# JokerYan/MS-GS

Hardware: AMD Instinct MI355X
Metric: Mpixels/s fwd+bwd @1080p, 1M Gaussians; fraction of HBM roofline (higher is better)
Workload: dtype f32

## Files before the change

### __graft_entry__.py

```python
import os
import subprocess
import sys

ROOT = os.path.dirname(os.path.abspath(__file__))
PKG = os.path.join(ROOT, "ms-gs_amd")


def _paths():
    for p in (ROOT, PKG, os.path.join(PKG, "host"), os.path.join(ROOT, "tests")):
        if p not in sys.path:
            sys.path.insert(0, p)


def build():
    subprocess.check_call(["make", "-C", PKG, "-j4"])
    subprocess.call(["make", "-C", PKG, "isa"], stdout=subprocess.DEVNULL, stderr=subprocess.DEVNULL)
    subprocess.check_call(["make", "-C", os.path.join(ROOT, "oracle")])
    _paths()
    import diff_gaussian_rasterization
    import gaussian_renderer
    import view_parallel
    lib = os.path.join(PKG, "lib", "libmsgs_hip.so")
    assert os.path.exists(lib), lib
    harness = os.path.join(PKG, "build", "libmsgs_sort_harness.so")
    assert os.path.exists(harness), harness
    print("built", lib)


def smoke():
    _paths()
    import torch
    assert torch.cuda.is_available(), "smoke() needs a GPU"
    import scenes
    from oracle import oracle_ctypes as oc
    from parity_utils import check_backward, check_forward, hip_render, small_scene
    torch.cuda.set_device(0)
    W, H = 160, 96
    sc, cam = small_scene(4000, W, H, seed=123, multiscale=True, scale_k=0.004 * 1920.0 / W * 0.25)
    st = dict(filter_small=True, filter_large=True, fade_size=0.0)
    bg = torch.tensor([0.1, 0.2, 0.3])
    dL = scenes.grad_seed(W, H, 123)
    out, pc, m2 = hip_render(sc, cam, st, bg, dL, device="cuda:0")
    orc = oc.rasterize(pc.seen, cam, st, bg)
    og = oc.backward(orc, dL)
    fwd = check_forward(out, orc, "smoke")
    bwd = check_backward(pc, m2, og, "smoke", flagged=orc.borderline_gaussians)
    print(f"smoke ok: visible={(out['radii'] > 0).sum().item()} fwd_maxdiff={fwd:.2e} bwd_rel={max(bwd.values()):.2e}")


if __name__ == "__main__":
    build()
    if len(sys.argv) > 1 and sys.argv[1] == "smoke":
        smoke()
```

### include/msgs.h

```cpp
#ifndef MSGS_H_
#define MSGS_H_

#include <stddef.h>
#include <stdint.h>

#ifdef __cplusplus
extern "C" {
#endif

#define MSGS_ABI_VERSION 11

#define MSGS_OK 0
#define MSGS_ERR_INVALID_ARG (-1)
#define MSGS_ERR_CAPACITY (-2)
#define MSGS_ERR_TOO_MANY (-3)
#define MSGS_ERR_SH_DEGREE (-4)
#define MSGS_ERR_INTERNAL (-5)

#define MSGS_TILE 16

typedef struct msgs_view {
    int32_t image_height;
    int32_t image_width;
    float tanfovx;
    float tanfovy;
    float scale_modifier;
    float fade_size;
    int32_t sh_degree;
    int32_t sh_coeffs;
    int32_t filter_small;
    int32_t filter_large;
    int32_t prefiltered;
    int32_t debug;
    int32_t no_heavy_queue;
    int32_t feedback_tag;
    float slab_fraction;
    int32_t reserved1;
    const float* bg;
    const float* viewmatrix;
    const float* projmatrix;
    const float* campos;
} msgs_view_t;

typedef struct msgs_gaussians {
    int32_t P;
    int32_t raw_params;
    const float* means3D;
    const float* shs;
    const float* colors_precomp;
    const float* opacities;
    const float* scales;
    const float* rotations;
    const float* cov3D_precomp;
    const float* max_pixel_sizes;
    const float* min_pixel_sizes;
    const float* occ_multiplier;
    const float* dc_delta;
    const uint8_t* base_mask;
    const float* features_dc;
    const float* features_rest;
    const float* rotations_raw;
} msgs_gaussians_t;

typedef struct msgs_adam_moments {
    float* exp_avg;
    float* exp_avg_sq;
    double lr;
} msgs_adam_moments_t;
typedef struct msgs_adam_in_backward {
    int64_t step;
    double beta1, beta2, eps;
    msgs_adam_moments_t t[6];
} msgs_adam_in_backward_t;

typedef struct msgs_grads {
    float* dL_dmeans3D;
    float* dL_dmeans2D;
    float* dL_dshs;
    float* dL_dcolors;
    float* dL_dopacities;
    float* dL_dscales;
    float* dL_drotations;
    float* dL_dcov3D;
    float* dL_dfeatures_dc;
    float* dL_dfeatures_rest;
    void* factors_ready;
    int32_t scratch_is_clear;
    int32_t accumulate;
    void* wait_before_accumulate;
    void* accumulated;
    const msgs_adam_in_backward_t* adam_in_backward;
} msgs_grads_t;

enum {
    MSGS_K_PREPROCESS = 0, MSGS_K_DEPTH_SORT = 1, MSGS_K_SCAN = 2, MSGS_K_EMIT = 3,
    MSGS_K_TILE_SORT = 4, MSGS_K_RANGES = 5, MSGS_K_BLEND_FWD = 6, MSGS_K_BLEND_BWD = 7,
    MSGS_K_PREPROCESS_BWD = 8,
    MSGS_K_SLAB_B = 9,
    MSGS_K_COUNT = 10
};
typedef struct msgs_timing {
    void* ev[2 * MSGS_K_COUNT];
} msgs_timing_t;

int msgs_abi_version(void);
const char* msgs_error_string(int code);

size_t msgs_geom_bytes(int32_t P);
size_t msgs_stage1_scratch_bytes(int32_t P);
size_t msgs_binning_bytes(int64_t num_instances, int32_t width, int32_t height);
size_t msgs_binning_bytes_slab(int64_t num_instances, int32_t width, int32_t height, float slab_fraction);
size_t msgs_stage2_scratch_bytes_slab(int64_t num_instances, int32_t width, int32_t height);
size_t msgs_stage2_scratch_bytes(int64_t num_instances, int32_t width, int32_t height);
size_t msgs_image_bytes(int32_t width, int32_t height);
size_t msgs_backward_scratch_bytes(int32_t P);

int msgs_forward_stage1(const msgs_view_t* view, const msgs_gaussians_t* g,
                        int32_t* radii, float* pixel_sizes,
                        void* geom, size_t geom_bytes,
                        void* scratch, size_t scratch_bytes,
                        int64_t* num_instances_host,
                        const msgs_timing_t* timing, void* stream);

int msgs_forward_stage2(const msgs_view_t* view, const msgs_gaussians_t* g,
                        const void* geom, size_t geom_bytes,
                        int64_t num_instances,
                        void* binning, size_t binning_bytes,
                        void* scratch, size_t scratch_bytes,
                        void* image_state, size_t image_bytes,
                        float* out_color, float* out_acc_pixel_size, float* out_depth,
                        void* grad_records, size_t grad_records_bytes, int32_t backward_follows,
                        const msgs_timing_t* timing, void* stream);

int msgs_backward(const msgs_view_t* view, const msgs_gaussians_t* g,
                  const int32_t* radii,
                  const void* geom, size_t geom_bytes,
                  int64_t num_instances,
                  const void* binning, size_t binning_bytes,
                  const void* image_state, size_t image_bytes,
                  const float* dL_dcolor,
                  void* scratch, size_t scratch_bytes,
                  const msgs_grads_t* grads,
                  const msgs_timing_t* timing, void* stream);

int msgs_backward_with_depth(const msgs_view_t* view, const msgs_gaussians_t* g,
                             const int32_t* radii,
                             const void* geom, size_t geom_bytes,
                             int64_t num_instances,
                             const void* binning, size_t binning_bytes,
                             const void* image_state, size_t image_bytes,
                             const float* dL_dcolor, const float* dL_ddepth,
                             void* scratch, size_t scratch_bytes,
                             const msgs_grads_t* grads,
                             const msgs_timing_t* timing, void* stream);

int msgs_backward_with_camera(const msgs_view_t* view, const msgs_gaussians_t* g,
                              const int32_t* radii,
                              const void* geom, size_t geom_bytes,
                              int64_t num_instances,
                              const void* binning, size_t binning_bytes,
                              const void* image_state, size_t image_bytes,
                              const float* dL_dcolor, const float* dL_ddepth,
                              void* scratch, size_t scratch_bytes,
                              const msgs_grads_t* grads,
                              float* dL_dviewmatrix, float* dL_dprojmatrix, float* dL_dcampos,
                              void* camera_scratch, size_t camera_scratch_bytes,
                              const msgs_timing_t* timing, void* stream);
size_t msgs_camera_grad_scratch_bytes(int32_t P);

int msgs_alpha_map(const msgs_view_t* view, const void* image_state, size_t image_bytes, float* out_alpha, void* stream);

int msgs_backward_with_alpha(const msgs_view_t* view, const msgs_gaussians_t* g,
                             const int32_t* radii,
                             const void* geom, size_t geom_bytes,
                             int64_t num_instances,
                             const void* binning, size_t binning_bytes,
                             const void* image_state, size_t image_bytes,
                             const float* dL_dcolor, const float* dL_ddepth, const float* dL_dalpha,
                             void* scratch, size_t scratch_bytes,
                             const msgs_grads_t* grads,
                             float* dL_dviewmatrix, float* dL_dprojmatrix, float* dL_dcampos,
                             void* camera_scratch, size_t camera_scratch_bytes,
                             const msgs_timing_t* timing, void* stream);

size_t msgs_bg_grad_scratch_bytes(int32_t width, int32_t height);
int msgs_bg_grad(const msgs_view_t* view, const void* image_state, size_t image_bytes, const float* dL_dcolor,
                 float* dL_dbg, void* scratch, size_t scratch_bytes, void* stream);

size_t msgs_absgrad_scratch_bytes(int32_t P);
int msgs_absgrad(const msgs_view_t* view, int32_t P,
                 const void* geom, size_t geom_bytes,
                 int64_t num_instances,
                 const void* binning, size_t binning_bytes,
                 const void* image_state, size_t image_bytes,
                 const float* dL_dcolor, const float* dL_ddepth, const float* dL_dalpha,
                 void* scratch, size_t scratch_bytes,
                 float* out_absgrad, void* stream);

size_t msgs_contrib_scratch_bytes(int32_t P);
int msgs_contrib_accumulate(const msgs_view_t* view, int32_t P,
                            const void* geom, size_t geom_bytes,
                            int64_t num_instances,
                            const void* binning, size_t binning_bytes,
                            const void* image_state, size_t image_bytes,
                            const float* pixel_weights,
                            void* acc, size_t acc_bytes, int32_t clear_first, void* stream);
int msgs_contrib_finish(int32_t P, const void* acc, size_t acc_bytes,
                        float* weight_sum, float* weight_max, int64_t* pixel_count, void* stream);

size_t msgs_features_scratch_bytes(int32_t P, int32_t C);
int msgs_features_forward(const msgs_view_t* view, int32_t P,
                          const void* geom, size_t geom_bytes,
                          int64_t num_instances,
                          const void* binning, size_t binning_bytes,
                          const void* image_state, size_t image_bytes,
                          const float* features, int32_t C,
                          float* out, void* stream);
int msgs_features_backward(const msgs_view_t* view, int32_t P,
                           const void* geom, size_t geom_bytes,
                           int64_t num_instances,
                           const void* binning, size_t binning_bytes,
                           const void* image_state, size_t image_bytes,
                           const float* features, int32_t C,
                           const float* dL_dfeature_map,
                           void* grad_records, size_t grad_records_bytes,
                           void* scratch, size_t scratch_bytes,
                           float* dL_dfeatures, void* stream);

int msgs_distortion_forward(const msgs_view_t* view, int32_t P,
                            const void* geom, size_t geom_bytes,
                            int64_t num_instances,
                            const void* binning, size_t binning_bytes,
                            const void* image_state, size_t image_bytes,
                            float* out_distortion, float* out_moment, void* stream);
int msgs_distortion_backward(const msgs_view_t* view, int32_t P,
                             const void* geom, size_t geom_bytes,
                             int64_t num_instances,
                             const void* binning, size_t binning_bytes,
                             const void* image_state, size_t image_bytes,
                             const float* moment, const float* dL_ddistortion,
                             void* grad_records, size_t grad_records_bytes, void* stream);

int msgs_median_depth_forward(const msgs_view_t* view, int32_t P,
                              const void* geom, size_t geom_bytes,
                              int64_t num_instances,
                              const void* binning, size_t binning_bytes,
                              const void* image_state, size_t image_bytes,
                              float* out_median_depth, int32_t* out_median_id, void* stream);
int msgs_median_depth_backward(const msgs_view_t* view, int32_t P,
                               const int32_t* median_id, const float* dL_dmedian_depth,
                               void* grad_records, size_t grad_records_bytes, void* stream);

size_t msgs_screen_compensation_scratch_bytes(int32_t P);
int msgs_screen_compensation_forward(const msgs_view_t* view, const msgs_gaussians_t* g, float* o_eff, void* stream);
int msgs_screen_compensation_backward(const msgs_view_t* view, const msgs_gaussians_t* g, const float* dL_do_eff,
                                      float* dL_dopacity, float* dL_dmeans3D, float* dL_dscales, float* dL_drotations,
                                      float* dL_dcov3D, float* dL_dV, void* scratch, size_t scratch_bytes, void* stream);

int msgs_backward_per_gaussian(const msgs_view_t* view, const msgs_gaussians_t* g, const int32_t* radii,
                               const void* geom, size_t geom_bytes, const double* sums2d, const msgs_grads_t* grads,
                               void* stream);

int msgs_sh_grad_from_views(int32_t P, int32_t n_views, int32_t sh_degree, const float* means3D, const float* campos,
                            int64_t campos_stride, const float* drgb, int64_t drgb_stride, float scale,
                            float* dL_dfeatures_dc, float* dL_dfeatures_rest, void* stream);

int msgs_mark_visible(int32_t P, const float* means3D, const float* viewmatrix,
                      const float* projmatrix, uint8_t* present, void* stream);

int msgs_binning_stats(const msgs_view_t* view, int32_t P, const int32_t* radii,
                       const void* binning, size_t binning_bytes,
                       const void* image_state, size_t image_bytes,
                       void* scratch, size_t scratch_bytes,
                       int64_t* out_host, void* stream);

int msgs_blend_lane_stats(const msgs_view_t* view, const void* geom, size_t geom_bytes, int32_t P, int64_t D,
                          const void* binning, size_t binning_bytes, const void* image_state, size_t image_bytes,
                          void* scratch, size_t scratch_bytes, int64_t* out_host, void* stream);

int msgs_set_deterministic(int32_t on);
int msgs_get_deterministic(void);
size_t msgs_backward_scratch_bytes_deterministic(int32_t P, int64_t D);
size_t msgs_backward_scratch_bytes_deterministic_depth(int32_t P, int64_t D);

int msgs_set_backward_generation(int32_t gen);

int msgs_set_blend_granularity(int32_t mode);

int msgs_set_occlusion(int32_t on);
int msgs_forward_info(int64_t* out_host);
int msgs_occlusion_stats(const void* geom, size_t geom_bytes, int32_t P, int64_t* out_host, void* stream);
int msgs_slab_stats(const void* geom, size_t geom_bytes, int32_t P, int64_t* out_host, void* stream);

int msgs_forward(const msgs_view_t* view, const msgs_gaussians_t* gaussians, int32_t* radii, float* pixel_sizes,
                 void* geom, size_t geom_bytes, void* scratch1, size_t scratch1_bytes, void* binning,
                 size_t binning_bytes, void* scratch2, size_t scratch2_bytes, void* image, size_t image_bytes,
                 float* out_color, float* out_acc_pixel_size, float* out_depth, void* grad_records,
                 size_t grad_records_bytes, int32_t backward_follows, int64_t* num_instances_host, int32_t* stage2_done,
                 const msgs_timing_t* timing, void* stream);

typedef struct msgs_status msgs_status_t;
int msgs_status_create(msgs_status_t** out);
int msgs_status_destroy(msgs_status_t* status);
int msgs_forward_launch(const msgs_view_t* view, const msgs_gaussians_t* gaussians, int32_t* radii, float* pixel_sizes,
                        void* geom, size_t geom_bytes, void* scratch1, size_t scratch1_bytes, void* binning,
                        size_t binning_bytes, void* scratch2, size_t scratch2_bytes, void* image, size_t image_bytes,
                        float* out_color, float* out_acc_pixel_size, float* out_depth, void* grad_records,
                        size_t grad_records_bytes, int32_t backward_follows, msgs_status_t* status,
                        const msgs_timing_t* timing, void* stream);
int msgs_forward_finish(msgs_status_t* status, int64_t* num_instances_host, int32_t* stage2_done);

int msgs_preprocess_only(const msgs_view_t* view, const msgs_gaussians_t* gaussians, int32_t* radii,
                         float* pixel_sizes, void* geom, size_t geom_bytes, void* stream);

size_t msgs_voxel_pool_scratch_bytes(int64_t M);
int msgs_voxel_pool_build(const float* positions, int64_t M, float voxel_size, uint32_t* order, uint32_t* seg_start,
                          int32_t* voxel_index, void* scratch, size_t scratch_bytes, int64_t* num_voxels_host,
                          void* stream);
int msgs_voxel_pool_average(const float* features, int32_t F, const uint32_t* order, const uint32_t* seg_start,
                            int64_t num_voxels, float* out, void* stream);

#define MSGS_ADAM_MAX_TENSORS 8
typedef struct msgs_adam_tensor {
    float* param;
    const float* grad;
    float* exp_avg;
    float* exp_avg_sq;
    int64_t n;
    double lr;
} msgs_adam_tensor_t;
int msgs_adam_step(const msgs_adam_tensor_t* tensors, int32_t n_tensors, int64_t step, double beta1, double beta2,
                   double eps, void* stream);

#define MSGS_STATS_BASE_MASK 1
#define MSGS_STATS_PIXEL_SIZES 2
#define MSGS_STATS_DENSIFY 4
typedef struct msgs_densify_stats {
    int32_t P;
    int32_t flags;
    int32_t reso_lvl;
    int32_t reso_lvls;
    const int32_t* radii;
    const float* pixel_sizes;
    const float* means2D_grad;
    const int64_t* target_reso_lvl;
    float* xyz_gradient_accum;
    float* denom;
    float* max_radii2D;
    float* max_pixel_sizes;
    float* min_pixel_sizes;
    uint8_t* base_mask;
} msgs_densify_stats_t;
int msgs_densify_stats(const msgs_densify_stats_t* stats, void* stream);

#define MSGS_DENSIFY_PRUNE 0
#define MSGS_DENSIFY_GROW 1
#define MSGS_DENSIFY_PRUNE_MASK 2
#define MSGS_DENSIFY_APPEND 3
typedef struct msgs_densify_select {
    int32_t mode;
    int32_t reso_lvl;
    int32_t reso_lvls;
    int32_t has_max_screen_size;
    int64_t P;
    int64_t n_append;
    float grad_threshold;
    float min_opacity;
    float scale_limit;
    float big_world_limit;
    float max_screen_size;
    int32_t reserved;
    const float* opacity;
    const float* scaling;
    float* xyz_gradient_accum;
    float* denom;
    const int64_t* target_reso_lvl;
    const uint8_t* prune_mask;
} msgs_densify_select_t;
size_t msgs_densify_scratch_bytes(int64_t P, int64_t n_append);
int msgs_densify_select(const msgs_densify_select_t* sel, void* scratch, size_t scratch_bytes, int64_t* counts_host,
                        void* stream);

#define MSGS_DR_COPY 0
#define MSGS_DR_ZERO 1
#define MSGS_DR_COPY_CLEAR_COL 2
#define MSGS_DR_SPLIT_XYZ 3
#define MSGS_DR_SPLIT_SCALE 4
#define MSGS_DR_SPLIT_DIV 5
#define MSGS_DR_GROW_OPACITY 6
#define MSGS_DR_GROW_SCALE 7
#define MSGS_DR_GROW_MUL 8
#define MSGS_DR_CONST 9
#define MSGS_DR_APPEND 10
#define MSGS_DENSIFY_MAX_TENSORS 32
typedef struct msgs_densify_tensor {
    void* dst;
    const void* src;
    const void* append_src;
    int64_t constant;
    int32_t width;
    int32_t elem_bytes;
    uint8_t rule[8];
} msgs_densify_tensor_t;
typedef struct msgs_densify_apply {
    int64_t P;
    int64_t n_append;
    int64_t P_out;
    int64_t n_split;
    int32_t n_tensors;
    int32_t reso_lvl;
    const float* xyz;
    const float* scaling;
    const float* rotation;
    const float* draws;
    const msgs_densify_tensor_t* tensors;
} msgs_densify_apply_t;
int msgs_densify_apply(const msgs_densify_apply_t* apply, const void* scratch, size_t scratch_bytes, void* stream);

size_t msgs_loss_scratch_bytes(int32_t C, int32_t H, int32_t W);
int msgs_loss_forward(const float* img, const float* gt, int32_t C, int32_t H, int32_t W, float lambda_dssim,
                      float* out3, void* scratch, size_t scratch_bytes, int32_t keep_for_backward, void* stream);
int msgs_loss_backward(const float* img, const float* gt, int32_t C, int32_t H, int32_t W, float lambda_dssim,
                       const float* upstream, const void* scratch, size_t scratch_bytes, float* dL_dimg, void* stream);
int msgs_ssim_window(float* taps11_host);

size_t msgs_knn_scratch_bytes(int64_t P);
int msgs_dist2_knn3(const float* points, int64_t P, float* mean_dist2, void* scratch, size_t scratch_bytes,
                    void* stream);

int msgs_timing_create(msgs_timing_t* t);
int msgs_timing_destroy(msgs_timing_t* t);
int msgs_timing_read(const msgs_timing_t* t, float* ms_host);

#ifdef __cplusplus
}
#endif
#endif
```

### ms-gs_amd/csrc/api.hip

```cpp
#include "msgs_internal.h"

#include <atomic>
#include <new>

#include <cstring>

using namespace msgs;

namespace {

struct Timer {
    const msgs_timing_t* t;
    hipStream_t s;
    void begin(int k) const { if (t && t->ev[2 * k]) (void)hipEventRecord((hipEvent_t)t->ev[2 * k], s); }
    void end(int k) const { if (t && t->ev[2 * k + 1]) (void)hipEventRecord((hipEvent_t)t->ev[2 * k + 1], s); }
};

inline int check_inputs(const msgs_view_t* v, const msgs_gaussians_t* g) {
    if (!v || !g) return MSGS_ERR_INVALID_ARG;
    if (g->P < 0 || v->image_width <= 0 || v->image_height <= 0) return MSGS_ERR_INVALID_ARG;
    if (!v->bg || !v->viewmatrix || !v->projmatrix || !v->campos) return MSGS_ERR_INVALID_ARG;
    if (g->P > 0 && (!g->means3D || !g->opacities)) return MSGS_ERR_INVALID_ARG;
    if (g->raw_params) {
        if (g->raw_params != 1 && g->raw_params != 2) return MSGS_ERR_INVALID_ARG;
        if (!g->features_dc || !g->features_rest || !g->scales || !g->rotations) return MSGS_ERR_INVALID_ARG;
        if (g->raw_params == 2 && !g->rotations_raw) return MSGS_ERR_INVALID_ARG;
        if ((g->shs && g->raw_params != 2) || g->colors_precomp || g->cov3D_precomp) return MSGS_ERR_INVALID_ARG;
        if (v->sh_degree < 0 || v->sh_degree > 3 || v->sh_coeffs != 16) return MSGS_ERR_SH_DEGREE;
        if ((v->image_width + TILE - 1) / TILE > 65535 || (v->image_height + TILE - 1) / TILE > 65535)
            return MSGS_ERR_INVALID_ARG;
        return MSGS_OK;
    }
    if ((g->shs != nullptr) == (g->colors_precomp != nullptr)) return MSGS_ERR_INVALID_ARG;
    const bool sr = g->scales != nullptr && g->rotations != nullptr;
    if ((g->scales != nullptr) != (g->rotations != nullptr)) return MSGS_ERR_INVALID_ARG;
    if (sr == (g->cov3D_precomp != nullptr)) return MSGS_ERR_INVALID_ARG;
    if (g->shs) {
        if (v->sh_degree < 0 || v->sh_degree > 3) return MSGS_ERR_SH_DEGREE;
        if ((v->sh_degree + 1) * (v->sh_degree + 1) > v->sh_coeffs) return MSGS_ERR_SH_DEGREE;
    }
    if ((v->image_width + TILE - 1) / TILE > 65535 || (v->image_height + TILE - 1) / TILE > 65535)
        return MSGS_ERR_INVALID_ARG;
    return MSGS_OK;
}

inline int debug_sync(const msgs_view_t* v, hipStream_t s) {
    if (!v->debug) return MSGS_OK;
    hipError_t e = hipStreamSynchronize(s);
    if (e != hipSuccess) return (int)e;
    e = hipGetLastError();
    return e == hipSuccess ? MSGS_OK : (int)e;
}

inline int tile_bits(int num_tiles) {
    int b = 1;
    while ((1ll << b) <= (long long)num_tiles) ++b;
    return b;
}

#define HIP_TRY(expr)                                   \
    do {                                                \
        hipError_t _e = (expr);                         \
        if (_e != hipSuccess) return (int)_e;           \
    } while (0)

}

extern "C" {

int msgs_abi_version(void) { return MSGS_ABI_VERSION; }

const char* msgs_error_string(int code) {
    switch (code) {
        case MSGS_OK: return "ok";
        case MSGS_ERR_INVALID_ARG: return "invalid argument (NULL or inconsistent pointers: provide exactly one of shs/colors_precomp and exactly one of scales+rotations/cov3D_precomp)";
        case MSGS_ERR_CAPACITY: return "a caller-supplied buffer is smaller than its size query";
        case MSGS_ERR_TOO_MANY: return "more than 2^32-1 tile instances";
        case MSGS_ERR_SH_DEGREE: return "sh_degree must be 0..3 and (sh_degree+1)^2 <= sh_coeffs";
        case MSGS_ERR_INTERNAL: return "internal error: a look-back wait in the sort/scan kernels timed out";
        default: return code > 0 ? hipGetErrorString((hipError_t)code) : "unknown error";
    }
}

size_t msgs_geom_bytes(int32_t P) { return GeomLayout(P > 0 ? P : 1).total; }
size_t msgs_stage1_scratch_bytes(int32_t P) { return Stage1Scratch(P > 0 ? P : 1).total; }
size_t msgs_binning_bytes(int64_t D, int32_t W, int32_t H) {
    return BinningLayout(D, (int64_t)((W + TILE - 1) / TILE) * ((H + TILE - 1) / TILE)).total;
}
size_t msgs_stage2_scratch_bytes(int64_t D, int32_t W, int32_t H) {
    (void)W; (void)H;
    const Stage2Scratch L(D);
    return L.total + align256(4 * (size_t)(D > 0 ? D : 1));
}
static int64_t tiles_of(int32_t W, int32_t H) { return (int64_t)((W + TILE - 1) / TILE) * ((H + TILE - 1) / TILE); }
size_t msgs_binning_bytes_slab(int64_t D, int32_t W, int32_t H, float fraction) {
    if (!(fraction > 0.f)) return msgs_binning_bytes(D, W, H);
    return msgs_binning_bytes(SlabGeom::ids_needed(D > 0 ? D : 1, (double)fraction, tiles_of(W, H)), W, H);
}
size_t msgs_stage2_scratch_bytes_slab(int64_t D, int32_t W, int32_t H) {
    return msgs_stage2_scratch_bytes((D > 0 ? D : 1) + SLAB_SLACK + 256, W, H);
}
size_t msgs_image_bytes(int32_t W, int32_t H) { return ImageLayout(W, H).total; }
size_t msgs_backward_scratch_bytes(int32_t P) {
    return align256(GRAD_REC_BYTES * (size_t)(P > 0 ? P : 1));
}
size_t msgs_backward_scratch_bytes_deterministic(int32_t P, int64_t D) { return DetScratch(P, D).total; }
size_t msgs_backward_scratch_bytes_deterministic_depth(int32_t P, int64_t D) { return DetScratch(P, D, DET_INST_FLOATS_DEPTH).total; }

static std::atomic<int> g_deterministic{[] { const char* e = getenv("MSGS_DETERMINISTIC"); return (e && e[0] == '1') ? 1 : 0; }()};
int msgs_set_deterministic(int32_t on) { return g_deterministic.exchange(on ? 1 : 0); }
int msgs_get_deterministic(void) { return g_deterministic.load(); }
int msgs_set_backward_generation(int32_t gen) { return set_backward_generation(gen); }
int msgs_set_blend_granularity(int32_t mode) { return set_blend_granularity(mode); }
int msgs_set_occlusion(int32_t on) { return set_occlusion(on); }

}

namespace {
struct Stage2Buffers {
    void* binning; size_t binning_bytes;
    void* scratch2; size_t scratch2_bytes;
    void* image; size_t image_bytes;
    float* out_color; float* out_acc_ps; float* out_depth;
    void* grad_records; size_t grad_records_bytes;
    int backward_follows;
};

struct SpecStage2 {
    int64_t capacity;
    Stage2Buffers buf;
    int launched_rc;
};
int forward_stage2_impl(const msgs_view_t* view, const msgs_gaussians_t* g, const void* geom_v, size_t geom_bytes, int64_t D,
                        const Stage2Buffers& b, const msgs_timing_t* timing, void* stream, const uint32_t* D_dev,
                        uint64_t* fb_dev, uint64_t fb_ticket);

struct StatusBlock {
    uint64_t* host = nullptr;
    uint64_t* dev = nullptr;
    uint64_t ticket = 0;
    bool tried = false;
    void ensure() {
        if (tried) return;
        tried = true;
        void* h = nullptr;
        if (hipHostMalloc(&h, 64, hipHostMallocPortable | hipHostMallocMapped) == hipSuccess) {
            void* d = nullptr;
            if (hipHostGetDevicePointer(&d, h, 0) == hipSuccess) {
                host = (uint64_t*)h;
                dev = (uint64_t*)d;
                for (int k = 0; k < 8; ++k) host[k] = 0;
            } else {
                (void)hipHostFree(h);
            }
        }
        (void)hipGetLastError();
    }
    void release() {
        if (host) (void)hipHostFree(host);
        host = dev = nullptr;
        tried = false;
    }
};

struct PendingCount {
    bool active = false;
    bool polled = false;
    hipStream_t stream = nullptr;
    uint64_t ticket = 0;
    volatile uint64_t* host = nullptr;
    const uint64_t* status_dev = nullptr;
};

thread_local uint64_t t_last_info = 0;
thread_local uint64_t t_last_feedback[4] = {0, 0, 0, 0};

static bool blocking_sync() {
    static const bool blocking = [] { const char* e = getenv("MSGS_BLOCKING_SYNC"); return e && e[0] == '1'; }();
    return blocking;
}

static bool slab_wanted(const msgs_view_t* view, const msgs_gaussians_t* g) {
    const float f = view->slab_fraction;
    if (!(f > 0.f) || !(f <= 0.5f) || g->P <= 0 || g_deterministic.load() != 0) return false;
    const int64_t tiles = (int64_t)((view->image_width + TILE - 1) / TILE) * ((view->image_height + TILE - 1) / TILE);
    return tiles >= SLAB_MIN_TILES && tiles < 65535 * 16 && forward_uses_quadrant_kernel((int)tiles);
}

int forward_stage1_launch(const msgs_view_t* view, const msgs_gaussians_t* g, int32_t* radii, float* pixel_sizes,
                          void* geom_v, size_t geom_bytes, void* scratch_v, size_t scratch_bytes,
                          const msgs_timing_t* timing, void* stream, SpecStage2* spec, StatusBlock& sb,
                          PendingCount& pend) {
    pend.active = false;
    int rc = check_inputs(view, g);
    if (rc) return rc;
    const int P = g->P;
    if (P == 0) return MSGS_OK;
    if (!radii || !pixel_sizes || !geom_v || !scratch_v) return MSGS_ERR_INVALID_ARG;
    if (geom_bytes < msgs_geom_bytes(P) || scratch_bytes < msgs_stage1_scratch_bytes(P)) return MSGS_ERR_CAPACITY;
    hipStream_t s = (hipStream_t)stream;
    char* geom = (char*)geom_v;
    char* scratch = (char*)scratch_v;
    const GeomLayout GL(P);
    const Stage1Scratch SL(P);
    const ViewParams vp = make_view_params(view);
    const Timer tm{timing, s};

    ZeroJob zj1{nullptr, 0, (uint32_t*)(geom + GL.slab_hdr), (GL.occ_hdr - GL.slab_hdr) / 4 + sizeof(OccHeader) / 4 + 2 * (size_t)OCC_BUCKETS};
    const bool sort1_prezeroed = radix_sort_zero_region(P, 0, 32, scratch + SL.sort, &zj1.p0, &zj1.n0);
    const bool occlusion = get_occlusion() != 0;
    uint32_t* heavy_list = occlusion ? (uint32_t*)(scratch + SL.heavy_list) : nullptr;
    uint32_t* heavy_count = occlusion ? (uint32_t*)(scratch + SL.heavy_count) : nullptr;
    uint32_t* heavy_blk = occlusion ? (uint32_t*)(scratch + SL.heavy_blk) : nullptr;
    tm.begin(MSGS_K_PREPROCESS);
    HIP_TRY(launch_preprocess(vp, *g, radii, pixel_sizes, geom, s, zj1, heavy_list, heavy_count, heavy_blk, g_deterministic.load() != 0));
    if (occlusion)
        HIP_TRY(launch_occlusion(vp, P, geom, heavy_list, heavy_count, heavy_blk, (OccCand*)(scratch + SL.occ_cand), s));
    tm.end(MSGS_K_PREPROCESS);
    if ((rc = debug_sync(view, s))) return rc;

    if (!blocking_sync()) sb.ensure();
    const bool polled = !blocking_sync() && sb.host != nullptr;
    const uint64_t ticket = ++sb.ticket;
    uint64_t* total_dev = (uint64_t*)(scratch + SL.total_out);
    uint64_t* status_dev = total_dev + 2;
    uint32_t* clamped_dev = (uint32_t*)(total_dev + 5);
    uint32_t* heavy_q_word = spec ? (uint32_t*)((char*)spec->buf.scratch2 + Stage2Scratch(spec->capacity).heavy_q) : nullptr;

    tm.begin(MSGS_K_DEPTH_SORT);
    HIP_TRY(radix_sort_pairs((uint32_t*)(geom + GL.key), nullptr, (uint32_t*)(geom + GL.skey),
                             (uint32_t*)(geom + GL.order), P, 0, 32, scratch + SL.sort, s, sort1_prezeroed,
                             (uint32_t*)(geom + GL.nvalid)));
    tm.end(MSGS_K_DEPTH_SORT);
    if ((rc = debug_sync(view, s))) return rc;
    tm.begin(MSGS_K_SCAN);
    HIP_TRY(exclusive_scan_u32((const uint32_t*)(geom + GL.tiles), (const uint32_t*)(geom + GL.order),
                               (uint32_t*)(geom + GL.offs), P, (uint64_t*)(scratch + SL.scan_partials), total_dev, s,
                               status_dev, polled ? sb.dev : nullptr, ticket,
                               (const uint32_t*)(geom + GL.nvalid), spec ? clamped_dev : nullptr,
                               spec ? (uint64_t)spec->capacity : 0, (const uint32_t*)(geom + GL.occ_hdr), heavy_q_word, nullptr,
                               vp.cell_sx >= 0 ? TILE_COUNT_MASK : 0xFFFFFFFFu,
                               vp.cell_sx >= 0 && slab_wanted(view, g) ? (uint32_t*)(geom + GL.offs_b) : nullptr,
                               &reinterpret_cast<SlabHeader*>(geom + GL.slab_hdr)->pad[0]));
    tm.end(MSGS_K_SCAN);
    pend.active = true;
    pend.polled = polled;
    pend.stream = s;
    pend.ticket = ticket;
    pend.host = sb.host;
    pend.status_dev = status_dev;
    if (spec)
        spec->launched_rc = forward_stage2_impl(view, g, geom_v, geom_bytes, spec->capacity, spec->buf, timing, stream,
                                                clamped_dev, polled ? sb.dev : nullptr, ticket);
    return MSGS_OK;
}

int forward_stage1_wait(PendingCount& pend, int64_t* num_instances_host) {
    *num_instances_host = 0;
    if (!pend.active) { t_last_info = 0; for (int k = 0; k < 4; ++k) t_last_feedback[k] = 0; return MSGS_OK; }
    pend.active = false;
    hipStream_t s = pend.stream;
    uint64_t host_status[3] = {0, 0, 0};
    if (pend.polled) {
        volatile uint64_t* hv = pend.host;
        const uint64_t ticket = pend.ticket;
        uint64_t spins = 0;
        while (hv[2] != ticket) {
            if ((++spins & 0xFFFF) == 0) {
                const hipError_t q = hipStreamQuery(s);
                if (q != hipErrorNotReady && q != hipSuccess) return (int)q;
                if (q == hipSuccess && hv[2] != ticket) {
                    HIP_TRY(hipMemcpyAsync(host_status, pend.status_dev, sizeof(host_status), hipMemcpyDeviceToHost, s));
                    HIP_TRY(hipStreamSynchronize(s));
                    break;
                }
            }
        }
        if (hv[2] == ticket) { host_status[0] = hv[0]; host_status[1] = hv[1]; host_status[2] = hv[3]; }
        for (int k = 0; k < 4; ++k) t_last_feedback[k] = 0;
        for (int attempt = 0; attempt < 4; ++attempt) {
            const uint64_t w7 = hv[7], w4 = hv[4], w5 = hv[5], w6 = hv[6];
            if (hv[7] == w7) { t_last_feedback[0] = w4; t_last_feedback[1] = w5; t_last_feedback[2] = w6; t_last_feedback[3] = w7; break; }
        }
    } else {
        for (int k = 0; k < 4; ++k) t_last_feedback[k] = 0;
        HIP_TRY(hipMemcpyAsync(host_status, pend.status_dev, sizeof(host_status), hipMemcpyDeviceToHost, s));
        HIP_TRY(hipStreamSynchronize(s));
    }
    const uint64_t total = host_status[0];
    t_last_info = host_status[2];
    if (host_status[1] != 0) return MSGS_ERR_INTERNAL;
    if (total > 0xFFFFFFFFull) return MSGS_ERR_TOO_MANY;
    *num_instances_host = (int64_t)total;
    return MSGS_OK;
}

StatusBlock& thread_status_block() {
    static thread_local StatusBlock sb;
    return sb;
}

template <class F>
static int64_t max_instances_for(size_t bytes, F bytes_of) {
    if (bytes_of(1) > bytes) return 0;
    int64_t lo = 1, hi = 0xFFFFFFFFll;
    while (lo < hi) {
        const int64_t mid = lo + (hi - lo + 1) / 2;
        if (bytes_of(mid) <= bytes) lo = mid; else hi = mid - 1;
    }
    return lo;
}

void stage2_capacities(const msgs_view_t* view, size_t binning_bytes, size_t scratch2_bytes, int64_t& cb, int64_t& cs) {
    const int W0 = view->image_width, H0 = view->image_height;
    cb = max_instances_for(binning_bytes, [&](int64_t d) { return msgs_binning_bytes(d, W0, H0); });
    cs = max_instances_for(scratch2_bytes, [&](int64_t d) { return msgs_stage2_scratch_bytes(d, W0, H0); });
}

bool prepare_spec(const msgs_view_t* view, const msgs_gaussians_t* g, const Stage2Buffers& b, SpecStage2& spec) {
    if (view->debug || g->P <= 0 || !b.binning || !b.scratch2 || !b.image || !b.out_color || !b.out_acc_ps || !b.out_depth ||
        view->image_width <= 0 || view->image_height <= 0)
        return false;
    const int W0 = view->image_width, H0 = view->image_height;
    int64_t cb, cs;
    stage2_capacities(view, b.binning_bytes, b.scratch2_bytes, cb, cs);
    int64_t cap = cb < cs ? cb : cs;
    const int tiles0 = ((W0 + TILE - 1) / TILE) * ((H0 + TILE - 1) / TILE);
    if (slab_wanted(view, g)) {
        const SlabGeom SG(cb, cs, (double)view->slab_fraction, tiles0, (int64_t)1 << 40);
        if (SG.ok && SG.cap_d >= 4096) cap = SG.cap_d;
    }
    if (cap < 4096 || !radix_sort_supports_device_count(cap, 0, tile_bits(tiles0))) return false;
    spec.capacity = cap;
    spec.buf = b;
    spec.launched_rc = MSGS_OK;
    return true;
}

struct ForwardLaunch {
    PendingCount pend;
    bool spec = false;
    int64_t capacity = 0;
    int launched_rc = MSGS_OK;
};

int forward_launch(const msgs_view_t* view, const msgs_gaussians_t* g, int32_t* radii, float* pixel_sizes, void* geom,
                   size_t geom_bytes, void* scratch1, size_t scratch1_bytes, const Stage2Buffers* b,
                   const msgs_timing_t* timing, void* stream, StatusBlock& sb, ForwardLaunch& fl) {
    SpecStage2 spec{};
    fl.spec = b && prepare_spec(view, g, *b, spec);
    const int rc = forward_stage1_launch(view, g, radii, pixel_sizes, geom, geom_bytes, scratch1, scratch1_bytes, timing,
                                         stream, fl.spec ? &spec : nullptr, sb, fl.pend);
    if (rc) return rc;
    fl.capacity = spec.capacity;
    fl.launched_rc = spec.launched_rc;
    return MSGS_OK;
}

int forward_finish(ForwardLaunch& fl, int64_t* num_instances_host, int32_t* stage2_done) {
    *stage2_done = 0;
    const int rc = forward_stage1_wait(fl.pend, num_instances_host);
    if (rc) return rc;
    if (fl.spec && fl.launched_rc != MSGS_OK) return fl.launched_rc;
    *stage2_done = fl.spec && *num_instances_host <= fl.capacity;
    return MSGS_OK;
}

int forward_stage2_exact(const msgs_view_t* view, const msgs_gaussians_t* g, const void* geom, size_t geom_bytes, int64_t D,
                         const Stage2Buffers& b, const msgs_timing_t* timing, void* stream) {
    uint64_t* fb_dev = nullptr;
    uint64_t fb_ticket = 0;
    if (view && view->feedback_tag != 0 && !blocking_sync()) {
        StatusBlock& sb = thread_status_block();
        sb.ensure();
        fb_dev = sb.dev;
        fb_ticket = sb.ticket;
    }
    return forward_stage2_impl(view, g, geom, geom_bytes, D, b, timing, stream, nullptr, fb_dev, fb_ticket);
}

}

struct msgs_status {
    StatusBlock sb;
    ForwardLaunch fl;
    bool launched = false;
};

extern "C" {

int msgs_forward_stage1(const msgs_view_t* view, const msgs_gaussians_t* g, int32_t* radii, float* pixel_sizes,
                        void* geom_v, size_t geom_bytes, void* scratch_v, size_t scratch_bytes,
                        int64_t* num_instances_host, const msgs_timing_t* timing, void* stream) {
    if (!num_instances_host) return MSGS_ERR_INVALID_ARG;
    *num_instances_host = 0;
    ForwardLaunch fl;
    int32_t stage2_done;
    const int rc = forward_launch(view, g, radii, pixel_sizes, geom_v, geom_bytes, scratch_v, scratch_bytes, nullptr, timing,
                                  stream, thread_status_block(), fl);
    return rc ? rc : forward_finish(fl, num_instances_host, &stage2_done);
}

int msgs_status_create(msgs_status_t** out) {
    if (!out) return MSGS_ERR_INVALID_ARG;
    *out = new (std::nothrow) msgs_status();
    if (!*out) return (int)hipErrorOutOfMemory;
    if (!blocking_sync()) (*out)->sb.ensure();
    return MSGS_OK;
}

int msgs_status_destroy(msgs_status_t* st) {
    if (!st) return MSGS_OK;
    if (st->launched && st->fl.pend.active) (void)hipStreamSynchronize(st->fl.pend.stream);
    st->sb.release();
    delete st;
    return MSGS_OK;
}

int msgs_forward_launch(const msgs_view_t* view, const msgs_gaussians_t* g, int32_t* radii, float* pixel_sizes, void* geom,
                        size_t geom_bytes, void* scratch1, size_t scratch1_bytes, void* binning, size_t binning_bytes,
                        void* scratch2, size_t scratch2_bytes, void* image, size_t image_bytes, float* out_color,
                        float* out_acc_ps, float* out_depth, void* grad_records, size_t grad_records_bytes,
                        int32_t backward_follows, msgs_status_t* status, const msgs_timing_t* timing, void* stream) {
    if (!view || !g || !status) return MSGS_ERR_INVALID_ARG;
    if (status->launched) return MSGS_ERR_INVALID_ARG;
    const Stage2Buffers b{binning, binning_bytes, scratch2, scratch2_bytes, image, image_bytes, out_color, out_acc_ps, out_depth,
                          grad_records, grad_records_bytes, backward_follows};
    const int rc = forward_launch(view, g, radii, pixel_sizes, geom, geom_bytes, scratch1, scratch1_bytes, &b, timing, stream,
                                  status->sb, status->fl);
    if (rc) return rc;
    status->launched = true;
    return MSGS_OK;
}

int msgs_forward_finish(msgs_status_t* status, int64_t* num_instances_host, int32_t* stage2_done) {
    if (!status || !num_instances_host || !stage2_done) return MSGS_ERR_INVALID_ARG;
    *stage2_done = 0;
    *num_instances_host = 0;
    if (!status->launched) return MSGS_ERR_INVALID_ARG;
    status->launched = false;
    return forward_finish(status->fl, num_instances_host, stage2_done);
}

int msgs_forward(const msgs_view_t* view, const msgs_gaussians_t* g, int32_t* radii, float* pixel_sizes, void* geom,
                 size_t geom_bytes, void* scratch1, size_t scratch1_bytes, void* binning, size_t binning_bytes,
                 void* scratch2, size_t scratch2_bytes, void* image, size_t image_bytes, float* out_color,
                 float* out_acc_ps, float* out_depth, void* grad_records, size_t grad_records_bytes,
                 int32_t backward_follows, int64_t* num_instances_host, int32_t* stage2_done, const msgs_timing_t* timing,
                 void* stream) {
    if (!stage2_done) return MSGS_ERR_INVALID_ARG;
    *stage2_done = 0;
    if (!view || !g || !num_instances_host) return MSGS_ERR_INVALID_ARG;
    *num_instances_host = 0;
    const Stage2Buffers b{binning, binning_bytes, scratch2, scratch2_bytes, image, image_bytes, out_color, out_acc_ps, out_depth,
                          grad_records, grad_records_bytes, backward_follows};
    ForwardLaunch fl;
    int rc = forward_launch(view, g, radii, pixel_sizes, geom, geom_bytes, scratch1, scratch1_bytes, &b, timing, stream,
                            thread_status_block(), fl);
    if (!rc) rc = forward_finish(fl, num_instances_host, stage2_done);
    if (rc || fl.spec) return rc;
    const int64_t D = *num_instances_host;
    const int W = view->image_width, H = view->image_height;
    if (!binning || binning_bytes < msgs_binning_bytes(D, W, H)) return MSGS_OK;
    if (D > 0 && (!scratch2 || scratch2_bytes < msgs_stage2_scratch_bytes(D, W, H))) return MSGS_OK;
    if ((rc = forward_stage2_exact(view, g, geom, geom_bytes, D, b, timing, stream))) return rc;
    *stage2_done = 1;
    return MSGS_OK;
}

int msgs_preprocess_only(const msgs_view_t* view, const msgs_gaussians_t* g, int32_t* radii, float* pixel_sizes,
                         void* geom_v, size_t geom_bytes, void* stream) {
    int rc = check_inputs(view, g);
    if (rc) return rc;
    const int P = g->P;
    if (P == 0) return MSGS_OK;
    if (!radii || !pixel_sizes || !geom_v) return MSGS_ERR_INVALID_ARG;
    if (geom_bytes < msgs_geom_bytes(P)) return MSGS_ERR_CAPACITY;
    hipStream_t s = (hipStream_t)stream;
    HIP_TRY(launch_preprocess(make_view_params(view), *g, radii, pixel_sizes, (char*)geom_v, s));
    return debug_sync(view, s);
}

int msgs_forward_stage2(const msgs_view_t* view, const msgs_gaussians_t* g, const void* geom_v, size_t geom_bytes,
                        int64_t D, void* binning_v, size_t binning_bytes, void* scratch_v, size_t scratch_bytes,
                        void* image_v, size_t image_bytes, float* out_color, float* out_acc_ps, float* out_depth,
                        void* grad_records, size_t grad_records_bytes, int32_t backward_follows, const msgs_timing_t* timing,
                        void* stream) {
    const Stage2Buffers b{binning_v, binning_bytes, scratch_v, scratch_bytes, image_v, image_bytes, out_color, out_acc_ps,
                          out_depth, grad_records, grad_records_bytes, backward_follows};
    return forward_stage2_exact(view, g, geom_v, geom_bytes, D, b, timing, stream);
}

}

namespace {
int forward_stage2_impl(const msgs_view_t* view, const msgs_gaussians_t* g, const void* geom_v, size_t geom_bytes, int64_t D,
                        const Stage2Buffers& b, const msgs_timing_t* timing, void* stream, const uint32_t* D_dev,
                        uint64_t* fb_dev, uint64_t fb_ticket) {
    int rc = check_inputs(view, g);
    if (rc) return rc;
    if (D < 0 || D > 0xFFFFFFFFll) return MSGS_ERR_TOO_MANY;
    const int P = g->P, W = view->image_width, H = view->image_height;
    if (!b.binning || !b.image || !b.out_color || !b.out_acc_ps || !b.out_depth) return MSGS_ERR_INVALID_ARG;
    if (P > 0 && (!geom_v || geom_bytes < msgs_geom_bytes(P))) return MSGS_ERR_CAPACITY;
    if (b.binning_bytes < msgs_binning_bytes(D, W, H) || b.image_bytes < msgs_image_bytes(W, H)) return MSGS_ERR_CAPACITY;
    if (D > 0 && (!b.scratch2 || b.scratch2_bytes < msgs_stage2_scratch_bytes(D, W, H))) return MSGS_ERR_CAPACITY;
    if (b.grad_records && b.grad_records_bytes < msgs_backward_scratch_bytes(P)) return MSGS_ERR_CAPACITY;
    hipStream_t s = (hipStream_t)stream;
    char* geom = const_cast<char*>((const char*)geom_v);
    char* binning = (char*)b.binning;
    char* scratch = (char*)b.scratch2;
    char* image = (char*)b.image;
    const ViewParams vp = make_view_params(view);
    const int num_tiles = vp.gx * vp.gy;
    const ImageLayout IL(W, H);
    const Timer tm{timing, s};
    const int tbits = tile_bits(num_tiles);
    const BinningLayout BL(D, num_tiles);
    uint32_t* ids = (uint32_t*)(binning + BL.ids);
    uint2* ranges = (uint2*)(binning + BL.ranges);
    float* final_T = (float*)(image + IL.final_T);
    uint32_t* n_contrib = (uint32_t*)(image + IL.n_contrib);
    uint32_t* tile_last = (uint32_t*)(image + IL.tile_last);
    const bool literal = g_deterministic.load() != 0;
    const bool feedback = view->feedback_tag != 0 && fb_dev != nullptr && P > 0 && forward_uses_quadrant_kernel(num_tiles) && !literal;
    unsigned long long* dtrav = feedback ? (unsigned long long*)(binning + BL.dtrav) : nullptr;
    const size_t clear_bytes = b.grad_records ? GRAD_REC_BYTES * (size_t)P : 0;

    bool slab = D > 0 && slab_wanted(view, g) && radix_sort_supports_device_count(D, 0, tbits);
    int64_t n_a_max = 0, cap_b = 0;
    if (slab) {
        int64_t cb, cs;
        stage2_capacities(view, b.binning_bytes, b.scratch2_bytes, cb, cs);
        const SlabGeom SG(cb, cs, (double)view->slab_fraction, num_tiles, D);
        slab = SG.ok && SG.cap_d == D && SortScratch(SG.n_a_max).total <= SortScratch(SG.cap_b).total;
// ... 326 lines not shown
    if (P == 0 || D == 0) {
        HIP_TRY(launch_zero(out_distortion, sizeof(float) * (size_t)W * H, s));
        HIP_TRY(launch_zero(out_moment, sizeof(float) * (size_t)W * H, s));
        return debug_sync(view, s);
    }
    if (!geom_v || !binning_v || !image_v) return MSGS_ERR_INVALID_ARG;
    if (geom_bytes < msgs_geom_bytes(P) || binning_bytes < msgs_binning_bytes(D, W, H) || image_bytes < msgs_image_bytes(W, H))
        return MSGS_ERR_CAPACITY;
    const ViewParams vp = make_view_params(view);
    const BinningLayout BL(D, vp.gx * vp.gy);
    const ImageLayout IL(W, H);
    const char* binning = (const char*)binning_v;
    const char* image = (const char*)image_v;
    HIP_TRY(launch_blend_distortion_forward(vp, (const char*)geom_v, (const uint32_t*)(binning + BL.ids),
                                            (const uint2*)(binning + BL.ranges), (const float*)(image + IL.final_T),
                                            (const uint32_t*)(image + IL.n_contrib), out_distortion, out_moment, s));
    return debug_sync(view, s);
}

int msgs_distortion_backward(const msgs_view_t* view, int32_t P, const void* geom_v, size_t geom_bytes, int64_t D,
                             const void* binning_v, size_t binning_bytes, const void* image_v, size_t image_bytes,
                             const float* moment, const float* dL_ddistortion, void* grad_records, size_t grad_records_bytes,
                             void* stream) {
    if (!view || P < 0 || D < 0 || view->image_width < 1 || view->image_height < 1) return MSGS_ERR_INVALID_ARG;
    if (g_deterministic.load() != 0) return MSGS_ERR_INVALID_ARG;
    if (P == 0 || D == 0) return MSGS_OK;
    if (!geom_v || !binning_v || !image_v || !moment || !dL_ddistortion || !grad_records || ((uintptr_t)grad_records & 7))
        return MSGS_ERR_INVALID_ARG;
    const int W = view->image_width, H = view->image_height;
    if (geom_bytes < msgs_geom_bytes(P) || binning_bytes < msgs_binning_bytes(D, W, H) || image_bytes < msgs_image_bytes(W, H) ||
        grad_records_bytes < msgs_backward_scratch_bytes(P))
        return MSGS_ERR_CAPACITY;
    hipStream_t s = (hipStream_t)stream;
    const ViewParams vp = make_view_params(view);
    const BinningLayout BL(D, vp.gx * vp.gy);
    const ImageLayout IL(W, H);
    const char* binning = (const char*)binning_v;
    const char* image = (const char*)image_v;
    HIP_TRY(launch_blend_distortion_backward(vp, (const char*)geom_v, (const uint32_t*)(binning + BL.ids),
                                             (const uint2*)(binning + BL.ranges), (const float*)(image + IL.final_T),
                                             (const uint32_t*)(image + IL.n_contrib), moment, dL_ddistortion,
                                             (grad_acc_t*)grad_records, s));
    return debug_sync(view, s);
}

int msgs_median_depth_forward(const msgs_view_t* view, int32_t P, const void* geom_v, size_t geom_bytes, int64_t D,
                              const void* binning_v, size_t binning_bytes, const void* image_v, size_t image_bytes,
                              float* out_median_depth, int32_t* out_median_id, void* stream) {
    if (!view || P < 0 || D < 0 || view->image_width < 1 || view->image_height < 1 || !out_median_depth || !out_median_id)
        return MSGS_ERR_INVALID_ARG;
    if (g_deterministic.load() != 0) return MSGS_ERR_INVALID_ARG;
    const int W = view->image_width, H = view->image_height;
    hipStream_t s = (hipStream_t)stream;
    if (P == 0 || D == 0) {
        HIP_TRY(launch_zero(out_median_depth, sizeof(float) * (size_t)W * H, s));
        HIP_TRY(hipMemsetAsync(out_median_id, 0xFF, sizeof(int32_t) * (size_t)W * H, s));
        return debug_sync(view, s);
    }
    if (!geom_v || !binning_v || !image_v) return MSGS_ERR_INVALID_ARG;
    if (geom_bytes < msgs_geom_bytes(P) || binning_bytes < msgs_binning_bytes(D, W, H) || image_bytes < msgs_image_bytes(W, H))
        return MSGS_ERR_CAPACITY;
    const ViewParams vp = make_view_params(view);
    const BinningLayout BL(D, vp.gx * vp.gy);
    const ImageLayout IL(W, H);
    const char* binning = (const char*)binning_v;
    const char* image = (const char*)image_v;
    HIP_TRY(launch_blend_median_depth_forward(vp, (const char*)geom_v, (const uint32_t*)(binning + BL.ids),
                                              (const uint2*)(binning + BL.ranges), (const uint32_t*)(image + IL.n_contrib),
                                              out_median_depth, out_median_id, s));
    return debug_sync(view, s);
}

int msgs_median_depth_backward(const msgs_view_t* view, int32_t P, const int32_t* median_id, const float* dL_dmedian_depth,
                               void* grad_records, size_t grad_records_bytes, void* stream) {
    if (!view || P < 0 || view->image_width < 1 || view->image_height < 1) return MSGS_ERR_INVALID_ARG;
    if (g_deterministic.load() != 0) return MSGS_ERR_INVALID_ARG;
    if (P == 0) return MSGS_OK;
    if (!median_id || !dL_dmedian_depth || !grad_records || ((uintptr_t)grad_records & 7)) return MSGS_ERR_INVALID_ARG;
    if (grad_records_bytes < msgs_backward_scratch_bytes(P)) return MSGS_ERR_CAPACITY;
    hipStream_t s = (hipStream_t)stream;
    const ViewParams vp = make_view_params(view);
    HIP_TRY(launch_median_depth_backward(vp, P, median_id, dL_dmedian_depth, (grad_acc_t*)grad_records, s));
    return debug_sync(view, s);
}

}
namespace {
inline int check_compensation_inputs(const msgs_view_t* v, const msgs_gaussians_t* g) {
    if (!v || !g || g->P < 0 || v->image_width <= 0 || v->image_height <= 0 || !v->viewmatrix) return MSGS_ERR_INVALID_ARG;
    if (g->raw_params != 0) return MSGS_ERR_INVALID_ARG;
    if (g->P == 0) return MSGS_OK;
    if (!g->means3D || !g->opacities) return MSGS_ERR_INVALID_ARG;
    const bool sr = g->scales != nullptr && g->rotations != nullptr;
    if ((g->scales != nullptr) != (g->rotations != nullptr) || sr == (g->cov3D_precomp != nullptr)) return MSGS_ERR_INVALID_ARG;
    return MSGS_OK;
}
}
extern "C" {

size_t msgs_screen_compensation_scratch_bytes(int32_t P) { return screen_compensation_rows_bytes(P); }

int msgs_screen_compensation_forward(const msgs_view_t* view, const msgs_gaussians_t* g, float* o_eff, void* stream) {
    const int rc = check_compensation_inputs(view, g);
    if (rc != MSGS_OK) return rc;
    if (g->P == 0) return MSGS_OK;
    if (!o_eff) return MSGS_ERR_INVALID_ARG;
    hipStream_t s = (hipStream_t)stream;
    HIP_TRY(launch_screen_compensation_forward(make_view_params(view), *g, o_eff, s));
    return debug_sync(view, s);
}

int msgs_screen_compensation_backward(const msgs_view_t* view, const msgs_gaussians_t* g, const float* dL_do_eff,
                                      float* dL_dopacity, float* dL_dmeans3D, float* dL_dscales, float* dL_drotations,
                                      float* dL_dcov3D, float* dL_dV, void* scratch, size_t scratch_bytes, void* stream) {
    const int rc = check_compensation_inputs(view, g);
    if (rc != MSGS_OK) return rc;
    hipStream_t s = (hipStream_t)stream;
    if (g->P == 0) {
        if (dL_dV) HIP_TRY(launch_zero(dL_dV, sizeof(float) * 16, s));
        return debug_sync(view, s);
    }
    if (!dL_do_eff) return MSGS_ERR_INVALID_ARG;
    if ((g->cov3D_precomp && (dL_dscales || dL_drotations)) || (!g->cov3D_precomp && dL_dcov3D)) return MSGS_ERR_INVALID_ARG;
    if (dL_dV) {
        if (!scratch || ((uintptr_t)scratch & 7)) return MSGS_ERR_INVALID_ARG;
        if (scratch_bytes < msgs_screen_compensation_scratch_bytes(g->P)) return MSGS_ERR_CAPACITY;
    }
    HIP_TRY(launch_screen_compensation_backward(make_view_params(view), *g, dL_do_eff, dL_dopacity, dL_dmeans3D, dL_dscales,
                                                dL_drotations, dL_dcov3D, dL_dV, (double*)scratch, s));
    return debug_sync(view, s);
}
}

namespace {
int backward_impl(const msgs_view_t* view, const msgs_gaussians_t* g, const int32_t* radii, const void* geom_v,
                  size_t geom_bytes, int64_t D, const void* binning_v, size_t binning_bytes, const void* image_v,
                  size_t image_bytes, const float* dL_dcolor, const float* dL_ddepth, const float* dL_dalpha, void* scratch_v,
                  size_t scratch_bytes, const msgs_grads_t* grads, const CameraGrads* cam, const msgs_timing_t* timing,
                  void* stream) {
    int rc = check_inputs(view, g);
    if (rc) return rc;
    if (!grads || !dL_dcolor) return MSGS_ERR_INVALID_ARG;
    const int P = g->P, W = view->image_width, H = view->image_height;
    if (P == 0) {
        if (cam) {
            hipStream_t s0 = (hipStream_t)stream;
            if (cam->dL_dviewmatrix) HIP_TRY(hipMemsetAsync(cam->dL_dviewmatrix, 0, 16 * sizeof(float), s0));
            if (cam->dL_dprojmatrix) HIP_TRY(hipMemsetAsync(cam->dL_dprojmatrix, 0, 16 * sizeof(float), s0));
            if (cam->dL_dcampos) HIP_TRY(hipMemsetAsync(cam->dL_dcampos, 0, 3 * sizeof(float), s0));
        }
        return MSGS_OK;
    }
    if (!radii || !geom_v || !binning_v || !image_v || !scratch_v) return MSGS_ERR_INVALID_ARG;
    const bool det = g_deterministic.load() != 0;
    if (geom_bytes < msgs_geom_bytes(P) || binning_bytes < msgs_binning_bytes(D, W, H) ||
        image_bytes < msgs_image_bytes(W, H) ||
        scratch_bytes < (det ? (dL_ddepth ? msgs_backward_scratch_bytes_deterministic_depth(P, D)
                                          : msgs_backward_scratch_bytes_deterministic(P, D))
                             : msgs_backward_scratch_bytes(P)))
        return MSGS_ERR_CAPACITY;
    if (g->shs && !g->raw_params && !grads->dL_dshs) return MSGS_ERR_INVALID_ARG;
    if (g->raw_params && (!grads->dL_dfeatures_dc != !grads->dL_dfeatures_rest)) return MSGS_ERR_INVALID_ARG;
    if (g->raw_params && !grads->dL_dfeatures_dc && !grads->dL_dcolors && !grads->adam_in_backward) return MSGS_ERR_INVALID_ARG;
    if (const msgs_adam_in_backward_t* ad = grads->adam_in_backward) {
        if (g->raw_params != 1 || !g->features_dc || !g->features_rest || g->shs || g->colors_precomp || g->cov3D_precomp ||
            !g->scales || !g->rotations || view->sh_coeffs != 16 || grads->accumulate || grads->wait_before_accumulate ||
            ad->step < 1)
            return MSGS_ERR_INVALID_ARG;
        uintptr_t bits = (uintptr_t)g->means3D | (uintptr_t)g->features_dc | (uintptr_t)g->features_rest |
                         (uintptr_t)g->opacities | (uintptr_t)g->scales | (uintptr_t)g->rotations;
        for (int t = 0; t < 6; ++t) {
            if (!ad->t[t].exp_avg || !ad->t[t].exp_avg_sq) return MSGS_ERR_INVALID_ARG;
            bits |= (uintptr_t)ad->t[t].exp_avg | (uintptr_t)ad->t[t].exp_avg_sq;
        }
        if (bits & 15) return MSGS_ERR_INVALID_ARG;
    }
    if (grads->accumulate && ((g->shs && !g->raw_params && view->sh_coeffs != 16) ||
                              (g->raw_params && !grads->dL_dfeatures_dc)))
        return MSGS_ERR_INVALID_ARG;
    hipStream_t s = (hipStream_t)stream;
    const char* geom = (const char*)geom_v;
    const char* binning = (const char*)binning_v;
    const char* image = (const char*)image_v;
    const ViewParams vp = make_view_params(view);
    const BinningLayout BL(D, vp.gx * vp.gy);
    const ImageLayout IL(W, H);
    const Timer tm{timing, s};
    grad_acc_t* grad_rec = (grad_acc_t*)scratch_v;

    if (det && grads->scratch_is_clear) return MSGS_ERR_INVALID_ARG;
    if (!grads->scratch_is_clear)
        HIP_TRY(launch_zero(grad_rec, GRAD_REC_BYTES * (size_t)P, s));
    tm.begin(MSGS_K_BLEND_BWD);
    if (det)
        HIP_TRY(launch_blend_backward_det(vp, P, geom, (const uint32_t*)(binning + BL.ids), D,
                                          (const uint2*)(binning + BL.ranges), (const float*)(image + IL.final_T),
                                          (const uint32_t*)(image + IL.n_contrib), dL_dcolor, (char*)scratch_v, s, dL_ddepth,
                                          dL_dalpha));
    else
        HIP_TRY(launch_blend_backward(vp, geom, (const uint32_t*)(binning + BL.ids), (const uint2*)(binning + BL.ranges),
                                      (const float*)(image + IL.final_T), (const uint32_t*)(image + IL.n_contrib),
                                      dL_dcolor, grad_rec, s, (const uint32_t*)(image + IL.tile_order), dL_ddepth,
                                      dL_dalpha));
    tm.end(MSGS_K_BLEND_BWD);
    if ((rc = debug_sync(view, s))) return rc;

    tm.begin(MSGS_K_PREPROCESS_BWD);
    HIP_TRY(launch_preprocess_backward(vp, *g, radii, geom, grad_rec, *grads, s, det, dL_ddepth != nullptr, cam));
    tm.end(MSGS_K_PREPROCESS_BWD);
    return debug_sync(view, s);
}
}

extern "C" {

int msgs_backward_per_gaussian(const msgs_view_t* view, const msgs_gaussians_t* g, const int32_t* radii,
                               const void* geom_v, size_t geom_bytes, const double* sums2d, const msgs_grads_t* grads,
                               void* stream) {
    int rc = check_inputs(view, g);
    if (rc) return rc;
    if (!grads || g->raw_params || grads->adam_in_backward) return MSGS_ERR_INVALID_ARG;
    if (grads->accumulate || grads->wait_before_accumulate || grads->accumulated) return MSGS_ERR_INVALID_ARG;
    const int P = g->P;
    if (P == 0) return MSGS_OK;
    if (!radii || !geom_v || !sums2d) return MSGS_ERR_INVALID_ARG;
    if (geom_bytes < msgs_geom_bytes(P)) return MSGS_ERR_CAPACITY;
    if (g->shs && !grads->dL_dshs) return MSGS_ERR_INVALID_ARG;
    hipStream_t s = (hipStream_t)stream;
    HIP_TRY(launch_preprocess_backward(make_view_params(view), *g, radii, (const char*)geom_v,
                                       reinterpret_cast<const grad_acc_t*>(sums2d), *grads, s, true));
    return debug_sync(view, s);
}

int msgs_sh_grad_from_views(int32_t P, int32_t n_views, int32_t sh_degree, const float* means3D, const float* campos,
                            int64_t campos_stride, const float* drgb, int64_t drgb_stride, float scale,
                            float* dL_dfeatures_dc, float* dL_dfeatures_rest, void* stream) {
    if (P < 0 || n_views < 1 || sh_degree < 0 || sh_degree > 3 || campos_stride < 0 || drgb_stride < 0)
        return MSGS_ERR_INVALID_ARG;
    if (P > 0 && (!means3D || !campos || !drgb || !dL_dfeatures_dc || !dL_dfeatures_rest)) return MSGS_ERR_INVALID_ARG;
    HIP_TRY(launch_sh_grad_from_views(P, n_views, sh_degree, means3D, campos, campos_stride, drgb, drgb_stride, scale,
                                      dL_dfeatures_dc, dL_dfeatures_rest, (hipStream_t)stream));
    return MSGS_OK;
}

int msgs_mark_visible(int32_t P, const float* means3D, const float* viewmatrix, const float* projmatrix,
                      uint8_t* present, void* stream) {
    if (P < 0 || (P > 0 && (!means3D || !viewmatrix || !present))) return MSGS_ERR_INVALID_ARG;
    HIP_TRY(launch_mark_visible(P, means3D, viewmatrix, projmatrix, present, (hipStream_t)stream));
    return MSGS_OK;
}

int msgs_binning_stats(const msgs_view_t* view, int32_t P, const int32_t* radii, const void* binning,
                       size_t binning_bytes, const void* image_v, size_t image_bytes, void* scratch,
                       size_t scratch_bytes, int64_t* out_host, void* stream) {
    (void)binning; (void)binning_bytes;
    if (!view || !image_v || !scratch || !out_host || scratch_bytes < 16) return MSGS_ERR_INVALID_ARG;
    const int W = view->image_width, H = view->image_height;
    if (image_bytes < msgs_image_bytes(W, H)) return MSGS_ERR_CAPACITY;
    hipStream_t s = (hipStream_t)stream;
    const ViewParams vp = make_view_params(view);
    const ImageLayout IL(W, H);
    unsigned long long* dev = (unsigned long long*)scratch;
    HIP_TRY(launch_binning_stats(vp, P, radii, (const uint32_t*)((const char*)image_v + IL.n_contrib), dev, s));
    unsigned long long host[2] = {0, 0};
    HIP_TRY(hipMemcpyAsync(host, dev, 16, hipMemcpyDeviceToHost, s));
    HIP_TRY(hipStreamSynchronize(s));
    out_host[0] = (int64_t)host[0];
    out_host[1] = (int64_t)host[1];
    return MSGS_OK;
}

int msgs_forward_info(int64_t* out_host) {
    if (!out_host) return MSGS_ERR_INVALID_ARG;
    out_host[0] = (int64_t)(t_last_info & 0xFFFFFFFFull);
    out_host[1] = (int64_t)(t_last_info >> 32) != 0 ? 1 : 0;
    const uint64_t w4 = t_last_feedback[0], w5 = t_last_feedback[1], w6 = t_last_feedback[2], w7 = t_last_feedback[3];
    const uint32_t n_open = (uint32_t)(w5 >> 32);
    out_host[2] = (int64_t)(w5 & 0xFFFFFFFFull);
    out_host[3] = (int64_t)(w7 & 0xFFFFFFFFFFull);
    out_host[4] = (int64_t)(w4 & ~(1ull << 63));
    out_host[5] = n_open == 0xFFFFFFFFu ? -1 : (int64_t)n_open;
    out_host[6] = (int64_t)(w6 & 0xFFFFFFFFull);
    out_host[7] = (w4 >> 63) ? -1 : (int64_t)(w6 >> 32);
    return MSGS_OK;
}

int msgs_slab_stats(const void* geom_v, size_t geom_bytes, int32_t P, int64_t* out_host, void* stream) {
    if (!geom_v || !out_host || P <= 0) return MSGS_ERR_INVALID_ARG;
    if (geom_bytes < msgs_geom_bytes(P)) return MSGS_ERR_CAPACITY;
    const GeomLayout GL(P);
    SlabHeader h;
    hipStream_t s = (hipStream_t)stream;
    HIP_TRY(hipMemcpyAsync(&h, (const char*)geom_v + GL.slab_hdr, sizeof(h), hipMemcpyDeviceToHost, s));
    HIP_TRY(hipStreamSynchronize(s));
    out_host[0] = h.active;
    out_host[1] = h.rA;
    out_host[2] = h.DA;
    out_host[3] = h.n_open;
    out_host[4] = (int64_t)h.total_b;
    out_host[5] = h.pad0;
    return MSGS_OK;
}

int msgs_occlusion_stats(const void* geom_v, size_t geom_bytes, int32_t P, int64_t* out_host, void* stream) {
    if (!geom_v || !out_host || P <= 0) return MSGS_ERR_INVALID_ARG;
    if (geom_bytes < msgs_geom_bytes(P)) return MSGS_ERR_CAPACITY;
    const GeomLayout GL(P);
    OccHeader h;
    hipStream_t s = (hipStream_t)stream;
    static uint32_t table[OCC_MAX_BLOCKS];
    HIP_TRY(hipMemcpyAsync(&h, (const char*)geom_v + GL.occ_hdr, sizeof(h), hipMemcpyDeviceToHost, s));
    HIP_TRY(hipStreamSynchronize(s));
    for (int k = 0; k < 8; ++k) out_host[k] = 0;
    out_host[0] = h.enabled ? (h.watchdog ? 2 : 1) : 0;
    if (!h.enabled) return MSGS_OK;
    const int n_blocks = (int)(h.nbx * h.nby);
    if (n_blocks < 0 || n_blocks > OCC_MAX_BLOCKS) return MSGS_ERR_INTERNAL;
    if (h.any_closed) {
        HIP_TRY(hipMemcpyAsync(table, (const char*)geom_v + GL.occ_cut, 4 * (size_t)n_blocks, hipMemcpyDeviceToHost, s));
        HIP_TRY(hipStreamSynchronize(s));
    } else {
        for (int k = 0; k < n_blocks; ++k) table[k] = 0xFFFFu;
    }
    uint32_t lo = 0xFFFFFFFFu, hi = 0u;
    int closed = 0;
    for (int k = 0; k < n_blocks; ++k) {
        const uint32_t key = table[k] >= 0xFFFFu ? 0xFFFFFFFFu : (((table[k] + OCC_KEY_BASE + 1u) << OCC_KEY_SHIFT) - 1u);
        closed += key != 0xFFFFFFFFu;
        lo = key < lo ? key : lo;
        hi = key > hi ? key : hi;
    }
    out_host[1] = h.n_heavy;
    out_host[2] = h.n_cand;
    out_host[3] = closed;
    out_host[4] = n_blocks;
    out_host[5] = 1u << h.block_log2;
    out_host[6] = lo;
    out_host[7] = hi;
    return MSGS_OK;
}

int msgs_blend_lane_stats(const msgs_view_t* view, const void* geom, size_t geom_bytes, int32_t P, int64_t D,
                          const void* binning_v, size_t binning_bytes, const void* image_v, size_t image_bytes,
                          void* scratch, size_t scratch_bytes, int64_t* out_host, void* stream) {
    if (!view || !geom || !binning_v || !scratch || !out_host || scratch_bytes < 64 || P < 0) return MSGS_ERR_INVALID_ARG;
    const int W = view->image_width, H = view->image_height;
    if (geom_bytes < msgs_geom_bytes(P) || binning_bytes < msgs_binning_bytes(D, W, H)) return MSGS_ERR_CAPACITY;
    if (image_v && image_bytes < msgs_image_bytes(W, H)) return MSGS_ERR_CAPACITY;
    hipStream_t s = (hipStream_t)stream;
    const ViewParams vp = make_view_params(view);
    const BinningLayout BL(D, vp.gx * vp.gy);
    const ImageLayout IL(W, H);
    const char* binning = (const char*)binning_v;
    unsigned long long* dev = (unsigned long long*)scratch;
    HIP_TRY(launch_blend_lane_stats(vp, (const char*)geom, (const uint32_t*)(binning + BL.ids),
                                    (const uint2*)(binning + BL.ranges), dev, s));
    if (image_v)
        HIP_TRY(launch_blend_backward_lane_stats(vp, (const char*)geom, (const uint32_t*)(binning + BL.ids),
                                                 (const uint2*)(binning + BL.ranges),
                                                 (const float*)((const char*)image_v + IL.final_T),
                                                 (const uint32_t*)((const char*)image_v + IL.n_contrib), dev + 4, s));
    unsigned long long host[8] = {0, 0, 0, 0, 0, 0, 0, 0};
    HIP_TRY(hipMemcpyAsync(host, dev, 64, hipMemcpyDeviceToHost, s));
    HIP_TRY(hipStreamSynchronize(s));
    for (int k = 0; k < 3; ++k) out_host[k] = (int64_t)host[k];
    for (int k = 0; k < 4; ++k) out_host[3 + k] = image_v ? (int64_t)host[4 + k] : -1;
    return MSGS_OK;
}

int msgs_adam_step(const msgs_adam_tensor_t* tensors, int32_t n_tensors, int64_t step, double beta1, double beta2,
                   double eps, void* stream) {
    if (n_tensors < 0 || n_tensors > MSGS_ADAM_MAX_TENSORS || step < 1 || (n_tensors && !tensors))
        return MSGS_ERR_INVALID_ARG;
    for (int k = 0; k < n_tensors; ++k) {
        const msgs_adam_tensor_t& t = tensors[k];
        if (t.n < 0 || (t.n > 0 && (!t.param || !t.grad || !t.exp_avg || !t.exp_avg_sq))) return MSGS_ERR_INVALID_ARG;
        if (t.n > (int64_t)1 << 40) return MSGS_ERR_TOO_MANY;
    }
    HIP_TRY(launch_adam(tensors, n_tensors, step, beta1, beta2, eps, (hipStream_t)stream));
    return MSGS_OK;
}

int msgs_densify_stats(const msgs_densify_stats_t* d, void* stream) {
    if (!d || d->P < 0 || d->reso_lvls < 1 || d->reso_lvl < 0 || d->reso_lvl >= d->reso_lvls) return MSGS_ERR_INVALID_ARG;
    if (d->P == 0 || d->flags == 0) return MSGS_OK;
    if (!d->radii) return MSGS_ERR_INVALID_ARG;
    if ((d->flags & MSGS_STATS_BASE_MASK) && !d->base_mask) return MSGS_ERR_INVALID_ARG;
    if ((d->flags & MSGS_STATS_PIXEL_SIZES) &&
        (!d->pixel_sizes || !d->target_reso_lvl || !d->max_pixel_sizes || !d->min_pixel_sizes)) return MSGS_ERR_INVALID_ARG;
    if ((d->flags & MSGS_STATS_DENSIFY) && (!d->means2D_grad || !d->xyz_gradient_accum || !d->denom || !d->max_radii2D))
        return MSGS_ERR_INVALID_ARG;
    HIP_TRY(launch_densify_stats(*d, (hipStream_t)stream));
    return MSGS_OK;
}

size_t msgs_densify_scratch_bytes(int64_t P, int64_t n_append) {
    return densify_scratch_bytes(P > 0 ? P : 0, n_append > 0 ? n_append : 0);
}

int msgs_densify_select(const msgs_densify_select_t* sel, void* scratch, size_t scratch_bytes, int64_t* counts_host,
                        void* stream) {
    if (!sel || !counts_host || !scratch) return MSGS_ERR_INVALID_ARG;
    if (int rc = densify_check_select(*sel)) return rc;
    if (scratch_bytes < densify_scratch_bytes(sel->P, sel->n_append)) return MSGS_ERR_CAPACITY;
    return densify_select(*sel, (char*)scratch, counts_host, (hipStream_t)stream);
}

int msgs_densify_apply(const msgs_densify_apply_t* apply, const void* scratch, size_t scratch_bytes, void* stream) {
    if (!apply || !scratch) return MSGS_ERR_INVALID_ARG;
    if (int rc = densify_check_apply(*apply)) return rc;
    if (scratch_bytes < densify_scratch_bytes(apply->P, apply->n_append)) return MSGS_ERR_CAPACITY;
    return densify_apply(*apply, (const char*)scratch, (hipStream_t)stream);
}

static int loss_args_ok(const float* img, const float* gt, int32_t C, int32_t H, int32_t W, float lambda) {
    if (!img || !gt || C < 1 || H < 1 || W < 1 || !(lambda >= 0.f && lambda <= 1.f)) return MSGS_ERR_INVALID_ARG;
    if ((int64_t)C * H * W > (int64_t)1 << 31 || C > 65535) return MSGS_ERR_TOO_MANY;
    return MSGS_OK;
}

size_t msgs_loss_scratch_bytes(int32_t C, int32_t H, int32_t W) {
    if (C < 1 || H < 1 || W < 1) return 0;
    return loss_scratch_bytes(C, H, W);
}

int msgs_loss_forward(const float* img, const float* gt, int32_t C, int32_t H, int32_t W, float lambda_dssim,
                      float* out3, void* scratch, size_t scratch_bytes, int32_t keep_for_backward, void* stream) {
    if (int rc = loss_args_ok(img, gt, C, H, W, lambda_dssim)) return rc;
    if (!out3 || !scratch) return MSGS_ERR_INVALID_ARG;
    if (scratch_bytes < loss_scratch_bytes(C, H, W)) return MSGS_ERR_CAPACITY;
    HIP_TRY(launch_loss_forward(img, gt, C, H, W, lambda_dssim, out3, (char*)scratch, keep_for_backward != 0,
                                (hipStream_t)stream));
    return MSGS_OK;
}

int msgs_loss_backward(const float* img, const float* gt, int32_t C, int32_t H, int32_t W, float lambda_dssim,
                       const float* upstream, const void* scratch, size_t scratch_bytes, float* dL_dimg, void* stream) {
    if (int rc = loss_args_ok(img, gt, C, H, W, lambda_dssim)) return rc;
    if (!dL_dimg || !scratch) return MSGS_ERR_INVALID_ARG;
    if (scratch_bytes < loss_scratch_bytes(C, H, W)) return MSGS_ERR_CAPACITY;
    HIP_TRY(launch_loss_backward(img, gt, C, H, W, lambda_dssim, upstream, (const char*)scratch, dL_dimg,
                                 (hipStream_t)stream));
    return MSGS_OK;
}

int msgs_ssim_window(float* taps11_host) {
    if (!taps11_host) return MSGS_ERR_INVALID_ARG;
    ssim_window_host(taps11_host);
    return MSGS_OK;
}

size_t msgs_knn_scratch_bytes(int64_t P) { return knn_scratch_bytes(P); }

int msgs_dist2_knn3(const float* points, int64_t P, float* mean_dist2, void* scratch, size_t scratch_bytes,
                    void* stream) {
    if (P < 4 || !points || !mean_dist2 || !scratch) return MSGS_ERR_INVALID_ARG;
    if (P > 0x7FFFFFFFll) return MSGS_ERR_TOO_MANY;
    if (scratch_bytes < knn_scratch_bytes(P)) return MSGS_ERR_CAPACITY;
    HIP_TRY(knn_mean_dist2(points, P, mean_dist2, (char*)scratch, (hipStream_t)stream));
    return MSGS_OK;
}

size_t msgs_voxel_pool_scratch_bytes(int64_t M) { return voxel_pool_scratch_bytes(M); }

int msgs_voxel_pool_build(const float* positions, int64_t M, float voxel_size, uint32_t* order, uint32_t* seg_start,
                          int32_t* voxel_index, void* scratch, size_t scratch_bytes, int64_t* num_voxels_host,
                          void* stream) {
    if (!num_voxels_host || M < 0 || !(voxel_size > 0.f)) return MSGS_ERR_INVALID_ARG;
    *num_voxels_host = 0;
    if (M == 0) return MSGS_OK;
    if (M > 0x7FFFFFFFll) return MSGS_ERR_TOO_MANY;
    if (!positions || !order || !seg_start || !scratch) return MSGS_ERR_INVALID_ARG;
    if (scratch_bytes < voxel_pool_scratch_bytes(M)) return MSGS_ERR_CAPACITY;
    HIP_TRY(voxel_pool_build(positions, M, voxel_size, order, seg_start, voxel_index, (char*)scratch, num_voxels_host,
                             (hipStream_t)stream));
    return MSGS_OK;
}

int msgs_voxel_pool_average(const float* features, int32_t F, const uint32_t* order, const uint32_t* seg_start,
                            int64_t num_voxels, float* out, void* stream) {
    if (F < 0 || num_voxels < 0) return MSGS_ERR_INVALID_ARG;
    if (F == 0 || num_voxels == 0) return MSGS_OK;
    if (!features || !order || !seg_start || !out) return MSGS_ERR_INVALID_ARG;
    HIP_TRY(voxel_pool_average(features, F, order, seg_start, num_voxels, out, (hipStream_t)stream));
    return MSGS_OK;
}

int msgs_timing_create(msgs_timing_t* t) {
    if (!t) return MSGS_ERR_INVALID_ARG;
    std::memset(t, 0, sizeof(*t));
    for (int i = 0; i < 2 * MSGS_K_COUNT; ++i) {
        hipEvent_t e;
        HIP_TRY(hipEventCreate(&e));
        t->ev[i] = (void*)e;
    }
    return MSGS_OK;
}

int msgs_timing_destroy(msgs_timing_t* t) {
    if (!t) return MSGS_ERR_INVALID_ARG;
    for (int i = 0; i < 2 * MSGS_K_COUNT; ++i)
        if (t->ev[i]) { (void)hipEventDestroy((hipEvent_t)t->ev[i]); t->ev[i] = nullptr; }
    return MSGS_OK;
}

int msgs_timing_read(const msgs_timing_t* t, float* ms_host) {
    if (!t || !ms_host) return MSGS_ERR_INVALID_ARG;
    for (int k = 0; k < MSGS_K_COUNT; ++k) {
        float ms = -1.0f;
        if (t->ev[2 * k] && t->ev[2 * k + 1]) {
            if (hipEventElapsedTime(&ms, (hipEvent_t)t->ev[2 * k], (hipEvent_t)t->ev[2 * k + 1]) != hipSuccess) {
                ms = -1.0f;
                (void)hipGetLastError();
            }
        }
        ms_host[k] = ms;
    }
    return MSGS_OK;
}

}
```

### ms-gs_amd/csrc/msgs_internal.h

```cpp
#pragma once
#include <hip/hip_runtime.h>
#include <stdint.h>
#include <cmath>
#include <type_traits>
#include "../../include/msgs.h"

namespace msgs {

constexpr int TILE = MSGS_TILE;
constexpr int WAVE = 64;

struct __attribute__((aligned(16))) GaussRec { float4 r0, r1, r2; };

struct __attribute__((aligned(32))) BinRec { float4 q0, q1; };

#if defined(MSGS_GRAD_REC_F32)
typedef float grad_acc_t;
constexpr int GRAD_REC_FLOATS = 12;
#else
typedef double grad_acc_t;
constexpr int GRAD_REC_FLOATS = 10;
#endif
constexpr uint32_t TILE_ORDER_MAGIC = 0x4C505431u;
constexpr size_t GRAD_REC_BYTES = sizeof(grad_acc_t) * GRAD_REC_FLOATS;
constexpr int DET_INST_FLOATS = 9;
constexpr int DET_INST_FLOATS_DEPTH = 10;

__host__ __device__ inline size_t align256(size_t x) { return (x + 255) & ~size_t(255); }

constexpr int OCC_MAX_BLOCKS = 2048;
constexpr int OCC_MAX_CAND = 32768;
constexpr uint32_t OCC_HEAVY_MIN = 96;
constexpr int OCC_BUCKETS = 2048;
constexpr int OCC_KEY_SHIFT = 19;
constexpr uint32_t OCC_KEY_BASE = 0x3E4CCCCDu >> OCC_KEY_SHIFT;
struct OccHeader {
    uint32_t n_cand;
    uint32_t any_closed;
    uint32_t n_heavy;
    uint32_t enabled;
    uint32_t block_log2;
    uint32_t nbx;
    uint32_t nby;
    uint32_t n_written;
    uint32_t depth_limit;
    uint32_t bar[3];
    uint32_t watchdog;
    uint32_t pad[3];
};
static_assert(sizeof(OccHeader) == 64, "OccHeader layout");
constexpr int SLAB_SCAN_CHUNK = 4096;
struct __attribute__((aligned(16))) OccCand { float4 c0, c1; uint32_t rect_lo, rect_hi, pad0, pad1; };
static_assert(sizeof(OccCand) == 48, "OccCand layout");

struct SlabHeader {
    uint32_t rA;
    uint32_t DA;
    uint32_t DB;
    uint32_t active;
    uint32_t n_open;
    uint32_t pad0;
    uint64_t total_b;
    uint32_t pad[8];
};
static_assert(sizeof(SlabHeader) == 64, "SlabHeader layout");

struct GeomLayout {
    size_t rec, binrec, tiles, key, flags, weight, order, offs, nvalid, skey, slab_hdr, occ_hdr, occ_cut, offs_b, scan_b, litrec, shjac, total;
    __host__ __device__ explicit GeomLayout(int64_t P) {
        size_t o = 0;
        rec = o;    o = align256(o + sizeof(GaussRec) * P);
        binrec = o; o = align256(o + sizeof(BinRec) * P);
        tiles = o;  o = align256(o + 4 * P);
        key = o;    o = align256(o + 4 * P);
        flags = o;  o = align256(o + 4 * P);
        weight = o; o = align256(o + 4 * P);
        order = o;  o = align256(o + 4 * P);
        offs = o;   o = align256(o + 4 * P);
        nvalid = o; o += 256;
        skey = o;   o = align256(o + 4 * P);
        slab_hdr = o; o += 256;
        occ_hdr = o; o = align256(o + sizeof(OccHeader) + 8 * (size_t)OCC_BUCKETS);
        occ_cut = o; o = align256(o + 4 * (size_t)OCC_MAX_BLOCKS);
        offs_b = o; o = align256(o + 4 * P);
        scan_b = o; o = align256(o + 8 * (size_t)((P + SLAB_SCAN_CHUNK - 1) / SLAB_SCAN_CHUNK + 2));
        litrec = o; o = align256(o + 16 * P);
        shjac = o;  o = align256(o + 36 * P);
        total = o;
    }
};

constexpr int SORT_THREADS = 256;
constexpr int SORT_ITEMS = 4;
constexpr int64_t SORT_BIG_N = 2'000'000;
constexpr int64_t SORT_MID_N = 400'000;
constexpr int SORT_MAX_GROUPS = 128;
constexpr int64_t SORT_SCANNED_MIN_BLOCKS = 4096;
constexpr int SORT_SCANNED_GSIZE = 32;
constexpr int SCAN_THREADS = 256;
constexpr int SCAN_ITEMS = 16;
constexpr int SCAN_CHUNK = SCAN_THREADS * SCAN_ITEMS;
static_assert(SCAN_CHUNK == SLAB_SCAN_CHUNK, "GeomLayout::scan_b is sized with SLAB_SCAN_CHUNK");

__host__ __device__ inline int64_t scan_blocks(int64_t n) { return (n + SCAN_CHUNK - 1) / SCAN_CHUNK; }

struct SortGeom {
    bool big, mid, scanned;
    int items, gsize, ngroups;
    int64_t nb;
    __host__ __device__ explicit SortGeom(int64_t n) {
        if (n < 1) n = 1;
        big = n >= SORT_BIG_N;
        mid = !big && n >= SORT_MID_N;
        items = big ? 16 : (mid ? 8 : SORT_ITEMS);
        nb = (n + (int64_t)SORT_THREADS * items - 1) / ((int64_t)SORT_THREADS * items);
        scanned = big && nb >= SORT_SCANNED_MIN_BLOCKS;
        if (scanned) {
            gsize = SORT_SCANNED_GSIZE;
        } else {
            gsize = 8;
            while ((int64_t)gsize * gsize < nb) gsize += 8;
            const int64_t floor_g = (nb + SORT_MAX_GROUPS - 1) / SORT_MAX_GROUPS;
            if (floor_g > gsize) gsize = (int)floor_g;
        }
        ngroups = (int)((nb + gsize - 1) / gsize);
    }
    __host__ __device__ size_t zero_words(int passes) const { return (size_t)passes * 256 * ngroups; }
};

struct SortScratch {
    size_t keys_alt, vals_alt, hist, total;
    __host__ __device__ explicit SortScratch(int64_t n) {
        size_t o = 0;
        const size_t nn = (size_t)(n > 0 ? n : 1);
        const SortGeom G(n);
        keys_alt = o; o = align256(o + 4 * nn);
        vals_alt = o; o = align256(o + 4 * nn);
        hist = o;     o = align256(o + 4 * ((size_t)256 * G.nb + G.zero_words(4)));
        total = o;
    }
};

struct Stage1Scratch {
    size_t sort, scan_partials, total_out, heavy_list, heavy_count, heavy_blk, occ_cand, total;
    __host__ __device__ explicit Stage1Scratch(int64_t P) {
        size_t o = 0;
        const size_t Pn = (size_t)(P > 0 ? P : 1);
        const size_t waves = 4 * ((Pn + 255) / 256);
        sort = o;          o = align256(o + SortScratch(P).total);
        scan_partials = o; o = align256(o + 8 * (size_t)(scan_blocks(P > 0 ? P : 1) + 2));
        total_out = o;     o = align256(o + 64);
        heavy_list = o;    o = align256(o + 8 * 64 * waves);
        heavy_count = o;   o = align256(o + 4 * waves);
        heavy_blk = o;     o = align256(o + 2 * waves);
        occ_cand = o;      o = align256(o + sizeof(OccCand) * OCC_MAX_CAND);
        total = o;
    }
};

constexpr int DTRAV_SLOTS = 64;
struct BinningLayout {
    size_t ids, ranges, dtrav, total;
    __host__ __device__ BinningLayout(int64_t D, int64_t tiles) {
        size_t o = 0;
        ranges = o; o = align256(o + 8 * (size_t)tiles);
        dtrav = o;  o = align256(o + 8 * (size_t)DTRAV_SLOTS);
        ids = o;    o = align256(o + 4 * (size_t)(D > 0 ? D : 1));
        total = o;
    }
    __host__ __device__ size_t ranges_and_dtrav_words() const { return (dtrav + 8 * (size_t)DTRAV_SLOTS - ranges) / 4; }
};

constexpr int64_t SLAB_SLACK = 65536;
constexpr int SLAB_MIN_TILES = 2048;
struct SlabGeom {
    int64_t cap_d, n_a_max, cap_b;
    bool ok;
    __host__ SlabGeom(int64_t cb, int64_t cs, double fraction, int64_t tiles, int64_t cap_d_limit) {
        const int64_t by_ids = (int64_t)((double)(cb - tiles - SLAB_SLACK - 256) / (1.0 + fraction));
        const int64_t by_scratch = cs - SLAB_SLACK;
        cap_d = by_ids < by_scratch ? by_ids : by_scratch;
        if (cap_d > cap_d_limit) cap_d = cap_d_limit;
        if (cap_d < 0) cap_d = 0;
        n_a_max = (((int64_t)(fraction * (double)cap_d) + tiles + 64) + 63) & ~(int64_t)63;
        cap_b = cap_d + SLAB_SLACK;
        ok = cap_d > 0 && n_a_max + cap_b <= cb && cap_b <= cs && n_a_max + cap_b <= 0xFFFFFFFFll;
    }
    __host__ static int64_t ids_needed(int64_t D, double fraction, int64_t tiles) {
        return (int64_t)((double)(D + 1) * (1.0 + fraction)) + tiles + SLAB_SLACK + 512;
    }
};

constexpr uint32_t EMIT_HEAVY_MIN = 96;
struct Stage2Scratch {
    size_t keys_a, ids_a, sort, heavy_q, total;
    __host__ __device__ explicit Stage2Scratch(int64_t D) {
        size_t o = 0;
        int64_t n = D > 0 ? D : 1;
        keys_a = o; o = align256(o + 4 * (size_t)n);
        ids_a = o;  o = align256(o + 4 * (size_t)n);
        sort = o;   o = align256(o + SortScratch(n).total);
        heavy_q = o; o = align256(o + 4 * ((size_t)n / EMIT_HEAVY_MIN + 66));
        total = o;
    }
};

struct ImageLayout {
    size_t final_T, n_contrib, tile_last, tile_order, open_bits, open_list, total;
    __host__ __device__ ImageLayout(int64_t W, int64_t H) {
        size_t o = 0;
        const size_t tiles = (size_t)((W + TILE - 1) / TILE) * (size_t)((H + TILE - 1) / TILE);
        final_T = o;    o = align256(o + 4 * (size_t)(W * H));
        n_contrib = o;  o = align256(o + 4 * (size_t)(W * H));
        tile_last = o;  o = align256(o + 4 * tiles);
        tile_order = o; o = align256(o + 4 * (tiles + 1));
        open_bits = o;  o = align256(o + 4 * ((tiles + 31) / 32 + 1));
        open_list = o;  o = align256(o + 4 * tiles);
        total = o;
    }
};

__device__ __forceinline__ double wave_sum_f64(double v) {
    for (int off = 32; off > 0; off >>= 1) {
        const unsigned long long u = (unsigned long long)__double_as_longlong(v);
        const unsigned lo = (unsigned)__shfl_xor((int)(unsigned)u, off), hi = (unsigned)__shfl_xor((int)(unsigned)(u >> 32), off);
        v += __longlong_as_double((long long)(((unsigned long long)hi << 32) | lo));
    }
    return v;
}
struct AdamScalars {
    float w1;
    float beta2, w2;
    float bc2_sqrt, eps;
};
inline AdamScalars adam_scalars(int64_t step, double beta1, double beta2, double eps) {
    AdamScalars a;
    a.w1 = (float)(1.0 - beta1);
    a.beta2 = (float)beta2;
    a.w2 = (float)(1.0 - beta2);
    a.bc2_sqrt = (float)sqrt(1.0 - pow(beta2, (double)step));
    a.eps = (float)eps;
    return a;
}
inline float adam_neg_step_size(double lr, int64_t step, double beta1) { return (float)(-(lr / (1.0 - pow(beta1, (double)step)))); }

struct AdamInBackward {
    float* m[6];
    float* v[6];
    float nss[6];
    AdamScalars a;
};

constexpr int CAM_PARTIALS = 27;
constexpr int CAM_ROW = 32;
struct CamPartials {
    double* rows;
};
struct CameraGrads {
    float* dL_dviewmatrix;
    float* dL_dprojmatrix;
    float* dL_dcampos;
    double* rows;
};
size_t camera_grad_rows_bytes(int P);

#if defined(__HIPCC__)

__device__ __forceinline__ void adam_update(float& p, float g, float& m, float& v, float nss, const AdamScalars& a) {
#pragma clang fp contract(off)
    m = __fmaf_rn(a.w1, g - m, m);
    v = __fmaf_rn(a.w2 * g, g, v * a.beta2);
    const float denom = __fsqrt_rn(v) / a.bc2_sqrt + a.eps;
    p = p + (nss * m) / denom;
}

__device__ __forceinline__ bool levelset_hits_rect(float gx, float gy, float A, float Bh, float C,
                                                   float tau2, float x0, float x1, float y0, float y1) {
#pragma clang fp contract(off)
    const float dxlo = __fsub_rn(gx, x1), dxhi = __fsub_rn(gx, x0);
    const float dylo = __fsub_rn(gy, y1), dyhi = __fsub_rn(gy, y0);
    const float cx = fminf(fmaxf(0.0f, dxlo), dxhi);
    const float cy = fminf(fmaxf(0.0f, dylo), dyhi);
    if (cx == 0.0f && cy == 0.0f) return true;
    float fbest = -3.0e38f;
    if (cx != 0.0f) {
        float dy = __fdiv_rn(-__fmul_rn(Bh, cx), C);
        dy = fminf(fmaxf(dy, dylo), dyhi);
        const float u = __fmaf_rn(A, cx, __fmul_rn(Bh, dy)), w = __fmaf_rn(C, dy, __fmul_rn(Bh, cx));
        fbest = fmaxf(fbest, __fmaf_rn(cx, u, __fmul_rn(dy, w)));
    }
    if (cy != 0.0f) {
        float dx = __fdiv_rn(-__fmul_rn(Bh, cy), A);
        dx = fminf(fmaxf(dx, dxlo), dxhi);
        const float u = __fmaf_rn(A, dx, __fmul_rn(Bh, cy)), w = __fmaf_rn(C, cy, __fmul_rn(Bh, dx));
        fbest = fmaxf(fbest, __fmaf_rn(dx, u, __fmul_rn(cy, w)));
    }
    return fbest >= tau2;
}

constexpr float LEVELSET_MARGIN_EMIT = 0.02f;
constexpr float LEVELSET_MARGIN_COUNT = 0.03f;
struct LevelSetRows {
    float A, Bh, C, Atau, det, invA, dymax, dyR;
};
__device__ __forceinline__ LevelSetRows levelset_rows_setup(float A, float Bh, float C, float tau2) {
#pragma clang fp contract(off)
    LevelSetRows r;
    r.A = A; r.Bh = Bh; r.C = C;
    r.det = __fsub_rn(__fmul_rn(A, C), __fmul_rn(Bh, Bh));
    r.Atau = __fmul_rn(A, tau2);
    r.invA = __frcp_rn(A);
    r.dymax = __fsqrt_rn(__fdiv_rn(r.Atau, r.det));
    const float dx_ext = __fsqrt_rn(__fdiv_rn(__fmul_rn(C, tau2), r.det));
    r.dyR = __fdiv_rn(-__fmul_rn(Bh, dx_ext), C);
    return r;
}
__device__ __forceinline__ bool levelset_row_interval(const LevelSetRows& r, float gx, float gy, int ty, int minx,
                                                      int maxx, float margin, int& tlo, int& thi) {
#pragma clang fp contract(off)
    const float y0 = (float)(ty * TILE);
    const float dym = r.dymax + margin;
    const float lo = fmaxf(__fsub_rn(gy, y0 + (float)(TILE - 1)), -dym);
    const float hi = fminf(__fsub_rn(gy, y0), dym);
    if (lo > hi) return false;
    const float dyr = fminf(fmaxf(r.dyR, lo), hi);
    const float dyl = fminf(fmaxf(-r.dyR, lo), hi);
    const float sr = __fsqrt_rn(fmaxf(0.0f, __fmaf_rn(-r.det, __fmul_rn(dyr, dyr), r.Atau)));
    const float sl = __fsqrt_rn(fmaxf(0.0f, __fmaf_rn(-r.det, __fmul_rn(dyl, dyl), r.Atau)));
    const float dx_max = __fmul_rn(__fsub_rn(-__fmul_rn(r.Bh, dyr), sr), r.invA);
    const float dx_min = __fmul_rn(__fadd_rn(-__fmul_rn(r.Bh, dyl), sl), r.invA);
    const float xl = __fsub_rn(__fsub_rn(gx, dx_max), margin);
    const float xr = __fadd_rn(__fsub_rn(gx, dx_min), margin);
    tlo = max(minx, (int)ceilf(__fmul_rn(__fsub_rn(xl, (float)(TILE - 1)), 1.0f / TILE)));
    thi = min(maxx - 1, (int)floorf(__fmul_rn(xr, 1.0f / TILE)));
    return tlo <= thi;
}

template <int CTRL, int ROW_MASK = 0xF, int BANK_MASK = 0xF, bool BOUND = false>
__device__ __forceinline__ float dpp_mov(float v, float old = 0.0f) {
    return __int_as_float(__builtin_amdgcn_update_dpp(__float_as_int(old), __float_as_int(v), CTRL, ROW_MASK,
                                                      BANK_MASK, BOUND));
}
template <int CTRL, int ROW_MASK = 0xF, int BANK_MASK = 0xF, bool BOUND = false>
__device__ __forceinline__ unsigned dpp_mov_u(unsigned v, unsigned old = 0u) {
    return (unsigned)__builtin_amdgcn_update_dpp((int)old, (int)v, CTRL, ROW_MASK, BANK_MASK, BOUND);
}

__device__ __forceinline__ float cross_row_allreduce(float x) {
    typedef unsigned u2 __attribute__((ext_vector_type(2)));
    const u2 a = __builtin_amdgcn_permlane16_swap(__float_as_uint(x), __float_as_uint(x), false, false);
    const float s = __uint_as_float(a.x) + __uint_as_float(a.y);
    const u2 b = __builtin_amdgcn_permlane32_swap(__float_as_uint(s), __float_as_uint(s), false, false);
    return __uint_as_float(b.x) + __uint_as_float(b.y);
}

__device__ __forceinline__ float cross_row_allreduce_bperm(float x, int addr16, int addr32) {
    x += __int_as_float(__builtin_amdgcn_ds_bpermute(addr16, __float_as_int(x)));
    x += __int_as_float(__builtin_amdgcn_ds_bpermute(addr32, __float_as_int(x)));
    return x;
}

__device__ __forceinline__ int lane_bcast(int v, int src) { return __builtin_amdgcn_readlane(v, src); }
__device__ __forceinline__ uint32_t lane_bcast(uint32_t v, int src) { return (uint32_t)__builtin_amdgcn_readlane((int)v, src); }
__device__ __forceinline__ float lane_bcast(float v, int src) {
    return __int_as_float(__builtin_amdgcn_readlane(__float_as_int(v), src));
}

__device__ __forceinline__ float wave_allreduce_sum(float v) {
    v += dpp_mov<0xB1>(v);
    v += dpp_mov<0x4E>(v);
    v += dpp_mov<0x124>(v);
    v += dpp_mov<0x128>(v);
    return cross_row_allreduce(v);
}

__device__ __forceinline__ unsigned wave_max_u32(unsigned v) {
    for (int off = 32; off > 0; off >>= 1) v = max(v, (unsigned)__shfl_xor((int)v, off));
    return v;
}

constexpr int OCC_MAX_BLOCK_ROWS = 256;
constexpr int OCC_LIGHT_RECT = 1024;
__device__ __forceinline__ uint32_t occ_bucket(uint32_t depth_key) {
    const uint32_t kb = depth_key >> OCC_KEY_SHIFT;
    return kb > OCC_KEY_BASE ? min(kb - OCC_KEY_BASE, (uint32_t)(OCC_BUCKETS - 1)) : 0u;
}
struct OccTable {
    uint16_t cut[OCC_MAX_BLOCKS];
    uint16_t rowmax[OCC_MAX_BLOCK_ROWS];
    uint32_t red[2][16];
    uint32_t cut_min, cut_max;
};
__device__ __forceinline__ void occ_table_load(OccTable& t, const uint32_t* __restrict__ occ_cut, int nbx, int nby) {
    const int n = nbx * nby;
    uint32_t lo = 0xFFFFu, hi = 0u;
    for (int q = threadIdx.x; q < n; q += blockDim.x) {
        const uint32_t c = min(occ_cut[q], 0xFFFFu);
        t.cut[q] = (uint16_t)c;
        lo = min(lo, c);
        hi = max(hi, c);
    }
    for (int off = 32; off > 0; off >>= 1) {
        lo = min(lo, (uint32_t)__shfl_xor((int)lo, off));
        hi = max(hi, (uint32_t)__shfl_xor((int)hi, off));
    }
    if ((threadIdx.x & 63) == 0) { t.red[0][threadIdx.x >> 6] = lo; t.red[1][threadIdx.x >> 6] = hi; }
    __syncthreads();
    for (int by = threadIdx.x; by < nby; by += blockDim.x) {
        uint32_t m = 0u;
        for (int bx = 0; bx < nbx; ++bx) m = max(m, (uint32_t)t.cut[by * nbx + bx]);
        t.rowmax[by] = (uint16_t)m;
    }
    if (threadIdx.x == 0) {
        uint32_t a = 0xFFFFu, b = 0u;
        for (int w = 0; w < (int)(blockDim.x + 63) / 64; ++w) { a = min(a, t.red[0][w]); b = max(b, t.red[1][w]); }
        t.cut_min = a;
        t.cut_max = b;
    }
    __syncthreads();
}

#endif

struct ViewParams {
    int W, H, gx, gy;
    float tanfovx, tanfovy, fx, fy;
    float scale_modifier, fade_size;
    int sh_degree, sh_coeffs;
    int filter_small, filter_large;
    const float* bg;
    const float* viewmatrix;
    const float* projmatrix;
    const float* campos;
    int cell_sx, cell_sy;
};

constexpr uint32_t TILE_COUNT_BITS = 20, TILE_COUNT_MASK = (1u << TILE_COUNT_BITS) - 1u;
__host__ __device__ inline uint32_t cell_range_pack(int minx, int miny, int maxx, int maxy, int sx, int sy) {
    return (uint32_t)(minx >> sx) | ((uint32_t)((maxx - 1) >> sx) << 3) | ((uint32_t)(miny >> sy) << 6) | ((uint32_t)((maxy - 1) >> sy) << 9);
}
__host__ __device__ inline uint64_t cell_range_mask(uint32_t packed) {
    const uint32_t c0 = packed & 7u, c1 = (packed >> 3) & 7u, r0 = (packed >> 6) & 7u, r1 = (packed >> 9) & 7u;
    const uint64_t cols = ((2ull << c1) - (1ull << c0)) & 0xFFull;
    uint64_t m = 0;
    for (uint32_t r = r0; r <= r1; ++r) m |= cols << (8u * r);
    return m;
}

inline ViewParams make_view_params(const msgs_view_t* v) {
    ViewParams p;
    p.W = v->image_width; p.H = v->image_height;
    p.gx = (p.W + TILE - 1) / TILE; p.gy = (p.H + TILE - 1) / TILE;
    p.tanfovx = v->tanfovx; p.tanfovy = v->tanfovy;
    p.fx = p.W / (2.0f * v->tanfovx); p.fy = p.H / (2.0f * v->tanfovy);
    p.scale_modifier = v->scale_modifier; p.fade_size = v->fade_size;
    p.sh_degree = v->sh_degree; p.sh_coeffs = v->sh_coeffs;
    p.filter_small = v->filter_small; p.filter_large = v->filter_large;
    p.bg = v->bg; p.viewmatrix = v->viewmatrix; p.projmatrix = v->projmatrix; p.campos = v->campos;
    p.cell_sx = p.cell_sy = -1;
    if ((int64_t)p.gx * p.gy < (int64_t)(1u << TILE_COUNT_BITS)) {
        p.cell_sx = p.cell_sy = 0;
        while ((p.gx + (1 << p.cell_sx) - 1) >> p.cell_sx > 8) ++p.cell_sx;
        while ((p.gy + (1 << p.cell_sy) - 1) >> p.cell_sy > 8) ++p.cell_sy;
    }
    return p;
}

struct ZeroJob { uint32_t* p0; size_t n0; uint32_t* p1; size_t n1; };

hipError_t launch_preprocess(const ViewParams& vp, const msgs_gaussians_t& g, int32_t* radii, float* pixel_sizes,
                             char* geom, hipStream_t s, ZeroJob zj = ZeroJob{nullptr, 0, nullptr, 0},
                             uint32_t* heavy_list = nullptr, uint32_t* heavy_count = nullptr, uint32_t* heavy_blk = nullptr,
                             bool write_litrec = false);
hipError_t launch_occlusion(const ViewParams& vp, int P, char* geom, const uint32_t* heavy_list, const uint32_t* heavy_count,
                            const uint32_t* heavy_blk, OccCand* cand, hipStream_t s);
int set_occlusion(int on);
int get_occlusion();
int occlusion_block_log2(int gx, int gy);
hipError_t launch_preprocess_backward(const ViewParams& vp, const msgs_gaussians_t& g, const int32_t* radii,
                                      const char* geom, const grad_acc_t* grad_rec, const msgs_grads_t& grads,
                                      hipStream_t s, bool textbook = false, bool depth = false,
                                      const CameraGrads* camera = nullptr);
hipError_t launch_blend_forward_literal(const ViewParams& vp, const char* geom, int P, const uint32_t* ids, const uint2* ranges,
                                        float* out_color, float* out_ps, float* out_depth, float* final_T, uint32_t* n_contrib,
                                        uint32_t* order_flag, hipStream_t s);
hipError_t launch_blend_backward_literal(const ViewParams& vp, const char* geom, int P, const uint32_t* ids, const uint2* ranges,
                                         const float* final_T, const uint32_t* n_contrib, const float* dL_dcolor, double* inst_grad,
                                         hipStream_t s, const float* dL_ddepth = nullptr,
                                         const float* dL_dalpha = nullptr);
hipError_t launch_sh_grad_from_views(int P, int n_views, int deg, const float* means3D, const float* campos,
                                     int64_t campos_stride, const float* drgb, int64_t drgb_stride, float scale,
                                     float* d_dc, float* d_rest, hipStream_t s);
hipError_t launch_mark_visible(int P, const float* means3D, const float* viewmatrix, const float* projmatrix,
                               uint8_t* present, hipStream_t s);
hipError_t radix_sort_pairs(uint32_t* keys_in, uint32_t* vals_in, uint32_t* keys_out, uint32_t* vals_out,
                            int64_t n, int begin_bit, int end_bit, char* scratch ,
                            hipStream_t s, bool pre_zeroed = false, uint32_t* n_valid_dev = nullptr,
                            const uint32_t* n_dev = nullptr, bool keys16 = false);
bool radix_sort_keys16_ok(int64_t n, int begin_bit, int end_bit);
bool radix_sort_zero_region(int64_t n, int begin_bit, int end_bit, char* scratch, uint32_t** ptr, size_t* words);
bool radix_sort_supports_device_count(int64_t n, int begin_bit, int end_bit);

hipError_t exclusive_scan_u32(const uint32_t* in, const uint32_t* gather, uint32_t* out, int64_t n,
                              uint64_t* partials , uint64_t* total, hipStream_t s,
                              uint64_t* status = nullptr, uint64_t* host_mapped = nullptr, uint64_t ticket = 0,
                              const uint32_t* n_ptr = nullptr, uint32_t* clamped_total = nullptr, uint64_t clamp = 0,
                              const uint32_t* extra = nullptr,
                              uint32_t* zero_word = nullptr,
                              uint32_t* overflow_flag = nullptr, uint32_t in_mask = 0xFFFFFFFFu, uint32_t* side_out = nullptr,
                              uint32_t* side_flag = nullptr);
template <class F>
inline void with_bool(bool b, F&& f) {
    if (b) f(std::true_type{}); else f(std::false_type{});
}
hipError_t launch_zero(void* ptr, size_t bytes, hipStream_t s);
hipError_t launch_emit(const ViewParams& vp, int P, const char* geom, uint32_t* keys, uint32_t* ids,
                       int64_t D, hipStream_t s, ZeroJob zj = ZeroJob{nullptr, 0, nullptr, 0}, const uint32_t* D_dev = nullptr,
                       bool keys16 = false, uint32_t* heavy_q = nullptr, int slab = 0, const uint32_t* open_bits = nullptr,
                       int64_t density_D = 0);
hipError_t launch_slab_split(int P, char* geom, int64_t D, const uint32_t* D_dev, float fraction, uint32_t* open_bits,
                             int num_tiles, hipStream_t s);
hipError_t launch_slab_recount(const ViewParams& vp, int P, char* geom, const uint32_t* open_bits, const uint32_t* open_list, int64_t D,
                               const uint32_t* D_dev, hipStream_t s);
hipError_t launch_ranges(const uint32_t* keys, int64_t D, uint2* ranges, int num_tiles, hipStream_t s,
                         bool pre_zeroed = false, const uint32_t* D_dev = nullptr, bool keys16 = false, uint32_t base = 0);
int set_backward_generation(int gen);
int set_blend_granularity(int mode);
struct DetScratch {
    size_t grad_rec, inst_grad, keys, keys_s, entry, sort, total;
    DetScratch(int64_t P, int64_t D, int nf = DET_INST_FLOATS);
};
hipError_t launch_blend_backward_det(const ViewParams& vp, int P, const char* geom, const uint32_t* ids, int64_t D,
                                     const uint2* ranges, const float* final_T, const uint32_t* n_contrib,
                                     const float* dL_dcolor, char* scratch, hipStream_t s, const float* dL_ddepth = nullptr,
                                     const float* dL_dalpha = nullptr);

hipError_t launch_alpha_map(const float* final_T, float* out_alpha, size_t N, hipStream_t s);
size_t bg_grad_rows_bytes(size_t N);
hipError_t launch_bg_grad(const float* final_T , const float* dL_dcolor, size_t N, float* dL_dbg,
                          double* rows, hipStream_t s);

hipError_t launch_adam(const msgs_adam_tensor_t* tensors, int n, int64_t step, double beta1, double beta2, double eps,
                       hipStream_t s);
hipError_t launch_densify_stats(const msgs_densify_stats_t& d, hipStream_t s);

size_t densify_scratch_bytes(int64_t P, int64_t n_append);
int densify_check_select(const msgs_densify_select_t& s);
int densify_check_apply(const msgs_densify_apply_t& a);
int densify_select(const msgs_densify_select_t& s, char* scratch, int64_t* counts_host, hipStream_t st);
int densify_apply(const msgs_densify_apply_t& a, const char* scratch, hipStream_t st);

size_t loss_scratch_bytes(int C, int H, int W);
void ssim_window_host(float w[11]);
hipError_t launch_loss_forward(const float* img, const float* gt, int C, int H, int W, float lambda, float* out3,
                               char* scratch, int write_maps, hipStream_t s);
hipError_t launch_loss_backward(const float* img, const float* gt, int C, int H, int W, float lambda,
                                const float* upstream, const char* scratch, float* dL_dimg, hipStream_t s);

size_t knn_scratch_bytes(int64_t P);
hipError_t knn_mean_dist2(const float* points, int64_t P, float* mean_dist2, char* scratch, hipStream_t s);

size_t voxel_pool_scratch_bytes(int64_t M);
hipError_t voxel_pool_build(const float* positions, int64_t M, float voxel_size, uint32_t* order, uint32_t* seg_start,
                            int32_t* voxel_index, char* scratch, int64_t* num_voxels_host, hipStream_t s);
hipError_t voxel_pool_average(const float* features, int F, const uint32_t* order, const uint32_t* seg_start,
                              int64_t Mv, float* out, hipStream_t s);
struct FwdSlabArgs {
    int pass;
    uint32_t* open_bits;
    uint32_t* open_list;
    uint32_t* n_open;
    unsigned long long* dtrav;
};
hipError_t launch_blend_forward(const ViewParams& vp, const char* geom, const uint32_t* ids, const uint2* ranges,
                                float* out_color, float* out_ps, float* out_depth, float* final_T,
                                uint32_t* n_contrib, uint32_t* tile_last, void* clear_ptr, size_t clear_bytes, hipStream_t s,
                                const FwdSlabArgs* slab = nullptr);
bool forward_uses_quadrant_kernel(int tiles);
hipError_t launch_forward_feedback(const unsigned long long* dtrav, const SlabHeader* hdr, int slab_mode, int64_t D,
                                   const uint32_t* D_dev, uint32_t tag, uint64_t ticket, uint64_t* host_mapped, hipStream_t s);
hipError_t launch_blend_backward(const ViewParams& vp, const char* geom, const uint32_t* ids, const uint2* ranges,
                                 const float* final_T, const uint32_t* n_contrib, const float* dL_dcolor,
                                 grad_acc_t* grad_rec, hipStream_t s, const uint32_t* tile_order = nullptr,
                                 const float* dL_ddepth = nullptr,
                                 const float* dL_dalpha = nullptr);
hipError_t launch_blend_absgrad(const ViewParams& vp, int P, const char* geom, const uint32_t* ids, const uint2* ranges,
                                const float* final_T, const uint32_t* n_contrib, const float* dL_dcolor, const float* dL_ddepth,
                                const float* dL_dalpha, double* acc, float* out, hipStream_t s);
constexpr size_t CONTRIB_ACC_BYTES = 24;
hipError_t launch_blend_contrib(const ViewParams& vp, const char* geom, const uint32_t* ids, const uint2* ranges,
                                const float* final_T, const uint32_t* n_contrib, const float* pixel_weights, void* acc,
                                hipStream_t s);
hipError_t launch_contrib_finish(int P, const void* acc, float* weight_sum, float* weight_max, int64_t* pixel_count, hipStream_t s);
size_t features_scratch_bytes(int P);
hipError_t launch_blend_features_forward(const ViewParams& vp, const char* geom, const uint32_t* ids, const uint2* ranges,
                                         const float* final_T, const uint32_t* n_contrib, const float* features, int C,
                                         float* out, hipStream_t s);
hipError_t launch_blend_features_backward(const ViewParams& vp, int P, const char* geom, const uint32_t* ids, const uint2* ranges,
                                          const float* final_T, const uint32_t* n_contrib, const float* features, int C,
                                          const float* dL_dF, grad_acc_t* grad_rec, double* acc, float* dL_dfeatures,
                                          hipStream_t s);
hipError_t launch_blend_distortion_forward(const ViewParams& vp, const char* geom, const uint32_t* ids, const uint2* ranges,
                                           const float* final_T, const uint32_t* n_contrib, float* out_distortion,
                                           float* out_moment, hipStream_t s);
hipError_t launch_blend_distortion_backward(const ViewParams& vp, const char* geom, const uint32_t* ids, const uint2* ranges,
                                            const float* final_T, const uint32_t* n_contrib, const float* moment,
                                            const float* dL_ddist, grad_acc_t* grad_rec, hipStream_t s);
size_t screen_compensation_rows_bytes(int P);
hipError_t launch_screen_compensation_forward(const ViewParams& vp, const msgs_gaussians_t& g, float* o_eff, hipStream_t s);
hipError_t launch_screen_compensation_backward(const ViewParams& vp, const msgs_gaussians_t& g, const float* dL_do_eff,
                                               float* dL_dopacity, float* dL_dmeans3D, float* dL_dscales, float* dL_drotations,
                                               float* dL_dcov3D, float* dL_dV, double* rows, hipStream_t s);
hipError_t launch_blend_median_depth_forward(const ViewParams& vp, const char* geom, const uint32_t* ids, const uint2* ranges,
                                             const uint32_t* n_contrib, float* out_depth, int32_t* out_id, hipStream_t s);
hipError_t launch_median_depth_backward(const ViewParams& vp, int P, const int32_t* median_id, const float* dL_dmedian,
                                        grad_acc_t* grad_rec, hipStream_t s);
hipError_t launch_tile_order(const ViewParams& vp, const uint32_t* tile_last, uint32_t* tile_order, hipStream_t s);
hipError_t launch_blend_lane_stats(const ViewParams& vp, const char* geom, const uint32_t* ids, const uint2* ranges,
                                   unsigned long long* out3 , hipStream_t s);
hipError_t launch_blend_backward_lane_stats(const ViewParams& vp, const char* geom, const uint32_t* ids, const uint2* ranges,
                                            const float* final_T, const uint32_t* n_contrib,
                                            unsigned long long* out4 , hipStream_t s);
hipError_t launch_binning_stats(const ViewParams& vp, int P, const int32_t* radii, const uint32_t* n_contrib,
                                unsigned long long* out2 , hipStream_t s);

}
```

### ms-gs_amd/csrc/sort.hip

```cpp
#include "msgs_internal.h"

#include <algorithm>

namespace msgs {

namespace {

__device__ __forceinline__ uint32_t wave_inclusive_scan(uint32_t v, int lane) {
#pragma unroll
    for (int off = 1; off < 64; off <<= 1) {
        const uint32_t n = (uint32_t)__shfl_up((int)v, off);
        if (lane >= off) v += n;
    }
    return v;
}

__device__ __forceinline__ uint32_t block_exclusive_scan(uint32_t v, uint32_t* s_wave , uint32_t* total) {
    const int lane = threadIdx.x & 63, w = threadIdx.x >> 6;
    const uint32_t inc = wave_inclusive_scan(v, lane);
    if (lane == 63) s_wave[w] = inc;
    __syncthreads();
    uint32_t base = 0;
#pragma unroll
    for (int k = 0; k < 4; ++k) {
        const uint32_t t = s_wave[k];
        if (k < w) base += t;
    }
    *total = s_wave[0] + s_wave[1] + s_wave[2] + s_wave[3];
    __syncthreads();
    return base + inc - v;
}

__device__ __forceinline__ uint64_t block_sum_u64(uint64_t v, uint64_t* s_sum ) {
    for (int off = 32; off > 0; off >>= 1)
        v += ((uint64_t)(uint32_t)__shfl_xor((int)(uint32_t)(v >> 32), off) << 32) | (uint32_t)__shfl_xor((int)(uint32_t)v, off);
    if ((threadIdx.x & 63) == 0) s_sum[threadIdx.x >> 6] = v;
    __syncthreads();
    return s_sum[0] + s_sum[1] + s_sum[2] + s_sum[3];
}

__device__ __forceinline__ void scan_load_items(const uint32_t* in, int64_t base, int64_t n, uint32_t v[SCAN_ITEMS]) {
    static_assert(SCAN_ITEMS % 4 == 0, "uint4 runs");
    if (base + SCAN_ITEMS <= n && (reinterpret_cast<uintptr_t>(in + base) & 15) == 0) {
#pragma unroll
        for (int q = 0; q < SCAN_ITEMS / 4; ++q) {
            const uint4 a = *reinterpret_cast<const uint4*>(in + base + 4 * q);
            v[4 * q] = a.x; v[4 * q + 1] = a.y; v[4 * q + 2] = a.z; v[4 * q + 3] = a.w;
        }
    } else {
#pragma unroll
        for (int k = 0; k < SCAN_ITEMS; ++k) v[k] = base + k < n ? in[base + k] : 0u;
    }
}
__device__ __forceinline__ void scan_store_items(uint32_t* out, int64_t base, int64_t n, const uint32_t v[SCAN_ITEMS]) {
    if (base + SCAN_ITEMS <= n && (reinterpret_cast<uintptr_t>(out + base) & 15) == 0) {
#pragma unroll
        for (int q = 0; q < SCAN_ITEMS / 4; ++q)
            *reinterpret_cast<uint4*>(out + base + 4 * q) = make_uint4(v[4 * q], v[4 * q + 1], v[4 * q + 2], v[4 * q + 3]);
    } else {
#pragma unroll
        for (int k = 0; k < SCAN_ITEMS; ++k) if (base + k < n) out[base + k] = v[k];
    }
}

__global__ __launch_bounds__(SCAN_THREADS) void scan_reduce_kernel(const uint32_t* __restrict__ in,
                                                                   const uint32_t* __restrict__ gather,
                                                                   int64_t n, uint64_t* __restrict__ partials,
                                                                   uint32_t* __restrict__ staged,
                                                                   const uint32_t* __restrict__ n_ptr, uint32_t in_mask,
                                                                   uint32_t* __restrict__ side_out, uint32_t* __restrict__ side_flag) {
    __shared__ uint64_t s_sum[4];
    if (n_ptr) n = (int64_t)*n_ptr;
    if (side_flag && blockIdx.x == 0 && threadIdx.x == 0) *side_flag = side_out ? 1u : 0u;
    const int64_t base = (int64_t)blockIdx.x * SCAN_CHUNK + (int64_t)threadIdx.x * SCAN_ITEMS;
    uint32_t v[SCAN_ITEMS];
    if (gather) {
        uint32_t g[SCAN_ITEMS];
        scan_load_items(gather, base, n, g);
#pragma unroll
        for (int k = 0; k < SCAN_ITEMS; ++k) v[k] = base + k < n ? in[g[k]] : 0u;
        if (side_out) {
#pragma unroll
            for (int k = 0; k < SCAN_ITEMS; ++k) g[k] = v[k] >> TILE_COUNT_BITS;
            scan_store_items(side_out, base, n, g);
        }
#pragma unroll
        for (int k = 0; k < SCAN_ITEMS; ++k) v[k] &= in_mask;
        if (staged) scan_store_items(staged, base, n, v);
    } else {
        scan_load_items(in, base, n, v);
    }
    uint64_t sum = 0;
#pragma unroll
    for (int k = 0; k < SCAN_ITEMS; ++k) sum += v[k];
    const uint64_t total = block_sum_u64(sum, s_sum);
    if (threadIdx.x == 0) partials[blockIdx.x] = total;
}

__global__ __launch_bounds__(SCAN_THREADS) void scan_apply_fused_kernel(const uint32_t* in, uint32_t* out, int64_t n,
                                                                        const uint64_t* __restrict__ partials, int64_t nb,
                                                                        const uint32_t* __restrict__ n_ptr,
                                                                        uint64_t* __restrict__ total_out,
                                                                        uint64_t* __restrict__ status,
                                                                        volatile uint64_t* host, uint64_t ticket,
                                                                        uint32_t* __restrict__ clamped_total, uint64_t clamp,
                                                                        const uint32_t* __restrict__ extra,
                                                                        uint32_t* __restrict__ zero_word,
                                                                        uint32_t* __restrict__ overflow_flag) {
    __shared__ uint32_t s_wave[4];
    __shared__ uint64_t s_sum[4];
    if (n_ptr) n = (int64_t)*n_ptr;
    const int64_t chunk0 = (int64_t)blockIdx.x * SCAN_CHUNK;
    if (blockIdx.x != 0 && chunk0 >= n) return;
    const int64_t upto = blockIdx.x == 0 ? nb : (int64_t)blockIdx.x;
    uint64_t acc = 0;
    for (int64_t q = threadIdx.x; q < upto; q += SCAN_THREADS) acc += partials[q];
    const uint64_t sum = block_sum_u64(acc, s_sum);
    uint64_t base = sum;
    if (blockIdx.x == 0) {
        base = 0;
        if (threadIdx.x == 0) {
            if (total_out) *total_out = sum;
            if (zero_word) *zero_word = 0u;
            if (clamped_total) *clamped_total = (uint32_t)(sum < clamp ? sum : clamp);
            if (overflow_flag && sum > clamp) *overflow_flag = 1u;
            const uint64_t info = extra ? ((uint64_t)extra[0] | ((uint64_t)extra[1] << 32)) : 0ull;
            if (status) { status[0] = sum; status[1] = 0; status[2] = info; }
            if (host) {
                host[0] = sum;
                host[1] = 0;
                host[3] = info;
                __threadfence_system();
                host[2] = ticket;
            }
        }
        if (chunk0 >= n) return;
    }
    const int64_t tb = chunk0 + (int64_t)threadIdx.x * SCAN_ITEMS;
    uint32_t v[SCAN_ITEMS];
    scan_load_items(in, tb, n, v);
    uint32_t tsum = 0;
#pragma unroll
    for (int k = 0; k < SCAN_ITEMS; ++k) tsum += v[k];
    uint32_t total;
    uint32_t run = block_exclusive_scan(tsum, s_wave, &total) + (uint32_t)base;
#pragma unroll
    for (int k = 0; k < SCAN_ITEMS; ++k) {
        const uint32_t x = v[k];
        v[k] = run;
        run += x;
    }
    scan_store_items(out, tb, n, v);
}

template <int ITEMS = SORT_ITEMS>
__device__ __forceinline__ int64_t elem_index(int64_t chunk_base, int w, int r, int lane) {
    return chunk_base + (int64_t)w * (64 * ITEMS) + r * 64 + lane;
}

template <int ITEMS, bool DROP = false, typename KeyT = uint32_t>
__global__ __launch_bounds__(SORT_THREADS) void radix_hist_kernel(const KeyT* __restrict__ keys, int64_t n,
                                                                  int shift, uint32_t mask, int64_t nblocks,
                                                                  uint32_t* __restrict__ hist,
                                                                  uint32_t* __restrict__ gsum, int gsize, int ngroups,
                                                                  const uint32_t* __restrict__ n_ptr = nullptr) {
    __shared__ uint32_t s_hist[256];
    const int64_t chunk_base = (int64_t)blockIdx.x * (SORT_THREADS * ITEMS);
    if (n_ptr) {
        n = (int64_t)*n_ptr;
        if (chunk_base >= n) return;
    }
    s_hist[threadIdx.x] = 0;
    __syncthreads();
    const int lane = threadIdx.x & 63, w = threadIdx.x >> 6;
    constexpr int KPV = 16 / (int)sizeof(KeyT);
    if (ITEMS % KPV == 0 && chunk_base + (int64_t)SORT_THREADS * ITEMS <= n) {
        const uint4* kv = reinterpret_cast<const uint4*>(keys + chunk_base);
#pragma unroll
        for (int r = 0; r < ITEMS / KPV; ++r) {
            const uint4 v = kv[r * SORT_THREADS + threadIdx.x];
            const uint32_t w4[4] = {v.x, v.y, v.z, v.w};
#pragma unroll
            for (int j = 0; j < KPV; ++j) {
                const uint32_t k = sizeof(KeyT) == 4 ? w4[j] : ((w4[j >> 1] >> ((j & 1) * 16)) & 0xFFFFu);
                if (!DROP || k != 0xFFFFFFFFu) atomicAdd(&s_hist[(k >> shift) & mask], 1u);
            }
        }
    } else {
#pragma unroll
        for (int r = 0; r < ITEMS; ++r) {
            const int64_t i = elem_index<ITEMS>(chunk_base, w, r, lane);
            if (i < n) {
                const uint32_t k = (uint32_t)keys[i];
                if (!DROP || k != 0xFFFFFFFFu) atomicAdd(&s_hist[(k >> shift) & mask], 1u);
            }
        }
    }
    __syncthreads();
    const uint32_t c = s_hist[threadIdx.x];
    hist[(int64_t)blockIdx.x * 256 + threadIdx.x] = c;
    if (c) atomicAdd(&gsum[(int64_t)(blockIdx.x / gsize) * 256 + threadIdx.x], c);
}

__global__ __launch_bounds__(256) void group_scan_kernel(uint32_t* __restrict__ gsum, int ngroups,
                                                         uint32_t* __restrict__ hist, int gsize, int64_t nblocks,
                                                         const uint32_t* __restrict__ n_ptr, int chunk) {
    if (n_ptr) {
        const int64_t n = (int64_t)*n_ptr;
        nblocks = (n + chunk - 1) / chunk;
        ngroups = (int)((nblocks + gsize - 1) / gsize);
        if ((int)blockIdx.x > ngroups) return;
        if (nblocks == 0) return;
    }
    const int d = threadIdx.x;
    if ((int)blockIdx.x < ngroups) {
        const int64_t first = (int64_t)blockIdx.x * gsize;
        const int rows = (int)min((int64_t)gsize, nblocks - first);
        uint32_t* q = hist + first * 256 + d;
        uint32_t run = 0;
#pragma unroll 8
        for (int k = 0; k < rows; ++k) {
            const uint32_t v = q[(int64_t)k * 256];
            q[(int64_t)k * 256] = run;
            run += v;
        }
        return;
    }
    __shared__ uint32_t s_wv[4];
    uint32_t tot = 0;
#pragma unroll 8
    for (int k = 0; k < ngroups; ++k) tot += gsum[(int64_t)k * 256 + d];
    uint32_t dummy;
    uint32_t run = block_exclusive_scan(tot, s_wv, &dummy);
#pragma unroll 8
    for (int k = 0; k < ngroups; ++k) {
        uint32_t* q = &gsum[(int64_t)k * 256 + d];
        const uint32_t v = *q;
        *q = run;
        run += v;
    }
}

template <int ITEMS, bool DROP = false, typename KeyT = uint32_t>
__global__ __launch_bounds__(SORT_THREADS) void radix_scatter_kernel(const KeyT* __restrict__ keys_in,
                                                                     const uint32_t* __restrict__ vals_in,
                                                                     KeyT* __restrict__ keys_out,
                                                                     uint32_t* __restrict__ vals_out, int64_t n,
                                                                     int shift, uint32_t mask, int64_t nblocks,
                                                                     const uint32_t* __restrict__ hist_scanned,
                                                                     const uint32_t* __restrict__ gsum, int gsize,
                                                                     int ngroups, bool gsum_is_base = false,
                                                                     const uint32_t* __restrict__ n_ptr = nullptr,
                                                                     uint32_t* __restrict__ n_out = nullptr) {
    __shared__ uint32_t s_cnt[4][256];
    __shared__ uint32_t s_wave[4];
    const int lane = threadIdx.x & 63, w = threadIdx.x >> 6;
    const int64_t chunk_base = (int64_t)blockIdx.x * (SORT_THREADS * ITEMS);
    if (n_ptr) {
        n = (int64_t)*n_ptr;
        if (chunk_base >= n) return;
    }
#pragma unroll
    for (int k = 0; k < 4; ++k) s_cnt[k][threadIdx.x] = 0;
    __syncthreads();

    uint32_t key[ITEMS], val[ITEMS], rank[ITEMS];
    const uint64_t lt_mask = (1ull << lane) - 1ull;
#pragma unroll
    for (int r = 0; r < ITEMS; ++r) {
        const int64_t i = elem_index<ITEMS>(chunk_base, w, r, lane);
        key[r] = i < n ? (uint32_t)keys_in[i] : 0xFFFFFFFFu;
        const bool valid = i < n && (!DROP || key[r] != 0xFFFFFFFFu);
        val[r] = valid ? (vals_in ? vals_in[i] : (uint32_t)i) : 0u;
        const uint32_t d = (key[r] >> shift) & mask;
        uint64_t peers = __ballot(valid);
#pragma unroll
        for (int b = 0; b < 8; ++b) {
            const uint64_t m = __ballot((d >> b) & 1u);
            peers &= ((d >> b) & 1u) ? m : ~m;
        }
        const uint32_t prev = s_cnt[w][d];
        const uint32_t before = (uint32_t)__popcll(peers & lt_mask);
        rank[r] = prev + before;
        if (valid && before == 0) s_cnt[w][d] = prev + (uint32_t)__popcll(peers);
    }
    __syncthreads();
    uint32_t gbase;
    {
        const uint32_t d = threadIdx.x;
        if (gsum_is_base) {
            const int g = blockIdx.x / gsize;
            gbase = gsum[(int64_t)g * 256 + d] + hist_scanned[(int64_t)blockIdx.x * 256 + d];
        } else {
            const int g = blockIdx.x / gsize;
            uint32_t tot = 0, before = 0;
#pragma unroll 8
            for (int k = 0; k < ngroups; ++k) {
                const uint32_t v = gsum[(int64_t)k * 256 + d];
                tot += v;
                before += k < g ? v : 0u;
            }
            const int nin = (int)(blockIdx.x - (int64_t)g * gsize);
            const uint32_t* hrow = hist_scanned + ((int64_t)g * gsize) * 256 + d;
#pragma unroll 8
            for (int k = 0; k < nin; ++k) before += hrow[(int64_t)k * 256];
            uint32_t total;
            gbase = block_exclusive_scan(tot, s_wave, &total) + before;
            if (n_out && blockIdx.x == 0 && threadIdx.x == 0) *n_out = total;
        }
    }
    __shared__ uint32_t s_key[SORT_THREADS * ITEMS], s_val[SORT_THREADS * ITEMS], s_delta[256];
    uint32_t nkept;
    {
        const uint32_t d = threadIdx.x;
        uint32_t c[4], ltot = 0;
#pragma unroll
        for (int k = 0; k < 4; ++k) { c[k] = s_cnt[k][d]; ltot += c[k]; }
        const uint32_t lbase = block_exclusive_scan(ltot, s_wave, &nkept);
        uint32_t run = lbase;
#pragma unroll
        for (int k = 0; k < 4; ++k) { s_cnt[k][d] = run; run += c[k]; }
        s_delta[d] = gbase - lbase;
    }
    __syncthreads();
#pragma unroll
    for (int r = 0; r < ITEMS; ++r) {
        const int64_t i = elem_index<ITEMS>(chunk_base, w, r, lane);
        if (i < n && (!DROP || key[r] != 0xFFFFFFFFu)) {
            const uint32_t lp = s_cnt[w][(key[r] >> shift) & mask] + rank[r];
            s_key[lp] = key[r];
            s_val[lp] = val[r];
        }
    }
    __syncthreads();
    const int nvalid = DROP ? (int)nkept : (int)min((int64_t)(SORT_THREADS * ITEMS), n - chunk_base);
#pragma unroll
    for (int r = 0; r < ITEMS; ++r) {
        const int j = r * SORT_THREADS + threadIdx.x;
        if (j < nvalid) {
            const uint32_t k = s_key[j];
            const uint32_t pos = (uint32_t)j + s_delta[(k >> shift) & mask];
            keys_out[pos] = (KeyT)k;
            vals_out[pos] = s_val[j];
        }
    }
}

}

hipError_t exclusive_scan_u32(const uint32_t* in, const uint32_t* gather, uint32_t* out, int64_t n,
                              uint64_t* partials, uint64_t* total, hipStream_t s, uint64_t* status,
                              uint64_t* host_mapped, uint64_t ticket, const uint32_t* n_ptr, uint32_t* clamped_total,
                              uint64_t clamp, const uint32_t* extra, uint32_t* zero_word, uint32_t* overflow_flag,
                              uint32_t in_mask, uint32_t* side_out, uint32_t* side_flag) {
    if ((in_mask != 0xFFFFFFFFu || side_out) && gather == nullptr) return hipErrorInvalidValue;
    if (n <= 0) {
        hipLaunchKernelGGL(scan_apply_fused_kernel, dim3(1), dim3(SCAN_THREADS), 0, s, in, out, (int64_t)0,
                           (const uint64_t*)partials, (int64_t)0, (const uint32_t*)nullptr, total, status,
                           (volatile uint64_t*)host_mapped, ticket, clamped_total, clamp, extra, zero_word, overflow_flag);
        return hipGetLastError();
    }
    if (gather != nullptr && out == in) return hipErrorInvalidValue;
    const int64_t nb = scan_blocks(n);
    const bool stage = gather != nullptr;
    hipLaunchKernelGGL(scan_reduce_kernel, dim3((unsigned)nb), dim3(SCAN_THREADS), 0, s, in, gather, n, partials,
                       stage ? out : (uint32_t*)nullptr, n_ptr, in_mask, side_out, side_flag);
    hipLaunchKernelGGL(scan_apply_fused_kernel, dim3((unsigned)nb), dim3(SCAN_THREADS), 0, s,
                       stage ? (const uint32_t*)out : in, out, n, (const uint64_t*)partials, nb, n_ptr, total, status,
                       (volatile uint64_t*)host_mapped, ticket, clamped_total, clamp, extra, zero_word, overflow_flag);
    return hipGetLastError();
}

namespace {
__global__ __launch_bounds__(256) void zero_kernel(uint32_t* __restrict__ p, size_t n_words) {
    const size_t n4 = n_words >> 2;
    uint4* p4 = reinterpret_cast<uint4*>(p);
    for (size_t i = (size_t)blockIdx.x * blockDim.x + threadIdx.x; i < n4; i += (size_t)gridDim.x * blockDim.x)
        p4[i] = make_uint4(0u, 0u, 0u, 0u);
    if (blockIdx.x == 0 && threadIdx.x < (n_words & 3)) p[(n4 << 2) + threadIdx.x] = 0u;
}
}

hipError_t launch_zero(void* ptr, size_t bytes, hipStream_t s) {
    if (bytes == 0) return hipSuccess;
    if ((reinterpret_cast<uintptr_t>(ptr) & 15) || (bytes & 3)) return hipMemsetAsync(ptr, 0, bytes, s);
    const size_t words = bytes >> 2;
    size_t blocks = (words / 4 + 255) / 256;
    if (blocks < 1) blocks = 1;
    if (blocks > 2048) blocks = 2048;
    hipLaunchKernelGGL(zero_kernel, dim3((unsigned)blocks), dim3(256), 0, s, (uint32_t*)ptr, words);
    return hipGetLastError();
}

static int passes_for(int begin_bit, int end_bit) {
    const int passes = (end_bit - begin_bit + 7) / 8;
    return passes < 1 ? 1 : passes;
}
typedef SortGeom GroupGeom;

bool radix_sort_supports_device_count(int64_t n, int begin_bit, int end_bit) {
    return n > 0 && passes_for(begin_bit, end_bit) <= 4;
}

bool radix_sort_keys16_ok(int64_t n, int begin_bit, int end_bit) {
    return end_bit <= 16 && radix_sort_supports_device_count(n, begin_bit, end_bit);
}

bool radix_sort_zero_region(int64_t n, int begin_bit, int end_bit, char* scratch, uint32_t** ptr, size_t* words) {
    if (n <= 0) return false;
    const int passes = passes_for(begin_bit, end_bit);
    if (passes > 4) return false;
    const GroupGeom G(n);
    const SortScratch L(n);
    *ptr = reinterpret_cast<uint32_t*>(scratch + L.hist) + (size_t)256 * G.nb;
    *words = G.zero_words(passes);
    return true;
}

namespace {
__global__ void store_u32_kernel(uint32_t* p, uint32_t v) { *p = v; }

template <int ITEMS, typename KeyT>
void launch_pass(const KeyT* src_k, const uint32_t* src_v, KeyT* dst_k, uint32_t* dst_v, int64_t n, int shift, uint32_t mask,
                 const GroupGeom& G, uint32_t* hist, uint32_t* gs, bool drop, const uint32_t* n_ptr, uint32_t* n_out,
                 hipStream_t s) {
    const dim3 grid((unsigned)G.nb), block(SORT_THREADS);
    if (drop) {
        hipLaunchKernelGGL((radix_hist_kernel<ITEMS, true, KeyT>), grid, block, 0, s, src_k, n, shift, mask, G.nb, hist, gs, G.gsize,
                           G.ngroups, (const uint32_t*)nullptr);
        hipLaunchKernelGGL((radix_scatter_kernel<ITEMS, true, KeyT>), grid, block, 0, s, src_k, src_v, dst_k, dst_v, n, shift,
                           mask, G.nb, hist, gs, G.gsize, G.ngroups, false, (const uint32_t*)nullptr, n_out);
        return;
    }
    hipLaunchKernelGGL((radix_hist_kernel<ITEMS, false, KeyT>), grid, block, 0, s, src_k, n, shift, mask, G.nb, hist, gs, G.gsize,
                       G.ngroups, n_ptr);
    if (G.scanned)
        hipLaunchKernelGGL(group_scan_kernel, dim3((unsigned)G.ngroups + 1), dim3(256), 0, s, gs, G.ngroups, hist, G.gsize, G.nb, n_ptr,
                           SORT_THREADS * ITEMS);
    hipLaunchKernelGGL((radix_scatter_kernel<ITEMS, false, KeyT>), grid, block, 0, s, src_k, src_v, dst_k, dst_v, n, shift, mask,
                       G.nb, hist, gs, G.gsize, G.ngroups, G.scanned, n_ptr, (uint32_t*)nullptr);
}

template <typename KeyT>
hipError_t sort_passes(KeyT* keys_in, uint32_t* vals_in, KeyT* keys_out, uint32_t* vals_out, int64_t n, int passes,
                       int begin_bit, int end_bit, const GroupGeom& G, KeyT* keys_alt, uint32_t* vals_alt, uint32_t* hist,
                       uint32_t* gsum_all, bool compact, uint32_t* n_valid_dev, const uint32_t* n_dev, hipStream_t s) {
    const KeyT* src_k = keys_in;
    const uint32_t* src_v = vals_in;
    int next_shift = begin_bit;
    for (int p = 0; p < passes; ++p) {
        const int shift = next_shift;
        const int left = end_bit - shift;
        const int bits = (left + (passes - p) - 1) / (passes - p);
        next_shift = shift + bits;
        const uint32_t mask = bits >= 8 ? 0xFFu : ((1u << (bits > 0 ? bits : 1)) - 1u);
        const bool to_out = ((passes - 1 - p) % 2) == 0;
        KeyT* dst_k = to_out ? keys_out : keys_alt;
        uint32_t* dst_v = to_out ? vals_out : vals_alt;
        uint32_t* gs = gsum_all + (size_t)p * 256 * G.ngroups;
        const bool drop = compact && p == 0;
        const uint32_t* np = n_dev ? n_dev : (compact && p > 0 ? n_valid_dev : nullptr);
        uint32_t* no = drop ? n_valid_dev : nullptr;
        if (G.big) launch_pass<16, KeyT>(src_k, src_v, dst_k, dst_v, n, shift, mask, G, hist, gs, drop, np, no, s);
        else if (G.mid) launch_pass<8, KeyT>(src_k, src_v, dst_k, dst_v, n, shift, mask, G, hist, gs, drop, np, no, s);
        else launch_pass<SORT_ITEMS, KeyT>(src_k, src_v, dst_k, dst_v, n, shift, mask, G, hist, gs, drop, np, no, s);
        src_k = dst_k;
        src_v = dst_v;
    }
    return hipGetLastError();
}
}

hipError_t radix_sort_pairs(uint32_t* keys_in, uint32_t* vals_in, uint32_t* keys_out, uint32_t* vals_out,
                            int64_t n, int begin_bit, int end_bit, char* scratch, hipStream_t s, bool pre_zeroed,
                            uint32_t* n_valid_dev, const uint32_t* n_dev, bool keys16) {
    if (n <= 0) {
        if (n_valid_dev) hipLaunchKernelGGL(store_u32_kernel, dim3(1), dim3(1), 0, s, n_valid_dev, 0u);
        return hipSuccess;
    }
    const int passes = passes_for(begin_bit, end_bit);
    if (passes > 4) return hipErrorInvalidValue;
    const SortScratch L(n);
    uint32_t* keys_alt = reinterpret_cast<uint32_t*>(scratch + L.keys_alt);
    uint32_t* vals_alt = reinterpret_cast<uint32_t*>(scratch + L.vals_alt);
    uint32_t* hist = reinterpret_cast<uint32_t*>(scratch + L.hist);
    const GroupGeom G(n);
    uint32_t* gsum_all = hist + (size_t)256 * G.nb;
    if (!pre_zeroed) {
        hipError_t e = launch_zero(gsum_all, sizeof(uint32_t) * G.zero_words(passes), s);
        if (e != hipSuccess) return e;
    }
    if (keys16) {
        if (n_valid_dev || end_bit > 16) return hipErrorInvalidValue;
        return sort_passes<uint16_t>(reinterpret_cast<uint16_t*>(keys_in), vals_in, reinterpret_cast<uint16_t*>(keys_out), vals_out,
                                     n, passes, begin_bit, end_bit, G, reinterpret_cast<uint16_t*>(keys_alt), vals_alt, hist,
                                     gsum_all, false, nullptr, n_dev, s);
    }
    const bool compact = n_valid_dev != nullptr && !G.scanned;
    if (n_valid_dev && !compact) hipLaunchKernelGGL(store_u32_kernel, dim3(1), dim3(1), 0, s, n_valid_dev, (uint32_t)n);
    return sort_passes<uint32_t>(keys_in, vals_in, keys_out, vals_out, n, passes, begin_bit, end_bit, G, keys_alt, vals_alt, hist,
                                 gsum_all, compact, n_valid_dev, n_dev, s);
}

}
```

### ms-gs_amd/diff_gaussian_rasterization/_backend.py

```python
import ctypes as C
import os
import threading

import torch

_PKG = os.path.dirname(os.path.abspath(__file__))
_LIB_PATH = os.environ.get("MSGS_HIP_LIB") or next(
    (p for p in (os.path.join(_PKG, "libmsgs_hip.so"),) if os.path.exists(p)),
    os.path.join(os.path.dirname(_PKG), "lib", "libmsgs_hip.so"))

ABI_VERSION = 11

K_NAMES = ("preprocess", "depth_sort", "scan", "emit", "tile_sort", "ranges", "blend_fwd", "blend_bwd",
           "preprocess_bwd", "slab_b")
K_COUNT = len(K_NAMES)


class View(C.Structure):
    _fields_ = [("image_height", C.c_int32), ("image_width", C.c_int32),
                ("tanfovx", C.c_float), ("tanfovy", C.c_float),
                ("scale_modifier", C.c_float), ("fade_size", C.c_float),
                ("sh_degree", C.c_int32), ("sh_coeffs", C.c_int32),
                ("filter_small", C.c_int32), ("filter_large", C.c_int32),
                ("prefiltered", C.c_int32), ("debug", C.c_int32),
                ("no_heavy_queue", C.c_int32), ("feedback_tag", C.c_int32),
                ("slab_fraction", C.c_float), ("reserved1", C.c_int32),
                ("bg", C.c_void_p), ("viewmatrix", C.c_void_p),
                ("projmatrix", C.c_void_p), ("campos", C.c_void_p)]


class Gaussians(C.Structure):
    _fields_ = [("P", C.c_int32), ("raw_params", C.c_int32),
                ("means3D", C.c_void_p), ("shs", C.c_void_p), ("colors_precomp", C.c_void_p),
                ("opacities", C.c_void_p), ("scales", C.c_void_p), ("rotations", C.c_void_p),
                ("cov3D_precomp", C.c_void_p), ("max_pixel_sizes", C.c_void_p),
                ("min_pixel_sizes", C.c_void_p), ("occ_multiplier", C.c_void_p),
                ("dc_delta", C.c_void_p), ("base_mask", C.c_void_p),
                ("features_dc", C.c_void_p), ("features_rest", C.c_void_p),
                ("rotations_raw", C.c_void_p)]


class Grads(C.Structure):
    _fields_ = [("dL_dmeans3D", C.c_void_p), ("dL_dmeans2D", C.c_void_p), ("dL_dshs", C.c_void_p),
                ("dL_dcolors", C.c_void_p), ("dL_dopacities", C.c_void_p), ("dL_dscales", C.c_void_p),
                ("dL_drotations", C.c_void_p), ("dL_dcov3D", C.c_void_p),
                ("dL_dfeatures_dc", C.c_void_p), ("dL_dfeatures_rest", C.c_void_p), ("factors_ready", C.c_void_p),
                ("scratch_is_clear", C.c_int32), ("accumulate", C.c_int32),
                ("wait_before_accumulate", C.c_void_p), ("accumulated", C.c_void_p), ("adam_in_backward", C.c_void_p)]


class AdamMoments(C.Structure):
    _fields_ = [("exp_avg", C.c_void_p), ("exp_avg_sq", C.c_void_p), ("lr", C.c_double)]


class AdamInBackward(C.Structure):
    _fields_ = [("step", C.c_int64), ("beta1", C.c_double), ("beta2", C.c_double), ("eps", C.c_double), ("t", AdamMoments * 6)]


class AdamTensor(C.Structure):
    _fields_ = [("param", C.c_void_p), ("grad", C.c_void_p), ("exp_avg", C.c_void_p), ("exp_avg_sq", C.c_void_p),
                ("n", C.c_int64), ("lr", C.c_double)]


ADAM_MAX_TENSORS = 8
STATS_BASE_MASK, STATS_PIXEL_SIZES, STATS_DENSIFY = 1, 2, 4


class DensifyStats(C.Structure):
    _fields_ = [("P", C.c_int32), ("flags", C.c_int32), ("reso_lvl", C.c_int32), ("reso_lvls", C.c_int32),
                ("radii", C.c_void_p), ("pixel_sizes", C.c_void_p), ("means2D_grad", C.c_void_p),
                ("target_reso_lvl", C.c_void_p), ("xyz_gradient_accum", C.c_void_p), ("denom", C.c_void_p),
                ("max_radii2D", C.c_void_p), ("max_pixel_sizes", C.c_void_p), ("min_pixel_sizes", C.c_void_p),
                ("base_mask", C.c_void_p)]


DENSIFY_PRUNE, DENSIFY_GROW, DENSIFY_PRUNE_MASK, DENSIFY_APPEND = 0, 1, 2, 3
(DR_COPY, DR_ZERO, DR_COPY_CLEAR_COL, DR_SPLIT_XYZ, DR_SPLIT_SCALE, DR_SPLIT_DIV, DR_GROW_OPACITY, DR_GROW_SCALE, DR_GROW_MUL,
 DR_CONST, DR_APPEND) = range(11)
DENSIFY_MAX_TENSORS = 32


class DensifySelect(C.Structure):
    _fields_ = [("mode", C.c_int32), ("reso_lvl", C.c_int32), ("reso_lvls", C.c_int32), ("has_max_screen_size", C.c_int32),
                ("P", C.c_int64), ("n_append", C.c_int64),
                ("grad_threshold", C.c_float), ("min_opacity", C.c_float), ("scale_limit", C.c_float),
                ("big_world_limit", C.c_float), ("max_screen_size", C.c_float), ("reserved", C.c_int32),
                ("opacity", C.c_void_p), ("scaling", C.c_void_p), ("xyz_gradient_accum", C.c_void_p), ("denom", C.c_void_p),
                ("target_reso_lvl", C.c_void_p), ("prune_mask", C.c_void_p)]


class DensifyTensor(C.Structure):
    _fields_ = [("dst", C.c_void_p), ("src", C.c_void_p), ("append_src", C.c_void_p), ("constant", C.c_int64),
                ("width", C.c_int32), ("elem_bytes", C.c_int32), ("rule", C.c_uint8 * 8)]


class DensifyApply(C.Structure):
    _fields_ = [("P", C.c_int64), ("n_append", C.c_int64), ("P_out", C.c_int64), ("n_split", C.c_int64),
                ("n_tensors", C.c_int32), ("reso_lvl", C.c_int32),
                ("xyz", C.c_void_p), ("scaling", C.c_void_p), ("rotation", C.c_void_p), ("draws", C.c_void_p),
                ("tensors", C.POINTER(DensifyTensor))]


class Timing(C.Structure):
    _fields_ = [("ev", C.c_void_p * (2 * K_COUNT))]


def _load():
    if not os.path.exists(_LIB_PATH):
        raise ImportError(
            f"diff_gaussian_rasterization: HIP library not found at {_LIB_PATH}. Build it with "
            f"`make -C {os.path.dirname(_PKG)}` (hipcc --offload-arch=gfx950). There is no fallback path.")
    lib = C.CDLL(_LIB_PATH)
    sz = C.c_size_t
    vp = C.c_void_p
    lib.msgs_abi_version.restype = C.c_int
    lib.msgs_error_string.restype = C.c_char_p
    lib.msgs_error_string.argtypes = [C.c_int]
    for name, args in (("msgs_geom_bytes", [C.c_int32]), ("msgs_stage1_scratch_bytes", [C.c_int32]),
                       ("msgs_binning_bytes", [C.c_int64, C.c_int32, C.c_int32]),
                       ("msgs_stage2_scratch_bytes", [C.c_int64, C.c_int32, C.c_int32]),
                       ("msgs_image_bytes", [C.c_int32, C.c_int32]),
                       ("msgs_binning_bytes_slab", [C.c_int64, C.c_int32, C.c_int32, C.c_float]),
                       ("msgs_stage2_scratch_bytes_slab", [C.c_int64, C.c_int32, C.c_int32]),
                       ("msgs_backward_scratch_bytes", [C.c_int32])):
        f = getattr(lib, name)
        f.restype = sz
        f.argtypes = args
    lib.msgs_forward_stage1.restype = C.c_int
    lib.msgs_forward_stage1.argtypes = [C.POINTER(View), C.POINTER(Gaussians), vp, vp, vp, sz, vp, sz,
                                        C.POINTER(C.c_int64), C.POINTER(Timing), vp]
    lib.msgs_set_deterministic.restype = C.c_int
    lib.msgs_set_deterministic.argtypes = [C.c_int32]
    lib.msgs_get_deterministic.restype = C.c_int
    lib.msgs_get_deterministic.argtypes = []
    lib.msgs_backward_scratch_bytes_deterministic.restype = sz
    lib.msgs_backward_scratch_bytes_deterministic.argtypes = [C.c_int32, C.c_int64]
    lib.msgs_backward_scratch_bytes_deterministic_depth.restype = sz
    lib.msgs_backward_scratch_bytes_deterministic_depth.argtypes = [C.c_int32, C.c_int64]
    lib.msgs_set_backward_generation.restype = C.c_int
    lib.msgs_set_backward_generation.argtypes = [C.c_int32]
    lib.msgs_set_blend_granularity.restype = C.c_int
    lib.msgs_set_blend_granularity.argtypes = [C.c_int32]
    lib.msgs_forward_info.restype = C.c_int
    lib.msgs_forward_info.argtypes = [C.POINTER(C.c_int64)]
    lib.msgs_set_occlusion.restype = C.c_int
    lib.msgs_set_occlusion.argtypes = [C.c_int32]
    lib.msgs_occlusion_stats.restype = C.c_int
    lib.msgs_occlusion_stats.argtypes = [vp, sz, C.c_int32, C.POINTER(C.c_int64), vp]
    lib.msgs_slab_stats.restype = C.c_int
    lib.msgs_slab_stats.argtypes = [vp, sz, C.c_int32, C.POINTER(C.c_int64), vp]
    lib.msgs_forward.restype = C.c_int
    lib.msgs_forward.argtypes = [C.POINTER(View), C.POINTER(Gaussians), vp, vp, vp, sz, vp, sz, vp, sz, vp, sz, vp, sz,
                                 vp, vp, vp, vp, sz, C.c_int32, C.POINTER(C.c_int64), C.POINTER(C.c_int32), C.POINTER(Timing), vp]
    lib.msgs_status_create.restype = C.c_int
    lib.msgs_status_create.argtypes = [C.POINTER(vp)]
    lib.msgs_status_destroy.restype = C.c_int
    lib.msgs_status_destroy.argtypes = [vp]
    lib.msgs_forward_launch.restype = C.c_int
    lib.msgs_forward_launch.argtypes = [C.POINTER(View), C.POINTER(Gaussians), vp, vp, vp, sz, vp, sz, vp, sz, vp, sz, vp, sz,
                                        vp, vp, vp, vp, sz, C.c_int32, vp, C.POINTER(Timing), vp]
    lib.msgs_forward_finish.restype = C.c_int
    lib.msgs_forward_finish.argtypes = [vp, C.POINTER(C.c_int64), C.POINTER(C.c_int32)]
    lib.msgs_preprocess_only.restype = C.c_int
    lib.msgs_preprocess_only.argtypes = [C.POINTER(View), C.POINTER(Gaussians), vp, vp, vp, sz, vp]
    lib.msgs_forward_stage2.restype = C.c_int
    lib.msgs_forward_stage2.argtypes = [C.POINTER(View), C.POINTER(Gaussians), vp, sz, C.c_int64, vp, sz, vp, sz,
                                        vp, sz, vp, vp, vp, vp, sz, C.c_int32, C.POINTER(Timing), vp]
    lib.msgs_backward.restype = C.c_int
    lib.msgs_backward.argtypes = [C.POINTER(View), C.POINTER(Gaussians), vp, vp, sz, C.c_int64, vp, sz, vp, sz,
                                  vp, vp, sz, C.POINTER(Grads), C.POINTER(Timing), vp]
    lib.msgs_backward_with_depth.restype = C.c_int
    lib.msgs_backward_with_depth.argtypes = [C.POINTER(View), C.POINTER(Gaussians), vp, vp, sz, C.c_int64, vp, sz, vp, sz,
                                             vp, vp, vp, sz, C.POINTER(Grads), C.POINTER(Timing), vp]
    lib.msgs_backward_with_camera.restype = C.c_int
    lib.msgs_backward_with_camera.argtypes = [C.POINTER(View), C.POINTER(Gaussians), vp, vp, sz, C.c_int64, vp, sz, vp, sz,
                                              vp, vp, vp, sz, C.POINTER(Grads), vp, vp, vp, vp, sz, C.POINTER(Timing), vp]
    lib.msgs_camera_grad_scratch_bytes.restype = sz
    lib.msgs_camera_grad_scratch_bytes.argtypes = [C.c_int32]
    lib.msgs_alpha_map.restype = C.c_int
    lib.msgs_alpha_map.argtypes = [C.POINTER(View), vp, sz, vp, vp]
    lib.msgs_backward_with_alpha.restype = C.c_int
    lib.msgs_backward_with_alpha.argtypes = [C.POINTER(View), C.POINTER(Gaussians), vp, vp, sz, C.c_int64, vp, sz, vp, sz,
                                             vp, vp, vp, vp, sz, C.POINTER(Grads), vp, vp, vp, vp, sz, C.POINTER(Timing), vp]
    lib.msgs_bg_grad_scratch_bytes.restype = sz
    lib.msgs_bg_grad_scratch_bytes.argtypes = [C.c_int32, C.c_int32]
    lib.msgs_bg_grad.restype = C.c_int
    lib.msgs_bg_grad.argtypes = [C.POINTER(View), vp, sz, vp, vp, vp, sz, vp]
    lib.msgs_absgrad_scratch_bytes.restype = sz
    lib.msgs_absgrad_scratch_bytes.argtypes = [C.c_int32]
    lib.msgs_absgrad.restype = C.c_int
    lib.msgs_absgrad.argtypes = [C.POINTER(View), C.c_int32, vp, sz, C.c_int64, vp, sz, vp, sz, vp, vp, vp, vp, sz, vp, vp]
    lib.msgs_contrib_scratch_bytes.restype = sz
    lib.msgs_contrib_scratch_bytes.argtypes = [C.c_int32]
    lib.msgs_contrib_accumulate.restype = C.c_int
    lib.msgs_contrib_accumulate.argtypes = [C.POINTER(View), C.c_int32, vp, sz, C.c_int64, vp, sz, vp, sz, vp, vp, sz, C.c_int32, vp]
    lib.msgs_contrib_finish.restype = C.c_int
    lib.msgs_contrib_finish.argtypes = [C.c_int32, vp, sz, vp, vp, vp, vp]
    lib.msgs_features_scratch_bytes.restype = sz
    lib.msgs_features_scratch_bytes.argtypes = [C.c_int32, C.c_int32]
    lib.msgs_features_forward.restype = C.c_int
    lib.msgs_features_forward.argtypes = [C.POINTER(View), C.c_int32, vp, sz, C.c_int64, vp, sz, vp, sz, vp, C.c_int32, vp, vp]
    lib.msgs_features_backward.restype = C.c_int
    lib.msgs_features_backward.argtypes = [C.POINTER(View), C.c_int32, vp, sz, C.c_int64, vp, sz, vp, sz, vp, C.c_int32, vp,
                                           vp, sz, vp, sz, vp, vp]
    lib.msgs_distortion_forward.restype = C.c_int
    lib.msgs_distortion_forward.argtypes = [C.POINTER(View), C.c_int32, vp, sz, C.c_int64, vp, sz, vp, sz, vp, vp, vp]
    lib.msgs_distortion_backward.restype = C.c_int
    lib.msgs_distortion_backward.argtypes = [C.POINTER(View), C.c_int32, vp, sz, C.c_int64, vp, sz, vp, sz, vp, vp, vp, sz, vp]
    lib.msgs_median_depth_forward.restype = C.c_int
    lib.msgs_median_depth_forward.argtypes = [C.POINTER(View), C.c_int32, vp, sz, C.c_int64, vp, sz, vp, sz, vp, vp, vp]
    lib.msgs_median_depth_backward.restype = C.c_int
    lib.msgs_median_depth_backward.argtypes = [C.POINTER(View), C.c_int32, vp, vp, vp, sz, vp]
    lib.msgs_screen_compensation_scratch_bytes.restype = sz
    lib.msgs_screen_compensation_scratch_bytes.argtypes = [C.c_int32]
    lib.msgs_screen_compensation_forward.restype = C.c_int
    lib.msgs_screen_compensation_forward.argtypes = [C.POINTER(View), C.POINTER(Gaussians), vp, vp]
    lib.msgs_screen_compensation_backward.restype = C.c_int
    lib.msgs_screen_compensation_backward.argtypes = [C.POINTER(View), C.POINTER(Gaussians), vp, vp, vp, vp, vp, vp, vp, vp, sz, vp]
    lib.msgs_backward_per_gaussian.restype = C.c_int
    lib.msgs_backward_per_gaussian.argtypes = [C.POINTER(View), C.POINTER(Gaussians), vp, vp, sz, vp, C.POINTER(Grads), vp]
    lib.msgs_sh_grad_from_views.restype = C.c_int
    lib.msgs_sh_grad_from_views.argtypes = [C.c_int32, C.c_int32, C.c_int32, vp, vp, C.c_int64, vp, C.c_int64,
                                                C.c_float, vp, vp, vp]
    lib.msgs_mark_visible.restype = C.c_int
    lib.msgs_mark_visible.argtypes = [C.c_int32, vp, vp, vp, vp, vp]
    lib.msgs_binning_stats.restype = C.c_int
    lib.msgs_binning_stats.argtypes = [C.POINTER(View), C.c_int32, vp, vp, sz, vp, sz, vp, sz,
                                       C.POINTER(C.c_int64), vp]
    lib.msgs_blend_lane_stats.restype = C.c_int
    lib.msgs_blend_lane_stats.argtypes = [C.POINTER(View), vp, sz, C.c_int32, C.c_int64, vp, sz, vp, sz, vp, sz,
                                          C.POINTER(C.c_int64), vp]
    lib.msgs_voxel_pool_scratch_bytes.restype = sz
    lib.msgs_voxel_pool_scratch_bytes.argtypes = [C.c_int64]
    lib.msgs_voxel_pool_build.restype = C.c_int
    lib.msgs_voxel_pool_build.argtypes = [vp, C.c_int64, C.c_float, vp, vp, vp, vp, sz, C.POINTER(C.c_int64), vp]
    lib.msgs_voxel_pool_average.restype = C.c_int
    lib.msgs_voxel_pool_average.argtypes = [vp, C.c_int32, vp, vp, C.c_int64, vp, vp]
    lib.msgs_adam_step.restype = C.c_int
    lib.msgs_adam_step.argtypes = [C.POINTER(AdamTensor), C.c_int32, C.c_int64, C.c_double, C.c_double, C.c_double, vp]
    lib.msgs_densify_stats.restype = C.c_int
    lib.msgs_densify_stats.argtypes = [C.POINTER(DensifyStats), vp]
    lib.msgs_densify_scratch_bytes.restype = sz
    lib.msgs_densify_scratch_bytes.argtypes = [C.c_int64, C.c_int64]
    lib.msgs_densify_select.restype = C.c_int
    lib.msgs_densify_select.argtypes = [C.POINTER(DensifySelect), vp, sz, C.POINTER(C.c_int64), vp]
    lib.msgs_densify_apply.restype = C.c_int
    lib.msgs_densify_apply.argtypes = [C.POINTER(DensifyApply), vp, sz, vp]
    lib.msgs_loss_scratch_bytes.restype = sz
    lib.msgs_loss_scratch_bytes.argtypes = [C.c_int32, C.c_int32, C.c_int32]
    lib.msgs_loss_forward.restype = C.c_int
    lib.msgs_loss_forward.argtypes = [vp, vp, C.c_int32, C.c_int32, C.c_int32, C.c_float, vp, vp, sz, C.c_int32, vp]
    lib.msgs_loss_backward.restype = C.c_int
    lib.msgs_loss_backward.argtypes = [vp, vp, C.c_int32, C.c_int32, C.c_int32, C.c_float, vp, vp, sz, vp, vp]
    lib.msgs_knn_scratch_bytes.restype = sz
    lib.msgs_knn_scratch_bytes.argtypes = [C.c_int64]
    lib.msgs_dist2_knn3.restype = C.c_int
    lib.msgs_dist2_knn3.argtypes = [vp, C.c_int64, vp, vp, sz, vp]
    lib.msgs_ssim_window.restype = C.c_int
    lib.msgs_ssim_window.argtypes = [C.POINTER(C.c_float)]
    for name in ("msgs_timing_create", "msgs_timing_destroy"):
        f = getattr(lib, name)
        f.restype = C.c_int
        f.argtypes = [C.POINTER(Timing)]
    lib.msgs_timing_read.restype = C.c_int
    lib.msgs_timing_read.argtypes = [C.POINTER(Timing), C.POINTER(C.c_float)]
    got = lib.msgs_abi_version()
    if got != ABI_VERSION:
        raise ImportError(f"libmsgs_hip.so ABI version {got} != expected {ABI_VERSION}; rebuild the library")
    return lib


lib = _load()

EXPORTS = ("msgs_abi_version", "msgs_error_string", "msgs_geom_bytes", "msgs_stage1_scratch_bytes",
           "msgs_binning_bytes", "msgs_stage2_scratch_bytes", "msgs_image_bytes", "msgs_backward_scratch_bytes",
           "msgs_forward_stage1", "msgs_forward_stage2", "msgs_backward", "msgs_mark_visible",
           "msgs_binning_stats", "msgs_timing_create", "msgs_timing_destroy", "msgs_timing_read",
           "msgs_voxel_pool_scratch_bytes", "msgs_voxel_pool_build", "msgs_voxel_pool_average", "msgs_adam_step",
           "msgs_densify_stats", "msgs_loss_scratch_bytes", "msgs_loss_forward", "msgs_loss_backward",
           "msgs_ssim_window", "msgs_preprocess_only", "msgs_knn_scratch_bytes",
           "msgs_dist2_knn3", "msgs_forward", "msgs_set_deterministic",
           "msgs_get_deterministic", "msgs_backward_scratch_bytes_deterministic",
           "msgs_set_backward_generation", "msgs_set_blend_granularity", "msgs_sh_grad_from_views",
           "msgs_blend_lane_stats", "msgs_backward_per_gaussian",
           "msgs_status_create", "msgs_status_destroy", "msgs_forward_launch", "msgs_forward_finish",
           "msgs_set_occlusion", "msgs_occlusion_stats", "msgs_forward_info", "msgs_binning_bytes_slab",
           "msgs_stage2_scratch_bytes_slab", "msgs_slab_stats", "msgs_backward_with_depth",
           "msgs_backward_scratch_bytes_deterministic_depth", "msgs_backward_with_camera", "msgs_camera_grad_scratch_bytes",
           "msgs_densify_scratch_bytes", "msgs_densify_select", "msgs_densify_apply",
           "msgs_alpha_map", "msgs_backward_with_alpha", "msgs_bg_grad_scratch_bytes", "msgs_bg_grad",
           "msgs_absgrad_scratch_bytes", "msgs_absgrad",
           "msgs_contrib_scratch_bytes", "msgs_contrib_accumulate", "msgs_contrib_finish",
           "msgs_features_scratch_bytes", "msgs_features_forward", "msgs_features_backward",
           "msgs_distortion_forward", "msgs_distortion_backward",
           "msgs_median_depth_forward", "msgs_median_depth_backward",
           "msgs_screen_compensation_forward", "msgs_screen_compensation_backward", "msgs_screen_compensation_scratch_bytes")


def check(rc, where):
    if rc == 0:
        return
    msg = lib.msgs_error_string(int(rc)).decode()
    if rc in (-1, -4):
        raise ValueError(f"{where}: {msg}")
    raise RuntimeError(f"{where}: error {rc}: {msg}")


class KernelTimer:

    def __init__(self, only=None):
        self.t = Timing()
        check(lib.msgs_timing_create(C.byref(self.t)), "msgs_timing_create")
        self.active = self.t
        if only is not None:
            self.active = Timing()
            for k, name in enumerate(K_NAMES):
                if name in only:
                    self.active.ev[2 * k], self.active.ev[2 * k + 1] = self.t.ev[2 * k], self.t.ev[2 * k + 1]

    def read_ms(self):
        out = (C.c_float * K_COUNT)()
        check(lib.msgs_timing_read(C.byref(self.active), out), "msgs_timing_read")
        return {K_NAMES[k]: float(out[k]) for k in range(K_COUNT)}

    def __del__(self):
        try:
            lib.msgs_timing_destroy(C.byref(self.t))
        except Exception:
            pass


_timer_lock = threading.Lock()
_active_timer = None


def set_timer(timer):
    global _active_timer
    with _timer_lock:
        _active_timer = timer


def timer_ptr():
    t = _active_timer
    return C.byref(t.active) if t is not None else None
```

Measured before the change: 1973.

## Replace 32-bit radix depth sort with histogram-bucketed split plus per-bucket LDS sort

Replaces the full 4-pass LSD radix sort of per-Gaussian depth keys with a bucket sort. A fine histogram over float-key bins is used to split the keys into 255 balanced buckets, one scatter pass distributes them, and each bucket is then sorted in LDS by a single block. The aim is to cut global memory passes over the keys from four round trips to roughly one. The trade-off is extra histogram and split kernels, and a slow fallback path when a bucket exceeds LDS capacity. It is on by default for P up to 1.5M.

```diff
diff --git a/__graft_entry__.py b/__graft_entry__.py
--- a/__graft_entry__.py
+++ b/__graft_entry__.py
@@ -23,6 +23,8 @@
     lib = os.path.join(PKG, "lib", "libmsgs_hip.so")
     assert os.path.exists(lib), lib
     harness = os.path.join(PKG, "build", "libmsgs_sort_harness.so")
+    assert os.path.exists(harness), harness
+    harness = os.path.join(PKG, "build", "libmsgs_depth_sort_harness.so")
     assert os.path.exists(harness), harness
     print("built", lib)
 
diff --git a/include/msgs.h b/include/msgs.h
--- a/include/msgs.h
+++ b/include/msgs.h
@@ -288,6 +288,8 @@
 int msgs_set_blend_granularity(int32_t mode);
 
 int msgs_set_occlusion(int32_t on);
+int msgs_set_depth_sort(int32_t mode);
+int msgs_depth_sort_stats(const void* geom, size_t geom_bytes, int32_t P, int64_t* out_host, void* stream);
 int msgs_forward_info(int64_t* out_host);
 int msgs_occlusion_stats(const void* geom, size_t geom_bytes, int32_t P, int64_t* out_host, void* stream);
 int msgs_slab_stats(const void* geom, size_t geom_bytes, int32_t P, int64_t* out_host, void* stream);
diff --git a/ms-gs_amd/csrc/api.hip b/ms-gs_amd/csrc/api.hip
--- a/ms-gs_amd/csrc/api.hip
+++ b/ms-gs_amd/csrc/api.hip
@@ -113,6 +113,7 @@
 int msgs_set_backward_generation(int32_t gen) { return set_backward_generation(gen); }
 int msgs_set_blend_granularity(int32_t mode) { return set_blend_granularity(mode); }
 int msgs_set_occlusion(int32_t on) { return set_occlusion(on); }
+int msgs_set_depth_sort(int32_t mode) { return set_depth_sort(mode); }
 
 }
 
@@ -207,7 +208,9 @@
     const Timer tm{timing, s};
 
     ZeroJob zj1{nullptr, 0, (uint32_t*)(geom + GL.slab_hdr), (GL.occ_hdr - GL.slab_hdr) / 4 + sizeof(OccHeader) / 4 + 2 * (size_t)OCC_BUCKETS};
-    const bool sort1_prezeroed = radix_sort_zero_region(P, 0, 32, scratch + SL.sort, &zj1.p0, &zj1.n0);
+    const bool sort1_buckets = depth_sort_uses_buckets(P);
+    const bool sort1_prezeroed = sort1_buckets ? depth_sort_zero_region(P, scratch + SL.sort, &zj1.p0, &zj1.n0)
+                                               : radix_sort_zero_region(P, 0, 32, scratch + SL.sort, &zj1.p0, &zj1.n0);
     const bool occlusion = get_occlusion() != 0;
     uint32_t* heavy_list = occlusion ? (uint32_t*)(scratch + SL.heavy_list) : nullptr;
     uint32_t* heavy_count = occlusion ? (uint32_t*)(scratch + SL.heavy_count) : nullptr;
@@ -228,9 +231,14 @@
     uint32_t* heavy_q_word = spec ? (uint32_t*)((char*)spec->buf.scratch2 + Stage2Scratch(spec->capacity).heavy_q) : nullptr;
 
     tm.begin(MSGS_K_DEPTH_SORT);
-    HIP_TRY(radix_sort_pairs((uint32_t*)(geom + GL.key), nullptr, (uint32_t*)(geom + GL.skey),
-                             (uint32_t*)(geom + GL.order), P, 0, 32, scratch + SL.sort, s, sort1_prezeroed,
-                             (uint32_t*)(geom + GL.nvalid)));
+    if (sort1_buckets)
+        HIP_TRY(depth_sort_buckets((const uint32_t*)(geom + GL.key), (uint32_t*)(geom + GL.skey), (uint32_t*)(geom + GL.order), P,
+                                   scratch + SL.sort, s, sort1_prezeroed, (uint32_t*)(geom + GL.nvalid),
+                                   (uint32_t*)(geom + GL.slab_hdr + DEPTH_SORT_INFO_OFFSET)));
+    else
+        HIP_TRY(radix_sort_pairs((uint32_t*)(geom + GL.key), nullptr, (uint32_t*)(geom + GL.skey),
+                                 (uint32_t*)(geom + GL.order), P, 0, 32, scratch + SL.sort, s, sort1_prezeroed,
+                                 (uint32_t*)(geom + GL.nvalid)));
     tm.end(MSGS_K_DEPTH_SORT);
     if ((rc = debug_sync(view, s))) return rc;
     tm.begin(MSGS_K_SCAN);
@@ -1163,6 +1171,22 @@
     return MSGS_OK;
 }
 
+int msgs_depth_sort_stats(const void* geom_v, size_t geom_bytes, int32_t P, int64_t* out_host, void* stream) {
+    if (!geom_v || !out_host || P <= 0) return MSGS_ERR_INVALID_ARG;
+    if (geom_bytes < msgs_geom_bytes(P)) return MSGS_ERR_CAPACITY;
+    static_assert(sizeof(SlabHeader) <= DEPTH_SORT_INFO_OFFSET && DEPTH_SORT_INFO_OFFSET + 8 <= 256, "inside the slab header's slot");
+    const GeomLayout GL(P);
+    uint32_t info[2], V;
+    hipStream_t s = (hipStream_t)stream;
+    HIP_TRY(hipMemcpyAsync(info, (const char*)geom_v + GL.slab_hdr + DEPTH_SORT_INFO_OFFSET, sizeof(info), hipMemcpyDeviceToHost, s));
+    HIP_TRY(hipMemcpyAsync(&V, (const char*)geom_v + GL.nvalid, sizeof(V), hipMemcpyDeviceToHost, s));
+    HIP_TRY(hipStreamSynchronize(s));
+    out_host[0] = info[0];
+    out_host[1] = info[1];
+    out_host[2] = V;
+    return MSGS_OK;
+}
+
 int msgs_occlusion_stats(const void* geom_v, size_t geom_bytes, int32_t P, int64_t* out_host, void* stream) {
     if (!geom_v || !out_host || P <= 0) return MSGS_ERR_INVALID_ARG;
     if (geom_bytes < msgs_geom_bytes(P)) return MSGS_ERR_CAPACITY;
diff --git a/ms-gs_amd/csrc/msgs_internal.h b/ms-gs_amd/csrc/msgs_internal.h
--- a/ms-gs_amd/csrc/msgs_internal.h
+++ b/ms-gs_amd/csrc/msgs_internal.h
@@ -141,13 +141,54 @@
     }
 };
 
+constexpr int DEPTH_BIN_SHIFT = 14;
+constexpr uint32_t DEPTH_BIN_LO = 0x3E400000u >> DEPTH_BIN_SHIFT;
+constexpr int DEPTH_COARSE = 261;
+constexpr int DEPTH_BINS = DEPTH_COARSE * 256;
+static_assert(DEPTH_BIN_LO + DEPTH_BINS - 1 == (0x7F7FFFFFu >> DEPTH_BIN_SHIFT), "the top bin is the one of FLT_MAX");
+constexpr int DEPTH_BUCKETS = 255;
+constexpr int DEPTH_LDS_THREADS = 1024;
+constexpr int DEPTH_LDS_ITEMS = 8;
+constexpr int DEPTH_LDS_CAP = DEPTH_LDS_THREADS * DEPTH_LDS_ITEMS;
+constexpr int64_t DEPTH_BUCKET_MAX_P = 1'500'000;
+constexpr size_t DEPTH_SORT_INFO_OFFSET = 64;
+
+__host__ __device__ inline uint32_t depth_bin(uint32_t key) {
+    uint32_t b = key >> DEPTH_BIN_SHIFT;
+    b = b < DEPTH_BIN_LO ? DEPTH_BIN_LO : b;
+    b -= DEPTH_BIN_LO;
+    return b < (uint32_t)DEPTH_BINS ? b : (uint32_t)DEPTH_BINS - 1u;
+}
+
+constexpr int DEPTH_HIST_KEYS = 32768;
+constexpr int DEPTH_HIST_MAX_BLOCKS = 64;
+constexpr int64_t DEPTH_BUCKET_HARD_MAX = (int64_t)DEPTH_HIST_KEYS * DEPTH_HIST_MAX_BLOCKS;
+__host__ __device__ inline int depth_hist_blocks(int64_t n) {
+    const int64_t b = (n + DEPTH_HIST_KEYS - 1) / DEPTH_HIST_KEYS;
+    return b < 1 ? 1 : (b > DEPTH_HIST_MAX_BLOCKS ? DEPTH_HIST_MAX_BLOCKS : (int)b);
+}
+
+struct DepthSortScratch {
+    size_t sort, coarse, map, bases, slices, total;
+    __host__ __device__ explicit DepthSortScratch(int64_t n) {
+        size_t o = 0;
+        sort = o;   o = align256(o + SortScratch(n).total);
+        coarse = o; o = align256(o + 4 * (size_t)DEPTH_COARSE);
+        map = o;    o = align256(o + (size_t)DEPTH_BINS);
+        bases = o;  o = align256(o + 4 * (size_t)(DEPTH_BUCKETS + 2 + 2));
+        slices = o; o = align256(o + 2 * (size_t)DEPTH_BINS * depth_hist_blocks(n));
+        total = o;
+    }
+    __host__ __device__ size_t zero_end() const { return coarse + 4 * (size_t)DEPTH_COARSE; }
+};
+
 struct Stage1Scratch {
     size_t sort, scan_partials, total_out, heavy_list, heavy_count, heavy_blk, occ_cand, total;
     __host__ __device__ explicit Stage1Scratch(int64_t P) {
         size_t o = 0;
         const size_t Pn = (size_t)(P > 0 ? P : 1);
         const size_t waves = 4 * ((Pn + 255) / 256);
-        sort = o;          o = align256(o + SortScratch(P).total);
+        sort = o;          o = align256(o + DepthSortScratch(P).total);
         scan_partials = o; o = align256(o + 8 * (size_t)(scan_blocks(P > 0 ? P : 1) + 2));
         total_out = o;     o = align256(o + 64);
         heavy_list = o;    o = align256(o + 8 * 64 * waves);
@@ -500,6 +541,14 @@
 bool radix_sort_keys16_ok(int64_t n, int begin_bit, int end_bit);
 bool radix_sort_zero_region(int64_t n, int begin_bit, int end_bit, char* scratch, uint32_t** ptr, size_t* words);
 bool radix_sort_supports_device_count(int64_t n, int begin_bit, int end_bit);
+
+hipError_t depth_sort_buckets(const uint32_t* keys_in, uint32_t* keys_out, uint32_t* vals_out, int64_t n,
+                              char* scratch , hipStream_t s, bool pre_zeroed, uint32_t* n_valid_dev,
+                              uint32_t* info = nullptr);
+bool depth_sort_zero_region(int64_t n, char* scratch, uint32_t** ptr, size_t* words);
+bool depth_sort_uses_buckets(int64_t n);
+int set_depth_sort(int mode);
+int get_depth_sort();
 
 hipError_t exclusive_scan_u32(const uint32_t* in, const uint32_t* gather, uint32_t* out, int64_t n,
                               uint64_t* partials , uint64_t* total, hipStream_t s,
diff --git a/ms-gs_amd/csrc/sort.hip b/ms-gs_amd/csrc/sort.hip
--- a/ms-gs_amd/csrc/sort.hip
+++ b/ms-gs_amd/csrc/sort.hip
@@ -1,6 +1,8 @@
 #include "msgs_internal.h"
 
 #include <algorithm>
+#include <atomic>
+#include <cstdlib>
 
 namespace msgs {
 
@@ -153,14 +155,24 @@
     scan_store_items(out, tb, n, v);
 }
 
+struct ShiftDigit {
+    int shift;
+    uint32_t mask;
+    __device__ __forceinline__ uint32_t operator()(uint32_t k) const { return (k >> shift) & mask; }
+};
+struct BucketDigit {
+    const uint8_t* __restrict__ map;
+    __device__ __forceinline__ uint32_t operator()(uint32_t k) const { return map[depth_bin(k)]; }
+};
+
 template <int ITEMS = SORT_ITEMS>
 __device__ __forceinline__ int64_t elem_index(int64_t chunk_base, int w, int r, int lane) {
     return chunk_base + (int64_t)w * (64 * ITEMS) + r * 64 + lane;
 }
 
-template <int ITEMS, bool DROP = false, typename KeyT = uint32_t>
+template <int ITEMS, bool DROP = false, typename KeyT = uint32_t, typename Digit = ShiftDigit>
 __global__ __launch_bounds__(SORT_THREADS) void radix_hist_kernel(const KeyT* __restrict__ keys, int64_t n,
-                                                                  int shift, uint32_t mask, int64_t nblocks,
+                                                                  Digit dg, int64_t nblocks,
                                                                   uint32_t* __restrict__ hist,
                                                                   uint32_t* __restrict__ gsum, int gsize, int ngroups,
                                                                   const uint32_t* __restrict__ n_ptr = nullptr) {
@@ -183,7 +195,7 @@
 #pragma unroll
             for (int j = 0; j < KPV; ++j) {
                 const uint32_t k = sizeof(KeyT) == 4 ? w4[j] : ((w4[j >> 1] >> ((j & 1) * 16)) & 0xFFFFu);
-                if (!DROP || k != 0xFFFFFFFFu) atomicAdd(&s_hist[(k >> shift) & mask], 1u);
+                if (!DROP || k != 0xFFFFFFFFu) atomicAdd(&s_hist[dg(k)], 1u);
             }
         }
     } else {
@@ -192,7 +204,7 @@
             const int64_t i = elem_index<ITEMS>(chunk_base, w, r, lane);
             if (i < n) {
                 const uint32_t k = (uint32_t)keys[i];
-                if (!DROP || k != 0xFFFFFFFFu) atomicAdd(&s_hist[(k >> shift) & mask], 1u);
+                if (!DROP || k != 0xFFFFFFFFu) atomicAdd(&s_hist[dg(k)], 1u);
             }
         }
     }
@@ -241,12 +253,12 @@
     }
 }
 
-template <int ITEMS, bool DROP = false, typename KeyT = uint32_t>
+template <int ITEMS, bool DROP = false, typename KeyT = uint32_t, typename Digit = ShiftDigit>
 __global__ __launch_bounds__(SORT_THREADS) void radix_scatter_kernel(const KeyT* __restrict__ keys_in,
                                                                      const uint32_t* __restrict__ vals_in,
                                                                      KeyT* __restrict__ keys_out,
                                                                      uint32_t* __restrict__ vals_out, int64_t n,
-                                                                     int shift, uint32_t mask, int64_t nblocks,
+                                                                     Digit dg, int64_t nblocks,
                                                                      const uint32_t* __restrict__ hist_scanned,
                                                                      const uint32_t* __restrict__ gsum, int gsize,
                                                                      int ngroups, bool gsum_is_base = false,
@@ -272,7 +284,7 @@
         key[r] = i < n ? (uint32_t)keys_in[i] : 0xFFFFFFFFu;
         const bool valid = i < n && (!DROP || key[r] != 0xFFFFFFFFu);
         val[r] = valid ? (vals_in ? vals_in[i] : (uint32_t)i) : 0u;
-        const uint32_t d = (key[r] >> shift) & mask;
+        const uint32_t d = dg(key[r]);
         uint64_t peers = __ballot(valid);
 #pragma unroll
         for (int b = 0; b < 8; ++b) {
@@ -327,7 +339,7 @@
     for (int r = 0; r < ITEMS; ++r) {
         const int64_t i = elem_index<ITEMS>(chunk_base, w, r, lane);
         if (i < n && (!DROP || key[r] != 0xFFFFFFFFu)) {
-            const uint32_t lp = s_cnt[w][(key[r] >> shift) & mask] + rank[r];
+            const uint32_t lp = s_cnt[w][dg(key[r])] + rank[r];
             s_key[lp] = key[r];
             s_val[lp] = val[r];
         }
@@ -339,7 +351,7 @@
         const int j = r * SORT_THREADS + threadIdx.x;
         if (j < nvalid) {
             const uint32_t k = s_key[j];
-            const uint32_t pos = (uint32_t)j + s_delta[(k >> shift) & mask];
+            const uint32_t pos = (uint32_t)j + s_delta[dg(k)];
             keys_out[pos] = (KeyT)k;
             vals_out[pos] = s_val[j];
         }
@@ -425,19 +437,20 @@
                  const GroupGeom& G, uint32_t* hist, uint32_t* gs, bool drop, const uint32_t* n_ptr, uint32_t* n_out,
                  hipStream_t s) {
     const dim3 grid((unsigned)G.nb), block(SORT_THREADS);
+    const ShiftDigit dg{shift, mask};
     if (drop) {
-        hipLaunchKernelGGL((radix_hist_kernel<ITEMS, true, KeyT>), grid, block, 0, s, src_k, n, shift, mask, G.nb, hist, gs, G.gsize,
+        hipLaunchKernelGGL((radix_hist_kernel<ITEMS, true, KeyT>), grid, block, 0, s, src_k, n, dg, G.nb, hist, gs, G.gsize,
                            G.ngroups, (const uint32_t*)nullptr);
-        hipLaunchKernelGGL((radix_scatter_kernel<ITEMS, true, KeyT>), grid, block, 0, s, src_k, src_v, dst_k, dst_v, n, shift,
-                           mask, G.nb, hist, gs, G.gsize, G.ngroups, false, (const uint32_t*)nullptr, n_out);
+        hipLaunchKernelGGL((radix_scatter_kernel<ITEMS, true, KeyT>), grid, block, 0, s, src_k, src_v, dst_k, dst_v, n, dg,
+                           G.nb, hist, gs, G.gsize, G.ngroups, false, (const uint32_t*)nullptr, n_out);
         return;
     }
-    hipLaunchKernelGGL((radix_hist_kernel<ITEMS, false, KeyT>), grid, block, 0, s, src_k, n, shift, mask, G.nb, hist, gs, G.gsize,
+    hipLaunchKernelGGL((radix_hist_kernel<ITEMS, false, KeyT>), grid, block, 0, s, src_k, n, dg, G.nb, hist, gs, G.gsize,
                        G.ngroups, n_ptr);
     if (G.scanned)
         hipLaunchKernelGGL(group_scan_kernel, dim3((unsigned)G.ngroups + 1), dim3(256), 0, s, gs, G.ngroups, hist, G.gsize, G.nb, n_ptr,
                            SORT_THREADS * ITEMS);
-    hipLaunchKernelGGL((radix_scatter_kernel<ITEMS, false, KeyT>), grid, block, 0, s, src_k, src_v, dst_k, dst_v, n, shift, mask,
+    hipLaunchKernelGGL((radix_scatter_kernel<ITEMS, false, KeyT>), grid, block, 0, s, src_k, src_v, dst_k, dst_v, n, dg,
                        G.nb, hist, gs, G.gsize, G.ngroups, G.scanned, n_ptr, (uint32_t*)nullptr);
 }
 
@@ -502,4 +515,343 @@
                                  gsum_all, compact, n_valid_dev, n_dev, s);
 }
 
-}
+namespace {
+
+constexpr int DEPTH_LDS_WAVES = DEPTH_LDS_THREADS / 64;
+constexpr int DEPTH_HIST_THREADS = 1024;
+constexpr int DEPTH_HIST_WORDS = DEPTH_BINS / 2;
+static_assert(DEPTH_HIST_KEYS < 65536 && DEPTH_BINS % 2 == 0 && DEPTH_HIST_KEYS % 4 == 0, "16-bit counters in pairs; uint4 loads");
+
+__global__ __launch_bounds__(DEPTH_HIST_THREADS) void depth_hist_kernel(const uint32_t* __restrict__ keys, int64_t n,
+                                                                        uint32_t* __restrict__ slices, uint32_t* __restrict__ coarse) {
+    __shared__ __attribute__((aligned(16))) uint32_t s_h[DEPTH_HIST_WORDS];
+    const int tid = threadIdx.x, lane = tid & 63;
+    const int64_t first = (int64_t)blockIdx.x * DEPTH_HIST_KEYS;
+    const int64_t end = first + DEPTH_HIST_KEYS < n ? first + DEPTH_HIST_KEYS : n;
+    const bool aligned = (reinterpret_cast<uintptr_t>(keys) & 15) == 0;
+    constexpr int ROUNDS = DEPTH_HIST_KEYS / (4 * DEPTH_HIST_THREADS);
+    static_assert(ROUNDS * 4 * DEPTH_HIST_THREADS == DEPTH_HIST_KEYS, "whole rounds of uint4 loads");
+    uint32_t k4[ROUNDS][4];
+#pragma unroll
+    for (int r = 0; r < ROUNDS; ++r) {
+        const int64_t i0 = first + 4 * ((int64_t)r * DEPTH_HIST_THREADS + tid);
+        if (aligned && i0 + 4 <= end) {
+            const uint4 v = *reinterpret_cast<const uint4*>(keys + i0);
+            k4[r][0] = v.x; k4[r][1] = v.y; k4[r][2] = v.z; k4[r][3] = v.w;
+        } else {
+#pragma unroll
+            for (int j = 0; j < 4; ++j) k4[r][j] = i0 + j < end ? keys[i0 + j] : 0xFFFFFFFFu;
+        }
+    }
+    for (int q = tid; q < DEPTH_HIST_WORDS / 4; q += DEPTH_HIST_THREADS) reinterpret_cast<uint4*>(s_h)[q] = make_uint4(0u, 0u, 0u, 0u);
+    __syncthreads();
+#pragma unroll
+    for (int r = 0; r < ROUNDS; ++r) {
+#pragma unroll
+        for (int j = 0; j < 4; ++j) {
+            if (k4[r][j] != 0xFFFFFFFFu) {
+                const uint32_t b = depth_bin(k4[r][j]);
+                atomicAdd(&s_h[b >> 1], 1u << ((b & 1u) * 16));
+            }
+        }
+    }
+    __syncthreads();
+    uint4* out = reinterpret_cast<uint4*>(slices + (size_t)blockIdx.x * DEPTH_HIST_WORDS);
+    constexpr int QUADS = DEPTH_HIST_WORDS / 4;
+    static_assert(QUADS * 4 == DEPTH_HIST_WORDS && QUADS % 32 == 0, "whole uint4s; whole groups per half wave");
+#pragma unroll
+    for (int q0 = 0; q0 < QUADS; q0 += DEPTH_HIST_THREADS) {
+        const int q = q0 + tid;
+        const uint4 v = q < QUADS ? reinterpret_cast<const uint4*>(s_h)[q] : make_uint4(0u, 0u, 0u, 0u);
+        if (q < QUADS) out[q] = v;
+        uint32_t c = (v.x & 0xFFFFu) + (v.x >> 16) + (v.y & 0xFFFFu) + (v.y >> 16) + (v.z & 0xFFFFu) + (v.z >> 16) + (v.w & 0xFFFFu) + (v.w >> 16);
+        for (int off = 16; off > 0; off >>= 1) c += (uint32_t)__shfl_xor((int)c, off);
+        if ((lane & 31) == 0 && c) atomicAdd(&coarse[q >> 5], c);
+    }
+}
+
+__global__ __launch_bounds__(256) void depth_split_kernel(const uint16_t* __restrict__ slices, int nslices,
+                                                          const uint32_t* __restrict__ coarse, uint8_t* __restrict__ map,
+                                                          uint32_t* __restrict__ bases, uint32_t* __restrict__ n_valid,
+                                                          uint32_t* __restrict__ info) {
+    __shared__ uint32_t s_wave[4], s_last[5];
+    __shared__ uint64_t s_sum[4];
+    const int t = threadIdx.x, j = blockIdx.x;
+    static_assert(DEPTH_COARSE <= 512 && DEPTH_HIST_MAX_BLOCKS <= 64, "two group sums per thread; one slice per lane of wave 0");
+    const int b = j * 256 + t;
+    uint32_t cnt = 0;
+#pragma unroll 16
+    for (int k = 0; k < nslices; ++k) cnt += slices[(size_t)k * DEPTH_BINS + b];
+    uint32_t front = (t < nslices && j > 0) ? slices[(size_t)t * DEPTH_BINS + b - t - 1] : 0u;
+    for (int off = 32; off > 0; off >>= 1) front += (uint32_t)__shfl_xor((int)front, off);
+    if ((t & 63) == 63) s_last[(t >> 6) + 1] = cnt;
+    if (t == 0) s_last[0] = front;
+    const uint32_t c0 = t < DEPTH_COARSE ? coarse[t] : 0u;
+    const uint32_t c1 = t + 256 < DEPTH_COARSE ? coarse[t + 256] : 0u;
+    const uint32_t mine_before = (t < j ? c0 : 0u) + (t + 256 < j ? c1 : 0u);
+    const uint64_t both = block_sum_u64(((uint64_t)mine_before << 32) + ((uint64_t)c0 + c1), s_sum);
+    const uint32_t before = (uint32_t)(both >> 32), V = (uint32_t)both;
+    uint32_t total;
+    const uint32_t excl = block_exclusive_scan(cnt, s_wave, &total) + before;
+    const int bucket = V ? (int)((uint64_t)excl * DEPTH_BUCKETS / V) : 0;
+    map[b] = (uint8_t)bucket;
+    uint32_t cnt_prev = (uint32_t)__shfl_up((int)cnt, 1);
+    if ((t & 63) == 0) cnt_prev = s_last[t >> 6];
+    const int prev = b == 0 ? -1 : (V ? (int)((uint64_t)(excl - cnt_prev) * DEPTH_BUCKETS / V) : 0);
+    for (int k = prev + 1; k <= bucket; ++k) bases[k] = excl;
+    if (b == DEPTH_BINS - 1)
+        for (int k = bucket + 1; k <= DEPTH_BUCKETS + 1; ++k) bases[k] = V;
+    if (b == 0) {
+        if (n_valid) *n_valid = V;
+        info[0] = 1u;
+        info[1] = 0u;
+    }
+}
+
+__device__ __forceinline__ void lds_rank(const uint32_t (&key)[DEPTH_LDS_ITEMS], uint32_t (&rank)[DEPTH_LDS_ITEMS], int R, int nloc,
+                                         int shift, uint32_t (*s_cnt)[256], uint32_t* s_wsum, uint32_t* s_dcount) {
+    const int tid = threadIdx.x, lane = tid & 63, w = tid >> 6;
+    for (int k = tid; k < DEPTH_LDS_WAVES * 256; k += DEPTH_LDS_THREADS) (&s_cnt[0][0])[k] = 0;
+    __syncthreads();
+    const uint64_t lt_mask = (1ull << lane) - 1ull;
+#pragma unroll
+    for (int r = 0; r < DEPTH_LDS_ITEMS; ++r) {
+        if (r < R) {
+            const bool valid = w * 64 * R + r * 64 + lane < nloc;
+            const uint32_t d = shift < 32 ? (key[r] >> shift) & 255u : 0u;
+            uint64_t peers = __ballot(valid);
+#pragma unroll
+            for (int b = 0; b < 8; ++b) {
+                const uint64_t m = __ballot((d >> b) & 1u);
+                peers &= ((d >> b) & 1u) ? m : ~m;
+            }
+            const uint32_t prev = s_cnt[w][d];
+            const uint32_t before = (uint32_t)__popcll(peers & lt_mask);
+            rank[r] = prev + before;
+            if (valid && before == 0) s_cnt[w][d] = prev + (uint32_t)__popcll(peers);
+        }
+    }
+    __syncthreads();
+    uint32_t c[DEPTH_LDS_WAVES], ltot = 0;
+    if (tid < 256) {
+#pragma unroll
+        for (int k = 0; k < DEPTH_LDS_WAVES; ++k) { c[k] = s_cnt[k][tid]; ltot += c[k]; }
+    }
+    const uint32_t inc = wave_inclusive_scan(ltot, lane);
+    if (tid < 256 && lane == 63) s_wsum[w] = inc;
+    __syncthreads();
+    if (tid < 256) {
+        uint32_t run = inc - ltot;
+#pragma unroll
+        for (int k = 0; k < 4; ++k) run += k < w ? s_wsum[k] : 0u;
+#pragma unroll
+        for (int k = 0; k < DEPTH_LDS_WAVES; ++k) { s_cnt[k][tid] = run; run += c[k]; }
+        s_dcount[tid] = ltot;
+    }
+    __syncthreads();
+}
+
+__global__ __launch_bounds__(DEPTH_LDS_THREADS) void depth_lds_sort_kernel(uint32_t* keys_a, uint32_t* vals_a, uint32_t* keys_out,
+                                                                           uint32_t* vals_out, const uint32_t* __restrict__ bases,
+                                                                           int64_t n, uint32_t* __restrict__ info) {
+    __shared__ uint32_t s_key[DEPTH_LDS_CAP], s_val[DEPTH_LDS_CAP];
+    __shared__ uint32_t s_cnt[DEPTH_LDS_WAVES][256];
+    __shared__ uint32_t s_wsum[4], s_dcount[256], s_run[256], s_or;
+    const int tid = threadIdx.x, lane = tid & 63, w = tid >> 6;
+    uint32_t lo = bases[blockIdx.x], hi = bases[blockIdx.x + 1];
+    if (hi > (uint32_t)n) hi = (uint32_t)n;
+    if (lo >= hi) return;
+    const int64_t count = (int64_t)hi - lo;
+
+    uint32_t key[DEPTH_LDS_ITEMS], val[DEPTH_LDS_ITEMS], rank[DEPTH_LDS_ITEMS];
+    const bool fits = count <= DEPTH_LDS_CAP;
+    const int R = fits ? ((int)count + DEPTH_LDS_THREADS - 1) / DEPTH_LDS_THREADS : DEPTH_LDS_ITEMS;
+
+    if (tid == 0) s_or = 0;
+    __syncthreads();
+    {
+        const uint32_t k0 = keys_a[lo];
+        uint32_t diff = 0;
+        if (fits) {
+#pragma unroll
+            for (int r = 0; r < DEPTH_LDS_ITEMS; ++r) {
+                const int e = w * 64 * R + r * 64 + lane;
+                const bool valid = r < R && e < (int)count;
+                key[r] = valid ? keys_a[lo + e] : 0xFFFFFFFFu;
+                val[r] = valid ? vals_a[lo + e] : 0u;
+            }
+#pragma unroll
+            for (int r = 0; r < DEPTH_LDS_ITEMS; ++r) {
+                const int e = w * 64 * R + r * 64 + lane;
+                if (r < R && e < (int)count) diff |= key[r] ^ k0;
+            }
+        } else {
+            for (int64_t i = tid; i < count; i += DEPTH_LDS_THREADS) diff |= keys_a[lo + i] ^ k0;
+        }
+        for (int off = 32; off > 0; off >>= 1) diff |= (uint32_t)__shfl_xor((int)diff, off);
+        if (lane == 0 && diff) atomicOr(&s_or, diff);
+    }
+    __syncthreads();
+    const int bits = 32 - __clz((int)s_or);
+    int npass = (bits + 7) / 8;
+
+    if (fits) {
+        const int nloc = (int)count;
+        if (npass == 0) {
+#pragma unroll
+            for (int r = 0; r < DEPTH_LDS_ITEMS; ++r) {
+                const int e = w * 64 * R + r * 64 + lane;
+                if (r < R && e < nloc) { keys_out[lo + e] = key[r]; vals_out[lo + e] = val[r]; }
+            }
+            return;
+        }
+        for (int p = 0; p < npass; ++p) {
+            lds_rank(key, rank, R, nloc, 8 * p, s_cnt, s_wsum, s_dcount);
+#pragma unroll
+            for (int r = 0; r < DEPTH_LDS_ITEMS; ++r) {
+                const int e = w * 64 * R + r * 64 + lane;
+                if (r < R && e < nloc) {
+                    const uint32_t lp = s_cnt[w][(key[r] >> (8 * p)) & 255u] + rank[r];
+                    s_key[lp] = key[r];
+                    s_val[lp] = val[r];
+                }
+            }
+            __syncthreads();
+            if (p + 1 < npass) {
+#pragma unroll
+                for (int r = 0; r < DEPTH_LDS_ITEMS; ++r) {
+                    const int e = w * 64 * R + r * 64 + lane;
+                    if (r < R && e < nloc) { key[r] = s_key[e]; val[r] = s_val[e]; }
+                }
+            }
+        }
+        for (int i = tid; i < nloc; i += DEPTH_LDS_THREADS) {
+            keys_out[lo + i] = s_key[i];
+            vals_out[lo + i] = s_val[i];
+        }
+        return;
+    }
+
+    if (tid == 0) atomicAdd(&info[1], 1u);
+    if ((npass & 1) == 0) ++npass;
+    for (int p = 0; p < npass; ++p) {
+        const int shift = 8 * p;
+        const uint32_t* src_k = (p & 1) ? keys_out : keys_a;
+        const uint32_t* src_v = (p & 1) ? vals_out : vals_a;
+        uint32_t* dst_k = (p & 1) ? keys_a : keys_out;
+        uint32_t* dst_v = (p & 1) ? vals_a : vals_out;
+        if (tid < 256) s_run[tid] = 0;
+        __syncthreads();
+        for (int64_t i = tid; i < count; i += DEPTH_LDS_THREADS)
+            atomicAdd(&s_run[shift < 32 ? (src_k[lo + i] >> shift) & 255u : 0u], 1u);
+        __syncthreads();
+        if (tid == 0) {
+            uint32_t run = 0;
+            for (int d = 0; d < 256; ++d) { const uint32_t c = s_run[d]; s_run[d] = run; run += c; }
+        }
+        __syncthreads();
+        for (int64_t c0 = 0; c0 < count; c0 += DEPTH_LDS_CAP) {
+            const int nloc = (int)(count - c0 < DEPTH_LDS_CAP ? count - c0 : DEPTH_LDS_CAP);
+            const int R = DEPTH_LDS_ITEMS;
+#pragma unroll
+            for (int r = 0; r < DEPTH_LDS_ITEMS; ++r) {
+                const int e = w * 64 * R + r * 64 + lane;
+                key[r] = e < nloc ? src_k[lo + c0 + e] : 0xFFFFFFFFu;
+                val[r] = e < nloc ? src_v[lo + c0 + e] : 0u;
+            }
+            lds_rank(key, rank, R, nloc, shift, s_cnt, s_wsum, s_dcount);
+#pragma unroll
+            for (int r = 0; r < DEPTH_LDS_ITEMS; ++r) {
+                const int e = w * 64 * R + r * 64 + lane;
+                if (e < nloc) {
+                    const uint32_t d = shift < 32 ? (key[r] >> shift) & 255u : 0u;
+                    const uint32_t pos = s_run[d] + (s_cnt[w][d] + rank[r] - s_cnt[0][d]);
+                    dst_k[lo + pos] = key[r];
+                    dst_v[lo + pos] = val[r];
+                }
+            }
+            __syncthreads();
+            if (tid < 256) s_run[tid] += s_dcount[tid];
+            __syncthreads();
+        }
+        __threadfence();
+        __syncthreads();
+    }
+}
+
+std::atomic<int> g_depth_sort{[] {
+    const char* e = getenv("MSGS_DEPTH_SORT");
+    return (e && (e[0] == '1' || e[0] == '2') && e[1] == 0) ? e[0] - '0' : 0;
+}()};
+
+template <int ITEMS>
+void launch_bucket_pass(const uint32_t* src_k, uint32_t* dst_k, uint32_t* dst_v, int64_t n, const uint8_t* map, const GroupGeom& G,
+                        uint32_t* hist, uint32_t* gs, hipStream_t s) {
+    const dim3 grid((unsigned)G.nb), block(SORT_THREADS);
+    const BucketDigit dg{map};
+    hipLaunchKernelGGL((radix_hist_kernel<ITEMS, true, uint32_t, BucketDigit>), grid, block, 0, s, src_k, n, dg, G.nb, hist, gs,
+                       G.gsize, G.ngroups, (const uint32_t*)nullptr);
+    hipLaunchKernelGGL((radix_scatter_kernel<ITEMS, true, uint32_t, BucketDigit>), grid, block, 0, s, src_k, (const uint32_t*)nullptr,
+                       dst_k, dst_v, n, dg, G.nb, (const uint32_t*)hist, (const uint32_t*)gs, G.gsize, G.ngroups, false,
+                       (const uint32_t*)nullptr, (uint32_t*)nullptr);
+}
+
+}
+
+int set_depth_sort(int mode) { return g_depth_sort.exchange(mode == 1 || mode == 2 ? mode : 0); }
+int get_depth_sort() { return g_depth_sort.load(); }
+
+bool depth_sort_uses_buckets(int64_t n) {
+    const int mode = g_depth_sort.load();
+    if (mode == 1 || n <= 0 || n > DEPTH_BUCKET_HARD_MAX) return false;
+    return mode == 2 || n <= DEPTH_BUCKET_MAX_P;
+}
+
+bool depth_sort_zero_region(int64_t n, char* scratch, uint32_t** ptr, size_t* words) {
+    const DepthSortScratch L(n);
+    size_t w = 0;
+    if (!radix_sort_zero_region(n, 0, 32, scratch + L.sort, ptr, &w)) return false;
+    *words = (size_t)((scratch + L.zero_end()) - reinterpret_cast<char*>(*ptr)) / 4;
+    return true;
+}
+
+hipError_t depth_sort_buckets(const uint32_t* keys_in, uint32_t* keys_out, uint32_t* vals_out, int64_t n, char* scratch,
+                              hipStream_t s, bool pre_zeroed, uint32_t* n_valid_dev, uint32_t* info) {
+    if (n <= 0) {
+        if (n_valid_dev) hipLaunchKernelGGL(store_u32_kernel, dim3(1), dim3(1), 0, s, n_valid_dev, 0u);
+        return hipSuccess;
+    }
+    const GroupGeom G(n);
+    if (n > DEPTH_BUCKET_HARD_MAX) return hipErrorInvalidValue;
+    const DepthSortScratch L(n);
+    const SortScratch SS(n);
+    char* sort = scratch + L.sort;
+    uint32_t* keys_a = reinterpret_cast<uint32_t*>(sort + SS.keys_alt);
+    uint32_t* vals_a = reinterpret_cast<uint32_t*>(sort + SS.vals_alt);
+    uint32_t* hist = reinterpret_cast<uint32_t*>(sort + SS.hist);
+    uint32_t* gsum = hist + (size_t)256 * G.nb;
+    uint32_t* slices = reinterpret_cast<uint32_t*>(scratch + L.slices);
+    uint32_t* coarse = reinterpret_cast<uint32_t*>(scratch + L.coarse);
+    uint8_t* map = reinterpret_cast<uint8_t*>(scratch + L.map);
+    uint32_t* bases = reinterpret_cast<uint32_t*>(scratch + L.bases);
+    if (!info) info = bases + DEPTH_BUCKETS + 2;
+    if (!pre_zeroed) {
+        uint32_t* zp = nullptr;
+        size_t zw = 0;
+        if (!depth_sort_zero_region(n, scratch, &zp, &zw)) return hipErrorInvalidValue;
+        const hipError_t e = launch_zero(zp, sizeof(uint32_t) * zw, s);
+        if (e != hipSuccess) return e;
+    }
+    const int hb = depth_hist_blocks(n);
+    hipLaunchKernelGGL(depth_hist_kernel, dim3((unsigned)hb), dim3(DEPTH_HIST_THREADS), 0, s, keys_in, n, slices, coarse);
+    hipLaunchKernelGGL(depth_split_kernel, dim3(DEPTH_COARSE), dim3(256), 0, s, (const uint16_t*)slices, hb, (const uint32_t*)coarse, map,
+                       bases, n_valid_dev, info);
+    if (G.big) launch_bucket_pass<16>(keys_in, keys_a, vals_a, n, map, G, hist, gsum, s);
+    else if (G.mid) launch_bucket_pass<8>(keys_in, keys_a, vals_a, n, map, G, hist, gsum, s);
+    else launch_bucket_pass<SORT_ITEMS>(keys_in, keys_a, vals_a, n, map, G, hist, gsum, s);
+    hipLaunchKernelGGL(depth_lds_sort_kernel, dim3(DEPTH_BUCKETS), dim3(DEPTH_LDS_THREADS), 0, s, keys_a, vals_a, keys_out, vals_out,
+                       (const uint32_t*)bases, n, info);
+    return hipGetLastError();
+}
+
+}
diff --git a/ms-gs_amd/diff_gaussian_rasterization/_backend.py b/ms-gs_amd/diff_gaussian_rasterization/_backend.py
--- a/ms-gs_amd/diff_gaussian_rasterization/_backend.py
+++ b/ms-gs_amd/diff_gaussian_rasterization/_backend.py
@@ -147,6 +147,10 @@
     lib.msgs_set_occlusion.argtypes = [C.c_int32]
     lib.msgs_occlusion_stats.restype = C.c_int
     lib.msgs_occlusion_stats.argtypes = [vp, sz, C.c_int32, C.POINTER(C.c_int64), vp]
+    lib.msgs_set_depth_sort.restype = C.c_int
+    lib.msgs_set_depth_sort.argtypes = [C.c_int32]
+    lib.msgs_depth_sort_stats.restype = C.c_int
+    lib.msgs_depth_sort_stats.argtypes = [vp, sz, C.c_int32, C.POINTER(C.c_int64), vp]
     lib.msgs_slab_stats.restype = C.c_int
     lib.msgs_slab_stats.argtypes = [vp, sz, C.c_int32, C.POINTER(C.c_int64), vp]
     lib.msgs_forward.restype = C.c_int
@@ -294,7 +298,8 @@
            "msgs_features_scratch_bytes", "msgs_features_forward", "msgs_features_backward",
            "msgs_distortion_forward", "msgs_distortion_backward",
            "msgs_median_depth_forward", "msgs_median_depth_backward",
-           "msgs_screen_compensation_forward", "msgs_screen_compensation_backward", "msgs_screen_compensation_scratch_bytes")
+           "msgs_screen_compensation_forward", "msgs_screen_compensation_backward", "msgs_screen_compensation_scratch_bytes",
+           "msgs_set_depth_sort", "msgs_depth_sort_stats")
 
 
 def check(rc, where):
```

After: 2011, median of 6. 1.02x the previous value.
